# faasm/faabric

Hardware: AMD Instinct MI355X
Metric: MPI_Allreduce GB/s + batch-exec msgs/sec, 8-rank world at 1/2/4/8 MI355X (higher is better)
Workload: dtype fp32; 1 GPU; model=faabric composite: 256MB fp32 allreduce + 1MB alltoall + kvtouch batch, global_batch=128, parallelism=mpi1, allreduce_bytes=268435456, pingpong_bytes=0, kv_bytes=4096, full=False, snapshot_bytes_per_rank=0, snapshot_dirty=random-scattered 25pct, random-byte region, gpu=True

## Files before the change

### cpp/bindings/bindings_runtime.cpp

```cpp
#include <pybind11/functional.h>
#include <pybind11/pybind11.h>
#include <pybind11/stl.h>

#include "faabricamd/endpoint.h"
#include "faabricamd/executor.h"
#include "faabricamd/flat.h"
#include "faabricamd/hipipc.h"
#include "faabricamd/planner.h"
#include "faabricamd/ptp.h"
#include "faabricamd/runner.h"
#include "faabricamd/scheduler.h"
#include "faabricamd/snapshot.h"
#include "faabricamd/state.h"
#include "faabricamd/util.h"
#include "faabricamd/utilextras.h"
#include "faabricamd/dirty.h"
#include <hip/hip_runtime.h>

namespace py = pybind11;
using namespace faabricamd;

namespace faabricamd {
void registerBenchFunctions();
std::map<std::string, std::vector<uint8_t>> benchLastOutputs();
void registerMpiExampleFunctions();
}

void initRuntimeBindings(py::module_& m)
{
    m.def("set_endpoint_host", [](const std::string& host) {
        getSystemConfig().endpointHost = host;
    });
    m.def("get_endpoint_host",
          [] { return getSystemConfig().endpointHost; });
    m.def("set_planner_host", [](const std::string& host) {
        getSystemConfig().plannerHost = host;
        resetPlannerClient();
    });
    m.def("set_batch_scheduler_mode", [](const std::string& mode) {
        resetBatchScheduler(mode);
    });
    m.def("test_make_scheduling_decision",
          [](const std::string& mode,
             const std::vector<std::tuple<std::string, int, int>>& hosts,
             int nMessages,
             int32_t appId,
             bool migration,
             const std::vector<std::pair<int32_t, std::vector<std::string>>>&
               inFlight) {
              std::shared_ptr<BatchScheduler> sched;
              if (mode == "bin-pack") {
                  sched = std::make_shared<BinPackScheduler>();
              } else if (mode == "compact") {
                  sched = std::make_shared<CompactScheduler>();
              } else if (mode == "spot") {
                  sched = std::make_shared<SpotScheduler>();
              } else {
                  throw FaabricException("bad mode");
              }
              HostMap hostMap;
              for (const auto& [ip, slots, used] : hosts) {
                  hostMap[ip] =
                    std::make_shared<HostState>(ip, slots, used);
              }
              InFlightReqs reqs;
              for (const auto& [ifAppId, ifHosts] : inFlight) {
                  auto ber = std::make_shared<BatchExecuteRequest>();
                  ber->appId = ifAppId;
                  ber->user = "t";
                  ber->function = "t";
                  auto dec =
                    std::make_shared<SchedulingDecision>(ifAppId, 1);
                  int idx = 0;
                  for (const auto& h : ifHosts) {
                      Message m;
                      m.id = ifAppId * 1000 + idx;
                      m.appId = ifAppId;
                      m.appIdx = idx;
                      m.groupIdx = idx;
                      ber->messages.push_back(m);
                      dec->addMessage(h, m);
                      idx++;
                  }
                  reqs[ifAppId] = { ber, dec };
              }
              BatchExecuteRequest req;
              req.appId = appId;
              req.user = "t";
              req.function = "t";
              req.type = migration ? BatchExecuteType::MIGRATION
                                   : BatchExecuteType::FUNCTIONS;
              for (int i = 0; i < nMessages; i++) {
                  Message m;
                  m.id = appId * 1000 + i;
                  m.appId = appId;
                  m.appIdx = i;
                  m.groupIdx = i;
                  req.messages.push_back(m);
              }
              return *sched->makeSchedulingDecision(hostMap, reqs, req);
          },
          py::arg("mode"),
          py::arg("hosts"),
          py::arg("n_messages"),
          py::arg("app_id") = 12345,
          py::arg("migration") = false,
          py::arg("in_flight") =
            std::vector<std::pair<int32_t, std::vector<std::string>>>{});
    m.def("decision_cache_size",
          [] { return DecisionCache::get().size(); });
    m.def("decision_cache_clear", [] { DecisionCache::get().clear(); });

    py::class_<SchedulingDecision>(m, "SchedulingDecision")
      .def(py::init<>())
      .def_readwrite("app_id", &SchedulingDecision::appId)
      .def_readwrite("group_id", &SchedulingDecision::groupId)
      .def_readwrite("n_functions", &SchedulingDecision::nFunctions)
      .def_readwrite("hosts", &SchedulingDecision::hosts)
      .def_readwrite("message_ids", &SchedulingDecision::messageIds)
      .def_readwrite("app_idxs", &SchedulingDecision::appIdxs)
      .def_readwrite("group_idxs", &SchedulingDecision::groupIdxs)
      .def_readwrite("mpi_ports", &SchedulingDecision::mpiPorts);

    m.def("NOT_ENOUGH_SLOTS", [] { return NOT_ENOUGH_SLOTS; });
    m.def("DO_NOT_MIGRATE", [] { return DO_NOT_MIGRATE; });
    m.def("MUST_FREEZE", [] { return MUST_FREEZE; });

    py::class_<PlannerRuntime>(m, "PlannerRuntime")
      .def(py::init<>())
      .def("start",
           &PlannerRuntime::start,
           py::arg("with_snapshot_server") = true,
           py::arg("with_state_server") = false,
           py::call_guard<py::gil_scoped_release>())
      .def("shutdown",
           &PlannerRuntime::shutdown,
           py::call_guard<py::gil_scoped_release>());

    py::class_<FaabricMain>(m, "FaabricMain")
      .def(py::init([]() {
          return new FaabricMain(getExecutorFactory());
      }))
      .def("start_background",
           &FaabricMain::startBackground,
           py::call_guard<py::gil_scoped_release>())
      .def("shutdown",
           &FaabricMain::shutdown,
           py::call_guard<py::gil_scoped_release>());

    m.def("register_function",
          [](const std::string& user,
             const std::string& function,
             py::function fn) {
              FunctionRegistry::get().registerFunction(
                user, function, [fn](Message& msg) -> int32_t {
                    py::gil_scoped_acquire gil;
                    py::object result = fn(&msg);
                    if (result.is_none()) {
                        return 0;
                    }
                    return result.cast<int32_t>();
                });
          });
    m.def("clear_function_registry",
          [] { FunctionRegistry::get().clear(); });

    m.def("register_native_noop",
          [](const std::string& user, const std::string& function) {
              FunctionRegistry::get().registerFunction(
                user, function, [](Message&) -> int32_t { return 0; });
          });
    m.def("register_native_echo",
          [](const std::string& user, const std::string& function) {
              FunctionRegistry::get().registerFunction(
                user, function, [](Message& msg) -> int32_t {
                    msg.outputData.assign(msg.inputData.begin(),
                                          msg.inputData.end());
                    return 0;
                });
          });
    m.def("register_native_sleep",
          [](const std::string& user,
             const std::string& function,
             int sleepMs) {
              FunctionRegistry::get().registerFunction(
                user, function, [sleepMs](Message&) -> int32_t {
                    std::this_thread::sleep_for(
                      std::chrono::milliseconds(sleepMs));
                    return 0;
                });
          });

    m.def(
      "call_functions",
      [](const BatchExecuteRequest& reqIn) {
          auto req = std::make_shared<BatchExecuteRequest>(reqIn);
          py::gil_scoped_release release;
          return *getPlannerClient().callFunctions(req);
      });
    m.def(
      "get_message_result",
      [](int32_t appId, int32_t msgId, int timeoutMs) {
          py::gil_scoped_release release;
          return getPlannerClient().getMessageResult(appId, msgId, timeoutMs);
      });
    m.def("get_batch_results", [](int32_t appId) {
        py::gil_scoped_release release;
        return getPlannerClient().getBatchResults(appId);
    });
    m.def("get_available_hosts", [] {
        py::gil_scoped_release release;
        return getPlannerClient().getAvailableHosts();
    });
    m.def("get_num_migrations", [] {
        py::gil_scoped_release release;
        return getPlannerClient().getNumMigrations();
    });
    m.def("preload_scheduling_decision",
          [](int32_t appId, const SchedulingDecision& decision) {
              py::gil_scoped_release release;
              getPlannerClient().preloadSchedulingDecision(appId, decision);
          });
    m.def("planner_ping", [] {
        py::gil_scoped_release release;
        getPlannerClient().ping();
    });

    m.def("planner_reset", [] { Planner::get().reset(); });
    m.def("planner_flush_scheduling_state",
          [] { Planner::get().flushSchedulingState(); });
    m.def("planner_set_next_evicted_vms",
          [](const std::vector<std::string>& ips) {
              Planner::get().setNextEvictedVm(
                { ips.begin(), ips.end() });
          });
    m.def("planner_set_policy",
          [](const std::string& p) { Planner::get().setPolicy(p); });
    m.def("planner_get_policy", [] { return Planner::get().getPolicy(); });
    m.def("planner_num_in_flight_apps", [] {
        return (int)Planner::get().getInFlightApps().apps.size();
    });

    m.def("set_this_host_resources", [](int slots, int usedSlots) {
        HostResources res;
        res.slots = slots;
        res.usedSlots = usedSlots;
        Scheduler::get().setThisHostResources(res);
    });
    m.def("get_this_host_slots", [] {
        return Scheduler::get().getThisHostResources().slots;
    });
    m.def("get_executor_count",
          [] { return (int)Scheduler::get().getExecutorCount(); });
    m.def("scheduler_reset", [] {
        py::gil_scoped_release release;
        Scheduler::get().reset();
    });
    m.def("get_recorded_messages",
          [] { return Scheduler::get().getRecordedMessages(); });
    m.def("set_test_mode", &setTestMode);

    m.def("ptp_send",
          [](int32_t appId,
             int32_t groupId,
             int32_t sendIdx,
             int32_t recvIdx,
             const py::bytes& data,
             bool ordered) {
              std::string s = data;
              py::gil_scoped_release release;
              getPointToPointBroker().sendMessage(appId,
                                                  groupId,
                                                  sendIdx,
                                                  recvIdx,
                                                  (const uint8_t*)s.data(),
                                                  s.size(),
                                                  ordered);
          },
          py::arg("app_id"),
          py::arg("group_id"),
          py::arg("send_idx"),
          py::arg("recv_idx"),
          py::arg("data"),
          py::arg("ordered") = false);
    m.def("ptp_recv",
          [](int32_t groupId,
             int32_t sendIdx,
             int32_t recvIdx,
             bool ordered,
             int timeoutMs) {
              std::vector<uint8_t> out;
              {
                  py::gil_scoped_release release;
                  out = getPointToPointBroker().recvMessage(
                    groupId, sendIdx, recvIdx, ordered, timeoutMs);
              }
              return py::bytes((const char*)out.data(), out.size());
          },
          py::arg("group_id"),
          py::arg("send_idx"),
          py::arg("recv_idx"),
          py::arg("ordered") = false,
          py::arg("timeout_ms") = DEFAULT_QUEUE_TIMEOUT_MS);
    m.def("ptp_send_device",
          [](int32_t appId,
             int32_t groupId,
             int32_t sendIdx,
             int32_t recvIdx,
             uintptr_t devPtr,
             size_t size,
             bool ordered) {
              py::gil_scoped_release release;
              getPointToPointBroker().sendMessageDevice(
                appId, groupId, sendIdx, recvIdx, (const void*)devPtr,
                size, ordered);
          },
          py::arg("app_id"),
          py::arg("group_id"),
          py::arg("send_idx"),
          py::arg("recv_idx"),
          py::arg("dev_ptr"),
          py::arg("size"),
          py::arg("ordered") = false);
    m.def("ptp_recv_device",
          [](int32_t groupId,
             int32_t sendIdx,
             int32_t recvIdx,
             uintptr_t devPtr,
             size_t capacity,
             bool ordered,
             int timeoutMs) {
              py::gil_scoped_release release;
              return getPointToPointBroker().recvMessageDevice(
                groupId, sendIdx, recvIdx, (void*)devPtr, capacity,
                ordered, timeoutMs);
          },
          py::arg("group_id"),
          py::arg("send_idx"),
          py::arg("recv_idx"),
          py::arg("dev_ptr"),
          py::arg("capacity"),
          py::arg("ordered") = false,
          py::arg("timeout_ms") = DEFAULT_QUEUE_TIMEOUT_MS);
    m.def("ptp_group_barrier", [](int32_t groupId, int32_t groupIdx) {
        py::gil_scoped_release release;
        PointToPointGroup::getOrAwaitGroup(groupId)->barrier(groupIdx);
    });
    m.def("ptp_group_lock",
          [](int32_t groupId, int32_t groupIdx, bool recursive) {
              py::gil_scoped_release release;
              PointToPointGroup::getOrAwaitGroup(groupId)->lock(groupIdx,
                                                                recursive);
          },
          py::arg("group_id"),
          py::arg("group_idx"),
          py::arg("recursive") = false);
    m.def("ptp_group_unlock",
          [](int32_t groupId, int32_t groupIdx, bool recursive) {
              py::gil_scoped_release release;
              PointToPointGroup::getOrAwaitGroup(groupId)->unlock(groupIdx,
                                                                  recursive);
          },
          py::arg("group_id"),
          py::arg("group_idx"),
          py::arg("recursive") = false);
    m.def("ptp_group_notify", [](int32_t groupId, int32_t groupIdx) {
        py::gil_scoped_release release;
        PointToPointGroup::getOrAwaitGroup(groupId)->notify(groupIdx);
    });
    m.def("ptp_setup_local_mappings", [](const SchedulingDecision& d) {
        getPointToPointBroker().setUpLocalMappingsFromSchedulingDecision(d);
    });
    m.def("ptp_clear", [] { getPointToPointBroker().clear(); });
    m.def("_test_ptp_deliver_seq",
          [](int32_t appId,
             int32_t groupId,
             int32_t sendIdx,
             int32_t recvIdx,
             const py::bytes& data,
             uint32_t seq) {
              PointToPointMessage msg;
              msg.appId = appId;
              msg.groupId = groupId;
              msg.sendIdx = sendIdx;
              msg.recvIdx = recvIdx;
              std::string s = data;
              msg.data.assign(s.begin(), s.end());
              py::gil_scoped_release release;
              getPointToPointBroker().deliverRemoteMessage(msg, seq);
          });
    py::class_<PointToPointServer>(m, "PointToPointServerHandle")
      .def(py::init<>())
      .def("start",
           [](PointToPointServer& s) {
               py::gil_scoped_release release;
               s.start();
           })
      .def("stop", [](PointToPointServer& s) {
          py::gil_scoped_release release;
          s.stop();
      });
    py::class_<StateServer>(m, "StateServerHandle")
      .def(py::init<>())
      .def("start",
           [](StateServer& s) {
               py::gil_scoped_release release;
               s.start();
           })
      .def("stop", [](StateServer& s) {
          py::gil_scoped_release release;
          s.stop();
      });
    py::class_<SnapshotServer>(m, "SnapshotServerHandle")
      .def(py::init<>())
      .def("start",
           [](SnapshotServer& s) {
               py::gil_scoped_release release;
               s.start();
           })
      .def("stop", [](SnapshotServer& s) {
          py::gil_scoped_release release;
          s.stop();
      });
    m.def("snapshot_push_device_from_ptr",
          [](const std::string& host,
             const std::string& key,
             uintptr_t devPtr,
             size_t size) {
              py::gil_scoped_release release;
              getSnapshotClient(host)->pushDeviceSnapshotFromDevice(
                key, (const void*)devPtr, size);
          },
          py::arg("host"),
          py::arg("key"),
          py::arg("dev_ptr"),
          py::arg("size"));
    m.def("ipc_shipped", [] {
        return py::make_tuple(IpcSender::get().shippedSegments(),
                              IpcSender::get().shippedBytes());
    });
    m.def("ipc_available",
          [](const std::string& host) {
              py::gil_scoped_release release;
              return IpcSender::get().available(host);
          },
          py::arg("host"));
    m.def("ptp_wait_for_mappings", [](int32_t groupId) {
        py::gil_scoped_release release;
        getPointToPointBroker().waitForMappingsOnThisHost(groupId);
    });

    py::class_<StateKeyValue, std::shared_ptr<StateKeyValue>>(m,
                                                              "StateKeyValue")
      .def_property_readonly("user", &StateKeyValue::getUser)
      .def_property_readonly("key", &StateKeyValue::getKey)
      .def_property_readonly("size", &StateKeyValue::size)
      .def_property_readonly("is_master", &StateKeyValue::isMaster)
      .def_property_readonly("master_host", &StateKeyValue::getMasterHost)
      .def_property_readonly("on_device", &StateKeyValue::isOnDevice)
      .def_property_readonly("data_ptr",
                             [](StateKeyValue& kv) {
                                 return (uintptr_t)kv.getDataPtr();
                             })
      .def("get",
           [](StateKeyValue& kv) {
               std::vector<uint8_t> out;
               {
                   py::gil_scoped_release release;
                   out = kv.get();
               }
               return py::bytes((const char*)out.data(), out.size());
           })
      .def("set",
           [](StateKeyValue& kv, const py::bytes& data) {
               std::string s = data;
               py::gil_scoped_release release;
               kv.set((const uint8_t*)s.data(), s.size());
           })
      .def("get_chunk",
           [](StateKeyValue& kv, uint64_t offset, size_t len) {
               std::vector<uint8_t> out(len);
               {
                   py::gil_scoped_release release;
                   kv.getChunk(offset, out.data(), len);
               }
               return py::bytes((const char*)out.data(), out.size());
           })
      .def("set_chunk",
           [](StateKeyValue& kv, uint64_t offset, const py::bytes& data) {
               std::string s = data;
               py::gil_scoped_release release;
               kv.setChunk(offset, (const uint8_t*)s.data(), s.size());
           })
      .def("append",
           [](StateKeyValue& kv, const py::bytes& data) {
               std::string s = data;
               py::gil_scoped_release release;
               kv.append((const uint8_t*)s.data(), s.size());
           })
      .def("get_appended",
           [](StateKeyValue& kv, size_t n) {
               std::vector<std::vector<uint8_t>> vals;
               {
                   py::gil_scoped_release release;
                   vals = kv.getAppended(n);
               }
               py::list out;
               for (auto& v : vals) {
                   out.append(py::bytes((const char*)v.data(), v.size()));
               }
               return out;
           })
      .def("clear_appended", [](StateKeyValue& kv) {
          py::gil_scoped_release release;
          kv.clearAppended();
      })
      .def("pull",
           [](StateKeyValue& kv) {
               py::gil_scoped_release release;
               kv.pull();
           })
      .def("push_partial", [](StateKeyValue& kv) {
          py::gil_scoped_release release;
          kv.pushPartial();
      })
      .def("push_full", [](StateKeyValue& kv) {
          py::gil_scoped_release release;
          kv.pushFull();
      })
      .def("sync", [](StateKeyValue& kv) {
          py::gil_scoped_release release;
          kv.sync();
      });
    m.def("state_sync_all", [] {
        py::gil_scoped_release release;
        State::get().syncAll();
    });
    m.def("set_state_mode", [](const std::string& mode) {
        getSystemConfig().stateMode = mode;
    });
    m.def("state_acquire_lock",
          [](const std::string& user, const std::string& key,
             int expiryMs) {
              py::gil_scoped_release release;
              return State::get().acquireLock(user, key, expiryMs);
          },
          py::arg("user"),
          py::arg("key"),
          py::arg("expiry_ms") = 10000);
    m.def("state_release_lock",
          [](const std::string& user, const std::string& key,
             uint64_t token) {
              py::gil_scoped_release release;
              State::get().releaseLock(user, key, token);
          });

    m.def("state_get_kv_device",
          [](const std::string& user,
             const std::string& key,
             size_t size,
             int device) {
              return State::get().getKVDevice(user, key, size, device);
          },
          py::arg("user"),
          py::arg("key"),
          py::arg("size"),
          py::arg("device") = 0);
    m.def("state_get_kv",
          [](const std::string& user, const std::string& key, size_t size) {
              return State::get().getKV(user, key, size);
          });
    m.def("state_set_master_host",
          [](const std::string& user,
             const std::string& key,
             const std::string& host) {
              State::get().setMasterHost(user, key, host);
          });
    m.def("state_size",
          [](const std::string& user, const std::string& key) {
              py::gil_scoped_release release;
              return State::get().getStateSize(user, key);
          });
    m.def("state_clear_all", [] { State::get().forceClearAll(false); });
    m.def("state_kv_count", [] { return State::get().getKVCount(); });

    py::enum_<SnapshotDataType>(m, "SnapshotDataType")
      .value("Raw", SnapshotDataType::Raw)
      .value("Bool", SnapshotDataType::Bool)
      .value("Int", SnapshotDataType::Int)
      .value("Long", SnapshotDataType::Long)
      .value("Float", SnapshotDataType::Float)
      .value("Double", SnapshotDataType::Double);

    py::enum_<SnapshotMergeOperation>(m, "SnapshotMergeOperation")
      .value("Bytewise", SnapshotMergeOperation::Bytewise)
      .value("Sum", SnapshotMergeOperation::Sum)
      .value("Product", SnapshotMergeOperation::Product)
      .value("Subtract", SnapshotMergeOperation::Subtract)
      .value("Max", SnapshotMergeOperation::Max)
      .value("Min", SnapshotMergeOperation::Min)
      .value("XOR", SnapshotMergeOperation::XOR);

    py::class_<SnapshotDiff>(m, "SnapshotDiff")
      .def(py::init<>())
      .def_readwrite("data_type", &SnapshotDiff::dataType)
      .def_readwrite("operation", &SnapshotDiff::operation)
      .def_readwrite("offset", &SnapshotDiff::offset)
      .def_property(
        "data",
        [](const SnapshotDiff& d) {
            return py::bytes((const char*)d.getData(), d.size());
        },
        [](SnapshotDiff& d, const py::bytes& b) {
            std::string s = b;
            d.dataCopy.assign(s.begin(), s.end());
        });

    py::class_<SnapshotData, std::shared_ptr<SnapshotData>>(m,
                                                            "SnapshotData")
      .def(py::init([](const py::bytes& data, size_t maxSize) {
               std::string s = data;
               std::vector<uint8_t> v(s.begin(), s.end());
               if (maxSize == 0) {
                   return std::make_shared<SnapshotData>(v);
               }
               return std::make_shared<SnapshotData>(v, maxSize);
           }),
           py::arg("data"),
           py::arg("max_size") = 0)
      .def(py::init([](size_t size) {
          return std::make_shared<SnapshotData>(size);
      }))
      .def_property_readonly("size", &SnapshotData::getSize)
      .def_property_readonly("max_size", &SnapshotData::getMaxSize)
      .def("get_data",
           [](SnapshotData& s) {
               auto v = s.getDataCopy();
               return py::bytes((const char*)v.data(), v.size());
           })
      .def("copy_in_data",
           [](SnapshotData& s, const py::bytes& data, uint32_t offset) {
               std::string str = data;
               s.copyInData((const uint8_t*)str.data(), str.size(), offset);
           },
           py::arg("data"),
           py::arg("offset") = 0)
      .def("add_merge_region",
           &SnapshotData::addMergeRegion,
           py::arg("offset"),
           py::arg("length"),
           py::arg("data_type"),
           py::arg("operation"))
      .def("fill_gaps_with_bytewise_regions",
           &SnapshotData::fillGapsWithBytewiseRegions)
      .def("clear_merge_regions", &SnapshotData::clearMergeRegions)
      .def("diff_with_memory",
           [](SnapshotData& s, const py::bytes& updated) {
               std::string str = updated;
               return s.diffWithMemory((const uint8_t*)str.data(),
                                       str.size());
           })
      .def("diff_with_dirty_regions",
           [](SnapshotData& s,
              const py::bytes& updated,
              const std::vector<char>& dirtyPages) {
               std::string str = updated;
               return s.diffWithDirtyRegions(
                 (const uint8_t*)str.data(), str.size(), dirtyPages);
           })
      .def("apply_diffs", &SnapshotData::applyDiffs)
      .def("queue_diffs", &SnapshotData::queueDiffs)
      .def("write_queued_diffs", &SnapshotData::writeQueuedDiffs);

    m.def("snapshot_register",
          [](const std::string& key, std::shared_ptr<SnapshotData> snap) {
              SnapshotRegistry::get().registerSnapshot(key, snap);
          });
    m.def("snapshot_get", [](const std::string& key) {
        return SnapshotRegistry::get().getSnapshot(key);
    });
    m.def("snapshot_exists", [](const std::string& key) {
        return SnapshotRegistry::get().snapshotExists(key);
    });
    m.def("snapshot_delete", [](const std::string& key) {
        SnapshotRegistry::get().deleteSnapshot(key);
    });
    m.def("snapshot_count",
          [] { return SnapshotRegistry::get().getSnapshotCount(); });
    m.def("snapshot_clear", [] { SnapshotRegistry::get().clear(); });

    m.def("get_batch_requests_sent_mock", [] {
        return getBatchRequestsSentMock();
    });
    m.def("clear_mocked_function_calls", &clearMockedFunctionCalls);

    m.def("delta_default_config", [] { return DeltaConfig{}.str(); });
    m.def("flat_encode_push",
          [](const std::string& key, uint64_t maxSize,
             const py::bytes& contents,
             const std::vector<std::tuple<int32_t, uint64_t, int32_t,
                                          int32_t>>& regions) {
              FlatSnapshotPush req;
              req.key = key;
              req.maxSize = maxSize;
              std::string c = contents;
              req.contents.assign(c.begin(), c.end());
              for (auto& [off, len, dt, op] : regions) {
                  FlatMergeRegion m;
                  m.offset = off;
                  m.length = len;
                  m.dataType = dt;
                  m.mergeOp = op;
                  req.mergeRegions.push_back(m);
              }
              std::string out = req.encode();
              return py::bytes(out);
          });
    m.def("flat_decode_push", [](const py::bytes& buf) {
        std::string s = buf;
        auto req = FlatSnapshotPush::decode(s);
        py::list regions;
        for (auto& m : req.mergeRegions) {
            regions.append(py::make_tuple(m.offset, m.length, m.dataType,
                                          m.mergeOp));
        }
        return py::make_tuple(
          req.key, req.maxSize,
          py::bytes((const char*)req.contents.data(),
                    req.contents.size()),
          regions);
    });
    m.def("flat_encode_thread_result",
          [](int32_t appId, int32_t messageId, int32_t returnValue,
             const std::string& key,
             const std::vector<std::tuple<int32_t, int32_t, int32_t,
                                          py::bytes>>& diffs) {
              FlatThreadResult req;
              req.appId = appId;
              req.messageId = messageId;
              req.returnValue = returnValue;
              req.key = key;
              for (auto& [off, dt, op, data] : diffs) {
                  FlatSnapshotDiff d;
                  d.offset = off;
                  d.dataType = dt;
                  d.mergeOp = op;
                  std::string s = data;
                  d.data.assign(s.begin(), s.end());
                  req.diffs.push_back(std::move(d));
              }
              return py::bytes(req.encode());
          });
    m.def("flat_decode_thread_result", [](const py::bytes& buf) {
        std::string s = buf;
        auto req = FlatThreadResult::decode(s);
        py::list diffs;
        for (auto& d : req.diffs) {
            diffs.append(py::make_tuple(
              d.offset, d.dataType, d.mergeOp,
              py::bytes((const char*)d.data.data(), d.data.size())));
        }
        return py::make_tuple(req.appId, req.messageId, req.returnValue,
                              req.key, diffs, req.executedHost);
    });
    m.def("delta_encode",
          [](const py::bytes& oldData,
             const py::bytes& newData,
             const std::string& config) {
              std::string o = oldData;
              std::string n = newData;
              DeltaConfig conf = config.empty() ? DeltaConfig{}
                                                : DeltaConfig::parse(config);
              auto out = deltaEncode({ o.begin(), o.end() },
                                     { n.begin(), n.end() },
                                     conf);
              return py::bytes((const char*)out.data(), out.size());
          },
          py::arg("old_data"),
          py::arg("new_data"),
          py::arg("config") = "");
    m.def("delta_apply",
          [](const py::bytes& oldData, const py::bytes& delta) {
              std::string o = oldData;
              std::string d = delta;
              auto out = deltaApply({ o.begin(), o.end() },
                                    { d.begin(), d.end() });
              return py::bytes((const char*)out.data(), out.size());
          });
    m.def("prof_summary", &profSummary);
    m.def("prof_clear", &profClear);
    m.def("set_up_crash_handler", &setUpCrashHandler);
    m.def("pin_thread_to_free_cpu", &pinThreadToFreeCpu);

    m.def("_selftest_segfault_tracker", [] {
        py::gil_scoped_release release;
        SegfaultDirtyTracker tracker;
        PageAlignedBuffer buf;
        buf.resize(16 * 4096);
        tracker.startTracking(buf.data(), buf.size());
        buf.data()[3 * 4096 + 5] = 42;
        buf.data()[9 * 4096] = 7;
        tracker.stopTracking(buf.data(), buf.size());
        auto dirty = tracker.getDirtyPages(buf.data(), buf.size());
        int nDirty = 0;
        for (char c : dirty) {
            nDirty += c != 0;
        }
        return nDirty == 2 && dirty[3] == 1 && dirty[9] == 1;
    });

    m.def("_selftest_uffd_tracker", []() -> py::object {
        if (!UffdDirtyTracker::isAvailable()) {
            return py::none();
        }
        bool ok;
        {
            py::gil_scoped_release release;
            UffdDirtyTracker tracker;
            PageAlignedBuffer buf;
            buf.resize(16 * 4096);
            tracker.startTracking(buf.data(), buf.size());
            buf.data()[2 * 4096 + 11] = 42;
            buf.data()[14 * 4096] = 7;
            tracker.stopTracking(buf.data(), buf.size());
            auto dirty = tracker.getDirtyPages(buf.data(), buf.size());
            int nDirty = 0;
            for (char d : dirty) {
                nDirty += d != 0;
            }
            ok = nDirty == 2 && dirty[2] == 1 && dirty[14] == 1;
        }
        return py::bool_(ok);
    });

    m.def("_selftest_softpte_tracker", []() -> py::object {
        if (!SoftPTEDirtyTracker::isAvailable()) {
            return py::none();
        }
        bool ok;
        {
            py::gil_scoped_release release;
            SoftPTEDirtyTracker tracker;
            PageAlignedBuffer buf;
            buf.resize(16 * 4096);
            std::memset(buf.data(), 1, buf.size());
            tracker.startTracking(buf.data(), buf.size());
            buf.data()[5 * 4096 + 3] = 42;
            buf.data()[12 * 4096] = 7;
            tracker.stopTracking(buf.data(), buf.size());
            auto dirty = tracker.getDirtyPages(buf.data(), buf.size());
            ok = dirty.size() == 16 && dirty[5] == 1 && dirty[12] == 1;
        }
        return py::bool_(ok);
    });

    m.def("_debug_runtime_sizes", [] {
        py::dict d;
        d["planner_app_results"] = Planner::get().debugAppResultsCount();
        d["planner_done_apps"] = Planner::get().debugDoneAppsCount();
        d["planner_in_flight"] = Planner::get().debugInFlightCount();
        d["broker_mappings"] = getPointToPointBroker().debugMappingsCount();
        d["broker_channels"] = getPointToPointBroker().debugChannelsCount();
        d["broker_send_seqs"] = getPointToPointBroker().debugSendSeqsCount();
        d["decision_cache"] = DecisionCache::get().size();
        return d;
    });
    m.def("_debug_kv_commit_stats", [] {
        KvCommitStats s = kvCommitStats();
        py::dict d;
        d["launches"] = s.launches;
        d["pages"] = s.pages;
        return d;
    });
    m.def("_debug_kv_sweep_bitmap",
          [](size_t nPages, const std::vector<uint64_t>& setBits) {
              size_t nWords = (nPages + 63) / 64;
              auto words = std::make_unique<std::atomic<uint64_t>[]>(
                std::max<size_t>(nWords, 1));
              for (size_t w = 0; w < nWords; w++) {
                  words[w].store(0);
              }
              for (uint64_t b : setBits) {
                  if (b >= nPages) {
                      throw FaabricException("bit beyond the bitmap");
                  }
                  words[b / 64].fetch_or(1ULL << (b % 64));
              }
              std::vector<uint32_t> pages(nPages);
              size_t n =
                kvSweepDirtyBitmap(words.get(), nPages, pages.data());
              pages.resize(n);
              std::vector<uint64_t> after(nWords);
              for (size_t w = 0; w < nWords; w++) {
                  after[w] = words[w].load();
              }
              return py::make_tuple(pages, after);
          },
          py::arg("n_pages"),
          py::arg("set_bits"));
    m.def("wait_batch_done",
          [](int32_t appId, int timeoutMs) {
              py::gil_scoped_release release;
              return getPlannerClient().waitBatchDone(appId, timeoutMs);
          },
          py::arg("app_id"),
          py::arg("timeout_ms") = 30000);
    m.def("set_bound_timeout",
          [](int ms) { getSystemConfig().boundTimeout = ms; });
    m.def("reap_stale_executors", [] {
        py::gil_scoped_release release;
        return Scheduler::get().reapStaleExecutors();
    });
    m.def("register_bench_functions", [] { registerBenchFunctions(); });
    m.def("bench_last_outputs", [] {
        py::dict d;
        for (const auto& [name, data] : benchLastOutputs()) {
            d[py::str(name)] =
              py::bytes((const char*)data.data(), data.size());
        }
        return d;
    });
    m.def("register_mpi_example_functions",
          [] { registerMpiExampleFunctions(); });

    m.def("execute_threads",
          [](const std::string& user,
             const std::string& function,
             int nThreads,
             const std::vector<std::tuple<uint32_t, size_t, int, int>>&
               regions,
             const py::bytes& inputData,
             bool elastic) {
              Executor* exec = ExecutorContext::get().getExecutor();
              std::string input = inputData;
              std::vector<std::pair<int32_t, int32_t>> results;
              {
                  py::gil_scoped_release release;
                  auto req = std::make_shared<BatchExecuteRequest>(
                    batchExecFactory(user, function, nThreads));
                  req->elasticScaleHint = elastic;
                  for (auto& m2 : req->messages) {
                      m2.inputData.assign(input.begin(), input.end());
                  }
                  std::vector<SnapshotMergeRegion> mr;
                  for (const auto& [off, len, dt, op] : regions) {
                      mr.emplace_back(off,
                                      len,
                                      (SnapshotDataType)dt,
                                      (SnapshotMergeOperation)op);
                  }
                  results = exec->executeThreads(req, mr);
              }
              py::list out;
              for (auto& [msgId, rv] : results) {
                  out.append(py::make_tuple(msgId, rv));
              }
              return out;
          },
          py::arg("user"),
          py::arg("function"),
          py::arg("n_threads"),
          py::arg("merge_regions") =
            std::vector<std::tuple<uint32_t, size_t, int, int>>{},
          py::arg("input_data") = py::bytes(""),
          py::arg("elastic") = false);

    m.def("chain_function",
          [](const std::string& user,
             const std::string& function,
             const py::bytes& input) {
              std::string s = input;
              std::vector<uint8_t> in(s.begin(), s.end());
              py::gil_scoped_release release;
              return chainFunction(user, function, in);
          },
          py::arg("user"),
          py::arg("function"),
          py::arg("input") = py::bytes(""));
    m.def("await_chained_call", [](int32_t msgId, int timeoutMs) {
        py::gil_scoped_release release;
        return awaitChainedCall(msgId, timeoutMs);
    },
          py::arg("msg_id"),
          py::arg("timeout_ms") = 60000);
    m.def("get_exec_graph_json", [](int32_t appId, int32_t msgId) {
        return getExecGraphJson(appId, msgId);
    });
    m.def("migration_point",
          [](const py::bytes& reentryInput) {
              std::string s = reentryInput;
              std::vector<uint8_t> in(s.begin(), s.end());
              py::gil_scoped_release release;
              return migrationPoint(in);
          },
          py::arg("reentry_input") = py::bytes(""));
    m.def("MIGRATED_FUNCTION_RETURN_VALUE",
          [] { return MIGRATED_FUNCTION_RETURN_VALUE; });
    m.def("FROZEN_FUNCTION_RETURN_VALUE",
          [] { return FROZEN_FUNCTION_RETURN_VALUE; });

    py::class_<PlannerEndpoint>(m, "PlannerEndpoint")
      .def(py::init<int>(), py::arg("port") = PLANNER_HTTP_PORT)
      .def("start",
           &PlannerEndpoint::start,
           py::call_guard<py::gil_scoped_release>())
      .def("stop",
           &PlannerEndpoint::stop,
           py::call_guard<py::gil_scoped_release>())
      .def("handle", [](PlannerEndpoint& ep, const std::string& body) {
          std::pair<int, std::string> out;
          {
              py::gil_scoped_release release;
              out = ep.handle(body);
          }
          return py::make_tuple(out.first, out.second);
      });

    m.def("executor_set_memory_size", [](size_t n) {
        ExecutorContext::get().getExecutor()->setMemorySize(n);
    });
    m.def("executor_memory_size", [] {
        return ExecutorContext::get().getExecutor()->getMemoryView().second;
    });
    m.def("executor_write_memory", [](size_t offset, const py::bytes& data) {
        std::string s = data;
        auto [base, size] = ExecutorContext::get().getExecutor()
                              ->getMemoryView();
        if (offset + s.size() > size) {
            throw FaabricException("executor memory write out of bounds");
        }
        std::memcpy(base + offset, s.data(), s.size());
    });
    m.def("executor_read_memory", [](size_t offset, size_t n) {
        auto [base, size] = ExecutorContext::get().getExecutor()
                              ->getMemoryView();
        if (offset + n > size) {
            throw FaabricException("executor memory read out of bounds");
        }
        return py::bytes((const char*)base + offset, n);
    });

    m.def("executor_set_device_memory_size", [](size_t n) {
        py::gil_scoped_release release;
        ExecutorContext::get().getExecutor()->setDeviceMemorySize(n);
    });
    m.def("executor_device_ptr", [] {
        return (uintptr_t)ExecutorContext::get()
          .getExecutor()
          ->getDeviceMemoryView()
          .first;
    });
    m.def("executor_device_write_memory",
          [](size_t offset, const py::bytes& data) {
              std::string s = data;
              auto [base, size] = ExecutorContext::get()
                                    .getExecutor()
                                    ->getDeviceMemoryView();
              if (base == nullptr || offset + s.size() > size) {
                  throw FaabricException("device arena write out of bounds");
              }
              py::gil_scoped_release release;
              if (hipMemcpy(base + offset, s.data(), s.size(),
                            hipMemcpyHostToDevice) != hipSuccess) {
                  throw FaabricException("device arena write failed");
              }
          });
    m.def("executor_device_read_memory", [](size_t offset, size_t n) {
        auto [base, size] =
          ExecutorContext::get().getExecutor()->getDeviceMemoryView();
        if (base == nullptr || offset + n > size) {
            throw FaabricException("device arena read out of bounds");
        }
        std::vector<uint8_t> out(n);
        {
            py::gil_scoped_release release;
            if (hipMemcpy(out.data(), base + offset, n,
                          hipMemcpyDeviceToHost) != hipSuccess) {
                throw FaabricException("device arena read failed");
            }
        }
        return py::bytes((const char*)out.data(), out.size());
    });
}
```

### cpp/include/faabricamd/executor.h

```cpp
#pragma once

#include <atomic>
#include <functional>
#include <memory>
#include <string>
#include <thread>
#include <vector>

#include "faabricamd/messages.h"
#include "faabricamd/queue.h"
#include "faabricamd/dirty.h"
#include "faabricamd/snapshot.h"

namespace faabricamd {

class Executor;


class ExecutorContext
{
  public:
    static bool isSet();
    static void set(Executor* executor,
                    std::shared_ptr<BatchExecuteRequest> req,
                    int msgIdx);
    static void unset();
    static ExecutorContext& get();

    Executor* getExecutor() const { return executor; }
    std::shared_ptr<BatchExecuteRequest> getBatchRequest() const
    {
        return req;
    }
    Message& getMsg();
    int getMsgIdx() const { return msgIdx; }

  private:
    Executor* executor = nullptr;
    std::shared_ptr<BatchExecuteRequest> req;
    int msgIdx = 0;
};


using FaabricFunction = std::function<int32_t(Message&)>;

class FunctionRegistry
{
  public:
    static FunctionRegistry& get();
    void registerFunction(const std::string& user,
                          const std::string& function,
                          FaabricFunction fn);
    FaabricFunction* getFunction(const std::string& user,
                                 const std::string& function);
    void clear();

  private:
    std::mutex mx;
    std::map<std::string, FaabricFunction> functions;
};


struct ExecutorTask
{
    ExecutorTask() = default;
    ExecutorTask(int msgIdxIn, std::shared_ptr<BatchExecuteRequest> reqIn)
      : msgIdx(msgIdxIn)
      , req(std::move(reqIn))
    {}
    int msgIdx = 0;
    std::shared_ptr<BatchExecuteRequest> req;
    bool stop = false;
};

class Executor
{
  public:
    explicit Executor(Message& msg);
    virtual ~Executor();

    void executeTasks(std::vector<int> msgIdxs,
                      std::shared_ptr<BatchExecuteRequest> req);

    std::vector<std::pair<int32_t, int32_t>> executeThreads(
      std::shared_ptr<BatchExecuteRequest> req,
      const std::vector<SnapshotMergeRegion>& mergeRegions);

    virtual int32_t executeTask(int threadPoolIdx,
                                int msgIdx,
                                std::shared_ptr<BatchExecuteRequest> req);

    virtual std::pair<uint8_t*, size_t> getMemoryView();
    virtual void setMemorySize(size_t newSize);
    void setDeviceMemorySize(size_t newSize);
    std::pair<uint8_t*, size_t> getDeviceMemoryView();
    bool hasDeviceArena() const { return deviceArena != nullptr; }
    virtual void restore(const std::string& snapshotKey);
    virtual void reset(Message& msg);
    virtual void flush();

    bool tryClaim();
    void claim();
    void releaseClaim();
    bool isClaimed() const { return claimed.load(); }

    long getMillisSinceLastExec() const;
    void shutdown();

    std::string id;
    Message boundMsg;
    int gpuDevice = -1;

    void setThreadResult(Message& msg,
                         int32_t returnValue,
                         const std::string& key,
                         const std::vector<SnapshotDiffMsg>& diffs);

  protected:
    void threadPoolThread(int poolIdx);
    void handleTaskResult(Message& msg,
                          int32_t returnValue,
                          std::shared_ptr<BatchExecuteRequest> req,
                          bool isLastInBatch);

    int threadPoolSize = 0;
    std::vector<std::shared_ptr<Queue<ExecutorTask>>> threadTaskQueues;
    std::vector<std::thread> threadPoolThreads;
    std::mutex threadsMx;

    std::atomic<bool> claimed{ false };
    std::atomic<int64_t> lastExecMs{ 0 };

    std::string lastForkSnapshotKey;
    std::vector<std::string> lastForkRemoteHosts;
    void cleanupForkSnapshot();

    std::shared_ptr<std::atomic<int>> batchCounter;

    PageAlignedBuffer dummyMemory;

    uint8_t* deviceArena = nullptr;
    size_t deviceArenaSize = 0;
};

class ExecutorFactory
{
  public:
    virtual ~ExecutorFactory() = default;
    virtual std::shared_ptr<Executor> createExecutor(Message& msg)
    {
        return std::make_shared<Executor>(msg);
    }
    virtual void flushHost() {}
};

void setExecutorFactory(std::shared_ptr<ExecutorFactory> factory);
std::shared_ptr<ExecutorFactory> getExecutorFactory();

int32_t chainFunction(const std::string& user,
                      const std::string& function,
                      const std::vector<uint8_t>& input);
Message awaitChainedCall(int32_t msgId, int timeoutMs = 60000);

int32_t migrationPoint(const std::vector<uint8_t>& reentryInput);

}
```

### cpp/include/faabricamd/planner.h

```cpp
#pragma once

#include <deque>
#include <atomic>
#include <map>
#include <memory>
#include <set>
#include <shared_mutex>
#include <thread>
#include <vector>

#include "faabricamd/messages.h"
#include "faabricamd/queue.h"
#include "faabricamd/scheduling.h"
#include "faabricamd/transport.h"

namespace faabricamd {

enum class PlannerCalls : uint8_t
{
    Ping = 1,
    GetAvailableHosts = 2,
    RegisterHost = 3,
    RemoveHost = 4,
    SetMessageResult = 8,
    SetMessageResultBatch = 15,
    GetMessageResult = 9,
    GetBatchResults = 10,
    GetSchedulingDecision = 11,
    GetNumMigrations = 12,
    CallBatch = 13,
    PreloadSchedulingDecision = 14,
    WaitBatchDone = 16,
};

inline constexpr int NUM_MPI_PORTS_PER_HOST = 64;

struct PlannerHost
{
    Host info;
    std::vector<bool> mpiPortUsed =
      std::vector<bool>(NUM_MPI_PORTS_PER_HOST, false);
};

struct PlannerState
{
    std::map<std::string, std::shared_ptr<PlannerHost>> hostMap;
    InFlightReqs inFlightReqs;
    std::map<int32_t, std::shared_ptr<SchedulingDecision>>
      preloadedSchedulingDecisions;
    std::map<int32_t, std::map<int32_t, std::shared_ptr<Message>>> appResults;
    std::deque<std::pair<int64_t, int32_t>> doneApps;
    std::map<int32_t, std::vector<std::string>> appResultWaiters;
    std::map<int32_t, std::shared_ptr<BatchExecuteRequest>> evictedRequests;
    std::map<int32_t, std::vector<std::string>> batchDoneWaiters;
    std::map<int32_t,
             std::vector<std::pair<int32_t, std::vector<std::string>>>>
      supersededGroups;
    std::set<std::string> nextEvictedHostIps;
    int numMigrations = 0;
};

class Planner
{
  public:
    static Planner& get();

    PlannerConfig getConfig();
    void printConfig();

    bool registerHost(const Host& hostIn, bool overwrite);
    void removeHost(const Host& hostIn);
    std::vector<Host> getAvailableHosts();

    size_t debugAppResultsCount();
    size_t debugDoneAppsCount();
    size_t debugInFlightCount();

    bool registerBatchDoneWaiter(int32_t appId, const std::string& host);

    std::shared_ptr<SchedulingDecision> callBatch(
      std::shared_ptr<BatchExecuteRequest> req);
    void dispatchSchedulingDecision(
      std::shared_ptr<BatchExecuteRequest> req,
      std::shared_ptr<SchedulingDecision> decision);
    void preloadSchedulingDecision(
      int32_t appId,
      std::shared_ptr<SchedulingDecision> decision);
    std::shared_ptr<SchedulingDecision> getSchedulingDecision(int32_t appId);

    void setMessageResult(std::shared_ptr<Message> msg);
    void setMessageResults(std::vector<std::shared_ptr<Message>>& msgs);
    std::shared_ptr<Message> getMessageResult(const Message& msg);
    std::shared_ptr<BatchExecuteRequestStatus> getBatchResults(int32_t appId);

    int getNumMigrations();
    GetInFlightAppsResponse getInFlightApps();
    void setNextEvictedVm(const std::set<std::string>& vmIps);
    void setPolicy(const std::string& policy);
    std::string getPolicy();

    void reset();
    void flushExecutors();
    void flushSchedulingState();

    int hostTimeoutMs = 5000;

  private:
    void purgeOldResultsLocked();
    void setMessageResultLocked(
      const std::shared_ptr<Message>& msg,
      std::vector<std::pair<std::string, std::shared_ptr<Message>>>& waiters,
      std::vector<std::pair<std::string, int32_t>>& batchWaiters,
      std::vector<std::pair<std::string, int32_t>>& groupClears);

    Planner();

    std::shared_mutex plannerMx;
    PlannerState state;

    bool isHostExpired(const PlannerHost& host, int64_t nowMs) const;
    void flushHosts();
    std::shared_ptr<SchedulingDecision> getPreloadedSchedulingDecision(
      int32_t appId,
      const BatchExecuteRequest& req);
    int32_t claimHostMpiPort(std::shared_ptr<PlannerHost>& host);
    void releaseHostMpiPort(std::shared_ptr<PlannerHost>& host, int32_t port);
};


class PlannerServer : public MessageEndpointServer
{
  public:
    PlannerServer();
    ~PlannerServer() override;
    void doAsyncRecv(uint8_t code,
                     const std::string& body,
                     uint32_t seq) override;
    std::string doSyncRecv(uint8_t code, const std::string& body) override;

  private:
    void resultWorkerLoop();
    Queue<std::string> resultQueue;
    std::vector<std::thread> resultWorkers;
    std::atomic<bool> resultWorkersStop{ false };
};

class PlannerClient
{
  public:
    PlannerClient();
    ~PlannerClient();

    void ping();
    std::vector<Host> getAvailableHosts();
    int32_t registerHost(const Host& host, bool overwrite);
    void removeHost(const Host& host);

    std::shared_ptr<SchedulingDecision> callFunctions(
      std::shared_ptr<BatchExecuteRequest> req);

    void setMessageResult(std::shared_ptr<Message> msg);
    void setMessageResults(std::vector<std::shared_ptr<Message>>& msgs);
    void setMessageResultsBatch(
      const std::vector<std::shared_ptr<Message>>& msgs);
    void setMessageResultLocally(std::shared_ptr<Message> msg);

    Message getMessageResult(const Message& msg, int timeoutMs);
    Message getMessageResult(int32_t appId, int32_t msgId, int timeoutMs);
    BatchExecuteRequestStatus getBatchResults(int32_t appId);
    std::pair<bool, int> getBatchStatusCounts(int32_t appId);

    bool waitBatchDone(int32_t appId, int timeoutMs);

    SchedulingDecision getSchedulingDecision(int32_t appId);
    void preloadSchedulingDecision(
      int32_t appId,
      const SchedulingDecision& decision);
    int getNumMigrations();

    void startKeepAlive();
    void stopKeepAlive();
    void clearCache();

  private:
    MessageEndpointClient rpc;

    std::mutex resultsMx;
    std::condition_variable resultsCv;
    std::map<int32_t, std::shared_ptr<Message>> localResults;

    class KeepAliveThread;
    std::shared_ptr<KeepAliveThread> keepAlive;
};

PlannerClient& getPlannerClient();
void resetPlannerClient();

}
```

### cpp/include/faabricamd/scheduler.h

```cpp
#pragma once

#include <memory>
#include <mutex>
#include <shared_mutex>
#include <unordered_map>
#include <vector>

#include "faabricamd/executor.h"
#include "faabricamd/messages.h"
#include "faabricamd/queue.h"
#include "faabricamd/transport.h"

namespace faabricamd {

enum class FunctionCalls : uint8_t
{
    ExecuteFunctions = 1,
    Flush = 2,
    SetMessageResult = 3,
    BatchDone = 4,
};

class Scheduler
{
  public:
    static Scheduler& get();

    void executeBatch(std::shared_ptr<BatchExecuteRequest> req);

    HostResources getThisHostResources();
    void setThisHostResources(const HostResources& res);

    int reapStaleExecutors();
    void startReaper();
    void stopReaper();

    std::shared_ptr<PendingMigration> checkForMigrationOpportunities(
      Message& msg,
      int32_t overwriteNewGroupId = 0);

    void flushLocally();
    void shutdown();
    void reset();

    std::vector<Message> getRecordedMessages();
    void clearRecordedMessages();

    size_t getExecutorCount();

  private:
    Scheduler();

    std::shared_ptr<Executor> claimExecutor(Message& msg);

    std::shared_mutex schedMx;
    struct WarmPool
    {
        std::vector<std::shared_ptr<Executor>> list;
        std::atomic<size_t> hint{ 0 };
    };
    std::unordered_map<std::string, std::unique_ptr<WarmPool>> executors;
    HostResources overriddenResources;
    bool resourcesOverridden = false;

    std::vector<Message> recordedMessages;

    class ReaperThread;
    std::shared_ptr<ReaperThread> reaper;
};

bool functionCallServerRunning();

class FunctionCallServer : public MessageEndpointServer
{
  public:
    FunctionCallServer();
    ~FunctionCallServer() override;
    void doAsyncRecv(uint8_t code,
                     const std::string& body,
                     uint32_t seq) override;
    std::string doSyncRecv(uint8_t code, const std::string& body) override;
};

class FunctionCallClient : public MessageEndpointClient
{
  public:
    explicit FunctionCallClient(const std::string& host);
    void executeFunctions(const BatchExecuteRequest& req);
    void setMessageResult(const Message& msg);
    void sendFlush();
    void batchDone(int32_t appId);
};

std::shared_ptr<FunctionCallClient> getFunctionCallClient(
  const std::string& host);

std::shared_ptr<FlagWaiter> batchDoneWaiterPrepare(int32_t appId);
void batchDoneWaiterDiscard(int32_t appId);
void signalBatchDone(int32_t appId);
void clearFunctionCallClients();

std::vector<std::pair<std::string, BatchExecuteRequest>>
getBatchRequestsSentMock();
void clearMockedFunctionCalls();

}
```

### cpp/include/faabricamd/scheduling.h

```cpp
#pragma once

#include <map>
#include <mutex>
#include <memory>
#include <set>
#include <string>
#include <vector>

#include "faabricamd/messages.h"

namespace faabricamd {

inline constexpr int32_t DO_NOT_MIGRATE = -98;
inline constexpr int32_t NOT_ENOUGH_SLOTS = -99;
inline constexpr int32_t MUST_FREEZE = -97;
inline const std::string MUST_EVICT_IP = "E.VI.CT.ME";

inline constexpr int32_t FIXED_SIZE_PRELOADED_DECISION_GROUPID = -99;

enum class DecisionType
{
    NO_DECISION_TYPE = 0,
    NEW = 1,
    DIST_CHANGE = 2,
    SCALE_CHANGE = 3,
};

class SchedulingDecision
{
  public:
    SchedulingDecision() = default;
    SchedulingDecision(int32_t appIdIn, int32_t groupIdIn)
      : appId(appIdIn)
      , groupId(groupIdIn)
    {}

    static SchedulingDecision fromPointToPointMappings(
      const PointToPointMappings& mappings);
    PointToPointMappings toPointToPointMappings() const;

    bool operator==(const SchedulingDecision& rhs) const
    {
        return appId == rhs.appId && groupId == rhs.groupId &&
               hosts == rhs.hosts && messageIds == rhs.messageIds;
    }

    int32_t appId = 0;
    int32_t groupId = 0;
    int32_t nFunctions = 0;
    std::vector<std::string> hosts;
    std::vector<int32_t> messageIds;
    std::vector<int32_t> appIdxs;
    std::vector<int32_t> groupIdxs;
    std::vector<int32_t> mpiPorts;
    std::string returnHost;

    bool isSingleHost() const;
    void addMessage(const std::string& host, const Message& msg);
    void addMessage(const std::string& host,
                    int32_t messageId,
                    int32_t appIdx,
                    int32_t groupIdx);
    void addMessageInPosition(int32_t pos,
                              const std::string& host,
                              int32_t messageId,
                              int32_t appIdx,
                              int32_t groupIdx,
                              int32_t mpiPort);
    int32_t removeMessage(int32_t messageId);
    std::set<std::string> uniqueHosts() const;
    void print() const;
};

struct HostState
{
    HostState(std::string ipIn, int slotsIn, int usedSlotsIn)
      : ip(std::move(ipIn))
      , slots(slotsIn)
      , usedSlots(usedSlotsIn)
    {}
    std::string ip;
    int slots;
    int usedSlots;
};

using HostMap = std::map<std::string, std::shared_ptr<HostState>>;
using InFlightPair = std::pair<std::shared_ptr<BatchExecuteRequest>,
                               std::shared_ptr<SchedulingDecision>>;
using InFlightReqs = std::map<int32_t, InFlightPair>;

class BatchScheduler
{
  public:
    virtual ~BatchScheduler() = default;

    static DecisionType getDecisionType(
      const InFlightReqs& inFlightReqs,
      const BatchExecuteRequest& req);

    virtual std::shared_ptr<SchedulingDecision> makeSchedulingDecision(
      HostMap& hostMap,
      const InFlightReqs& inFlightReqs,
      const BatchExecuteRequest& req) = 0;

  protected:
    static int numSlotsAvailable(const std::shared_ptr<HostState>& h)
    {
        return std::max(0, h->slots - h->usedSlots);
    }
};

class BinPackScheduler : public BatchScheduler
{
  public:
    std::shared_ptr<SchedulingDecision> makeSchedulingDecision(
      HostMap& hostMap,
      const InFlightReqs& inFlightReqs,
      const BatchExecuteRequest& req) override;
};

class CompactScheduler : public BatchScheduler
{
  public:
    std::shared_ptr<SchedulingDecision> makeSchedulingDecision(
      HostMap& hostMap,
      const InFlightReqs& inFlightReqs,
      const BatchExecuteRequest& req) override;
};

class SpotScheduler : public BatchScheduler
{
  public:
    std::shared_ptr<SchedulingDecision> makeSchedulingDecision(
      HostMap& hostMap,
      const InFlightReqs& inFlightReqs,
      const BatchExecuteRequest& req) override;
};

class DecisionCache
{
  public:
    static DecisionCache& get();
    std::shared_ptr<SchedulingDecision> getCachedDecision(
      const BatchExecuteRequest& req);
    void addCachedDecision(const BatchExecuteRequest& req,
                           const SchedulingDecision& decision);
    void clear();
    size_t size();

  private:
    std::string keyOf(const BatchExecuteRequest& req);
    std::mutex mx;
    std::map<std::string, std::shared_ptr<SchedulingDecision>> cache;
};

std::shared_ptr<BatchScheduler> getBatchScheduler();
void resetBatchScheduler();
void resetBatchScheduler(const std::string& newMode);
std::string getBatchSchedulerMode();

std::shared_ptr<SchedulingDecision> minimiseNumOfMigrations(
  std::shared_ptr<SchedulingDecision> newDecision,
  std::shared_ptr<SchedulingDecision> oldDecision);

}
```

### cpp/include/faabricamd/utilextras.h

```cpp
#pragma once

#include <cstdint>
#include <string>
#include <vector>

namespace faabricamd {


struct DeltaConfig
{
    size_t pageSize = 4096;
    bool xorWithOld = true;
    bool compress = true;
    bool useZstd = true;

    static DeltaConfig parse(const std::string& s);
    std::string str() const;
};

std::vector<uint8_t> deltaEncode(const std::vector<uint8_t>& oldData,
                                 const std::vector<uint8_t>& newData,
                                 const DeltaConfig& conf = {});

std::vector<uint8_t> deltaApply(const std::vector<uint8_t>& oldData,
                                const std::vector<uint8_t>& delta);


void profStart(const std::string& name);
void profEnd(const std::string& name);
std::vector<std::pair<std::string, double>> profTotalsMs();
void profClear();
std::string profSummary();

#define PROF_START(name) ::faabricamd::profStart(#name);
#define PROF_END(name) ::faabricamd::profEnd(#name);

void setUpCrashHandler();

int pinThreadToFreeCpu();
void unpinThisThread();

}
```

### cpp/src/batchsched.cpp

```cpp
#include "faabricamd/scheduling.h"
#include "faabricamd/util.h"

#include <algorithm>
#include <mutex>

namespace faabricamd {


SchedulingDecision SchedulingDecision::fromPointToPointMappings(
  const PointToPointMappings& mappings)
{
    SchedulingDecision d(mappings.appId, mappings.groupId);
    for (const auto& m : mappings.mappings) {
        d.addMessageInPosition(
          d.nFunctions, m.host, m.messageId, m.appIdx, m.groupIdx, m.mpiPort);
    }
    return d;
}

PointToPointMappings SchedulingDecision::toPointToPointMappings() const
{
    PointToPointMappings out;
    out.appId = appId;
    out.groupId = groupId;
    for (int i = 0; i < nFunctions; i++) {
        PointToPointMapping m;
        m.host = hosts[i];
        m.messageId = messageIds[i];
        m.appIdx = appIdxs[i];
        m.groupIdx = groupIdxs[i];
        m.mpiPort = mpiPorts[i];
        out.mappings.push_back(std::move(m));
    }
    return out;
}

bool SchedulingDecision::isSingleHost() const
{
    const std::string& thisHost = getSystemConfig().endpointHost;
    return std::all_of(hosts.begin(), hosts.end(), [&](const auto& h) {
        return h == thisHost;
    });
}

void SchedulingDecision::addMessage(const std::string& host,
                                    const Message& msg)
{
    addMessage(host, msg.id, msg.appIdx, msg.groupIdx);
}

void SchedulingDecision::addMessage(const std::string& host,
                                    int32_t messageId,
                                    int32_t appIdx,
                                    int32_t groupIdx)
{
    nFunctions++;
    hosts.push_back(host);
    messageIds.push_back(messageId);
    appIdxs.push_back(appIdx);
    groupIdxs.push_back(groupIdx);
    mpiPorts.push_back(0);
}

void SchedulingDecision::addMessageInPosition(int32_t pos,
                                              const std::string& host,
                                              int32_t messageId,
                                              int32_t appIdx,
                                              int32_t groupIdx,
                                              int32_t mpiPort)
{
    int32_t desiredSize = std::max<int32_t>(pos + 1, nFunctions);
    nFunctions = desiredSize;
    if ((int32_t)hosts.size() < desiredSize) {
        hosts.resize(desiredSize);
        messageIds.resize(desiredSize, 0);
        appIdxs.resize(desiredSize, 0);
        groupIdxs.resize(desiredSize, 0);
        mpiPorts.resize(desiredSize, 0);
    }
    hosts[pos] = host;
    messageIds[pos] = messageId;
    appIdxs[pos] = appIdx;
    groupIdxs[pos] = groupIdx;
    mpiPorts[pos] = mpiPort;
}

int32_t SchedulingDecision::removeMessage(int32_t messageId)
{
    auto it = std::find(messageIds.begin(), messageIds.end(), messageId);
    if (it == messageIds.end()) {
        return 0;
    }
    size_t idx = (size_t)std::distance(messageIds.begin(), it);
    int32_t port = mpiPorts[idx];
    nFunctions--;
    size_t last = messageIds.size() - 1;
    hosts[idx] = std::move(hosts[last]);
    messageIds[idx] = messageIds[last];
    appIdxs[idx] = appIdxs[last];
    groupIdxs[idx] = groupIdxs[last];
    mpiPorts[idx] = mpiPorts[last];
    hosts.pop_back();
    messageIds.pop_back();
    appIdxs.pop_back();
    groupIdxs.pop_back();
    mpiPorts.pop_back();
    return port;
}

std::set<std::string> SchedulingDecision::uniqueHosts() const
{
    return { hosts.begin(), hosts.end() };
}

void SchedulingDecision::print() const
{
    FAM_DEBUG("decision app=%d group=%d n=%d", appId, groupId, nFunctions);
    for (int i = 0; i < nFunctions; i++) {
        FAM_DEBUG("  msg=%d appIdx=%d grpIdx=%d host=%s port=%d",
                  messageIds[i],
                  appIdxs[i],
                  groupIdxs[i],
                  hosts[i].c_str(),
                  mpiPorts[i]);
    }
}


DecisionType BatchScheduler::getDecisionType(const InFlightReqs& inFlightReqs,
                                             const BatchExecuteRequest& req)
{
    if (inFlightReqs.find(req.appId) == inFlightReqs.end()) {
        return DecisionType::NEW;
    }
    if (req.type == BatchExecuteType::MIGRATION) {
        return DecisionType::DIST_CHANGE;
    }
    return DecisionType::SCALE_CHANGE;
}

using HostPtr = std::shared_ptr<HostState>;

static std::map<std::string, int> hostFreqCountOf(
  const SchedulingDecision& decision)
{
    std::map<std::string, int> freq;
    for (const auto& h : decision.hosts) {
        freq[h] += 1;
    }
    return freq;
}

static bool moreCapacityFirst(const HostPtr& a, const HostPtr& b)
{
    int availA = std::max(0, a->slots - a->usedSlots);
    int availB = std::max(0, b->slots - b->usedSlots);
    if (availA != availB) {
        return availA > availB;
    }
    if (a->slots != b->slots) {
        return a->slots > b->slots;
    }
    return a->ip > b->ip;
}

static auto makeFreqComparator(const std::map<std::string, int>& freq)
{
    return [&freq](const HostPtr& a, const HostPtr& b) {
        auto count = [&freq](const HostPtr& h) {
            auto it = freq.find(h->ip);
            return it == freq.end() ? 0 : it->second;
        };
        int fa = count(a);
        int fb = count(b);
        if (fa != fb) {
            return fa > fb;
        }
        return moreCapacityFirst(a, b);
    };
}

static bool binPackInto(std::vector<HostPtr>& sortedHosts,
                        const BatchExecuteRequest& req,
                        SchedulingDecision& decision)
{
    int numLeft = (int)req.messages.size();
    int msgIdx = 0;
    for (auto& h : sortedHosts) {
        int avail = std::max(0, h->slots - h->usedSlots);
        int n = std::min(numLeft, avail);
        for (int i = 0; i < n; i++) {
            decision.addMessage(h->ip, req.messages[msgIdx++]);
        }
        numLeft -= n;
        if (numLeft == 0) {
            return true;
        }
    }
    return false;
}

std::shared_ptr<SchedulingDecision> minimiseNumOfMigrations(
  std::shared_ptr<SchedulingDecision> newDecision,
  std::shared_ptr<SchedulingDecision> oldDecision)
{
    auto out = std::make_shared<SchedulingDecision>(oldDecision->appId,
                                                    oldDecision->groupId);
    auto freq = hostFreqCountOf(*newDecision);

    for (int i = 0; i < oldDecision->nFunctions; i++) {
        const auto& oldHost = oldDecision->hosts[i];
        auto it = freq.find(oldHost);
        if (it != freq.end() && it->second > 0) {
            out->addMessageInPosition(i,
                                      oldHost,
                                      oldDecision->messageIds[i],
                                      oldDecision->appIdxs[i],
                                      oldDecision->groupIdxs[i],
                                      oldDecision->mpiPorts[i]);
            it->second--;
        }
    }

    for (int i = 0; i < oldDecision->nFunctions; i++) {
        if (out->nFunctions <= i || out->hosts[i].empty()) {
            std::string nextHost;
            for (auto& [ip, n] : freq) {
                if (n > 0) {
                    nextHost = ip;
                    break;
                }
            }
            if (nextHost.empty()) {
                throw FaabricException("migration histogram exhausted");
            }
            out->addMessageInPosition(i,
                                      nextHost,
                                      oldDecision->messageIds[i],
                                      oldDecision->appIdxs[i],
                                      oldDecision->groupIdxs[i],
                                      -1);
            freq[nextHost]--;
        }
    }
    return out;
}


static std::pair<int, int> localityScore(const SchedulingDecision& d)
{
    auto freq = hostFreqCountOf(d);
    if (freq.size() <= 1) {
        return { (int)freq.size(), 0 };
    }
    int total = 0;
    for (auto& [h, n] : freq) {
        total += n;
    }
    int score = 0;
    for (auto& [h, n] : freq) {
        score += n * (total - n);
    }
    return { (int)freq.size(), score / 2 };
}

std::shared_ptr<SchedulingDecision> BinPackScheduler::makeSchedulingDecision(
  HostMap& hostMap,
  const InFlightReqs& inFlightReqs,
  const BatchExecuteRequest& req)
{
    auto decision = std::make_shared<SchedulingDecision>(req.appId, 0);
    auto decisionType = getDecisionType(inFlightReqs, req);

    std::vector<HostPtr> sorted;
    for (auto& [ip, h] : hostMap) {
        sorted.push_back(h);
    }

    std::map<std::string, int> freq;
    if (decisionType != DecisionType::NEW) {
        freq = hostFreqCountOf(*inFlightReqs.at(req.appId).second);
    }

    switch (decisionType) {
        case DecisionType::NEW:
            std::sort(sorted.begin(), sorted.end(), moreCapacityFirst);
            break;
        case DecisionType::SCALE_CHANGE:
            std::sort(sorted.begin(), sorted.end(), makeFreqComparator(freq));
            break;
        case DecisionType::DIST_CHANGE: {
            for (auto& h : sorted) {
                auto it = freq.find(h->ip);
                if (it != freq.end()) {
                    h->usedSlots = std::max(0, h->usedSlots - it->second);
                }
            }
            auto freqCmp = makeFreqComparator(freq);
            std::sort(sorted.begin(),
                      sorted.end(),
                      [&](const HostPtr& a, const HostPtr& b) {
                          int availA = std::max(0, a->slots - a->usedSlots);
                          int availB = std::max(0, b->slots - b->usedSlots);
                          if (availA != availB) {
                              return availA > availB;
                          }
                          return freqCmp(a, b);
                      });
            break;
        }
        default:
            throw FaabricException("unrecognised decision type");
    }

    if (!binPackInto(sorted, req, *decision)) {
        return std::make_shared<SchedulingDecision>(NOT_ENOUGH_SLOTS,
                                                    NOT_ENOUGH_SLOTS);
    }

    if (decisionType == DecisionType::DIST_CHANGE) {
        auto oldDecision = inFlightReqs.at(req.appId).second;
        auto newScore = localityScore(*decision);
        auto oldScore = localityScore(*oldDecision);
        bool better = newScore.first != oldScore.first
                        ? newScore.first < oldScore.first
                        : newScore.second < oldScore.second;
        if (better) {
            return minimiseNumOfMigrations(decision, oldDecision);
        }
        return std::make_shared<SchedulingDecision>(DO_NOT_MIGRATE,
                                                    DO_NOT_MIGRATE);
    }
    return decision;
}


std::shared_ptr<SchedulingDecision> CompactScheduler::makeSchedulingDecision(
  HostMap& hostMap,
  const InFlightReqs& inFlightReqs,
  const BatchExecuteRequest& req)
{
    auto decision = std::make_shared<SchedulingDecision>(req.appId, 0);
    auto decisionType = getDecisionType(inFlightReqs, req);

    HostMap filtered = hostMap;
    for (const auto& [appId, pair] : inFlightReqs) {
        if (pair.first->subType == req.subType) {
            continue;
        }
        for (const auto& ip : pair.second->hosts) {
            filtered.erase(ip);
        }
    }

    std::vector<HostPtr> sorted;
    for (auto& [ip, h] : filtered) {
        sorted.push_back(h);
    }

    std::map<std::string, int> freq;
    if (decisionType != DecisionType::NEW) {
        freq = hostFreqCountOf(*inFlightReqs.at(req.appId).second);
    }

    switch (decisionType) {
        case DecisionType::NEW:
            std::sort(sorted.begin(), sorted.end(), moreCapacityFirst);
            break;
        case DecisionType::SCALE_CHANGE:
            std::sort(sorted.begin(), sorted.end(), makeFreqComparator(freq));
            break;
        case DecisionType::DIST_CHANGE: {
            for (auto& h : sorted) {
                auto it = freq.find(h->ip);
                if (it != freq.end()) {
                    h->usedSlots = std::max(0, h->usedSlots - it->second);
                }
            }
            std::sort(sorted.begin(),
                      sorted.end(),
                      [&](const HostPtr& a, const HostPtr& b) {
                          if (a->usedSlots != b->usedSlots) {
                              return a->usedSlots > b->usedSlots;
                          }
                          return moreCapacityFirst(a, b);
                      });
            break;
        }
        default:
            throw FaabricException("unrecognised decision type");
    }

    if (!binPackInto(sorted, req, *decision)) {
        return std::make_shared<SchedulingDecision>(NOT_ENOUGH_SLOTS,
                                                    NOT_ENOUGH_SLOTS);
    }

    if (decisionType == DecisionType::DIST_CHANGE) {
        auto oldDecision = inFlightReqs.at(req.appId).second;

        auto countFreeWith = [&](const SchedulingDecision& d) {
            std::map<std::string, int> used;
            for (auto& [ip, h] : filtered) {
                used[ip] = h->usedSlots;
            }
            for (const auto& ip : d.hosts) {
                used[ip]++;
            }
            int free = 0;
            for (auto& [ip, u] : used) {
                if (u == 0) {
                    free++;
                }
            }
            return free;
        };
        if (countFreeWith(*decision) > countFreeWith(*oldDecision)) {
            return minimiseNumOfMigrations(decision, oldDecision);
        }
        return std::make_shared<SchedulingDecision>(DO_NOT_MIGRATE,
                                                    DO_NOT_MIGRATE);
    }
    return decision;
}


std::shared_ptr<SchedulingDecision> SpotScheduler::makeSchedulingDecision(
  HostMap& hostMap,
  const InFlightReqs& inFlightReqs,
  const BatchExecuteRequest& req)
{
    auto decision = std::make_shared<SchedulingDecision>(req.appId, 0);
    auto decisionType = getDecisionType(inFlightReqs, req);

    std::set<std::string> evictedIps;
    HostMap filtered;
    for (auto& [ip, h] : hostMap) {
        if (h->ip == MUST_EVICT_IP) {
            evictedIps.insert(ip);
        } else {
            filtered[ip] = h;
        }
    }

    std::vector<HostPtr> sorted;
    for (auto& [ip, h] : filtered) {
        sorted.push_back(h);
    }

    std::map<std::string, int> freq;
    if (decisionType != DecisionType::NEW) {
        freq = hostFreqCountOf(*inFlightReqs.at(req.appId).second);
    }

    switch (decisionType) {
        case DecisionType::NEW:
            std::sort(sorted.begin(), sorted.end(), moreCapacityFirst);
            break;
        case DecisionType::SCALE_CHANGE:
            std::sort(sorted.begin(), sorted.end(), makeFreqComparator(freq));
            break;
        case DecisionType::DIST_CHANGE: {
            for (auto& h : sorted) {
                auto it = freq.find(h->ip);
                if (it != freq.end()) {
                    h->usedSlots = std::max(0, h->usedSlots - it->second);
                }
            }
            std::sort(sorted.begin(), sorted.end(), makeFreqComparator(freq));
            break;
        }
        default:
            throw FaabricException("unrecognised decision type");
    }

    bool fits = binPackInto(sorted, req, *decision);
    bool isDistChange = decisionType == DecisionType::DIST_CHANGE;

    if (!fits && !isDistChange) {
        return std::make_shared<SchedulingDecision>(NOT_ENOUGH_SLOTS,
                                                    NOT_ENOUGH_SLOTS);
    }

    if (isDistChange) {
        if (!fits) {
            return std::make_shared<SchedulingDecision>(MUST_FREEZE,
                                                        MUST_FREEZE);
        }
        auto oldDecision = inFlightReqs.at(req.appId).second;
        for (const auto& ip : oldDecision->hosts) {
            if (evictedIps.count(ip) > 0) {
                return minimiseNumOfMigrations(decision, oldDecision);
            }
        }
        return std::make_shared<SchedulingDecision>(DO_NOT_MIGRATE,
                                                    DO_NOT_MIGRATE);
    }
    return decision;
}


DecisionCache& DecisionCache::get()
{
    static DecisionCache cache;
    return cache;
}

std::string DecisionCache::keyOf(const BatchExecuteRequest& req)
{
    return req.user + "/" + req.function + "/" +
           std::to_string(req.messages.size());
}

std::shared_ptr<SchedulingDecision> DecisionCache::getCachedDecision(
  const BatchExecuteRequest& req)
{
    std::lock_guard<std::mutex> lock(mx);
    auto it = cache.find(keyOf(req));
    return it == cache.end() ? nullptr : it->second;
}

void DecisionCache::addCachedDecision(const BatchExecuteRequest& req,
                                      const SchedulingDecision& decision)
{
    std::lock_guard<std::mutex> lock(mx);
    cache[keyOf(req)] = std::make_shared<SchedulingDecision>(decision);
}

void DecisionCache::clear()
{
    std::lock_guard<std::mutex> lock(mx);
    cache.clear();
}

size_t DecisionCache::size()
{
    std::lock_guard<std::mutex> lock(mx);
    return cache.size();
}


static std::shared_ptr<BatchScheduler> currentScheduler;
static std::string currentMode;
static std::mutex schedulerMx;

std::shared_ptr<BatchScheduler> getBatchScheduler()
{
    std::lock_guard<std::mutex> lock(schedulerMx);
    if (currentScheduler != nullptr) {
        return currentScheduler;
    }
    currentMode = getSystemConfig().batchSchedulerMode;
    if (currentMode == "bin-pack") {
        currentScheduler = std::make_shared<BinPackScheduler>();
    } else if (currentMode == "compact") {
        currentScheduler = std::make_shared<CompactScheduler>();
    } else if (currentMode == "spot") {
        currentScheduler = std::make_shared<SpotScheduler>();
    } else {
        throw FaabricException("unrecognised batch scheduler mode: " +
                               currentMode);
    }
    return currentScheduler;
}

void resetBatchScheduler()
{
    std::lock_guard<std::mutex> lock(schedulerMx);
    currentScheduler = nullptr;
}

void resetBatchScheduler(const std::string& newMode)
{
    {
        std::lock_guard<std::mutex> lock(schedulerMx);
        currentScheduler = nullptr;
        getSystemConfig().batchSchedulerMode = newMode;
    }
    getBatchScheduler();
}

std::string getBatchSchedulerMode()
{
    getBatchScheduler();
    std::lock_guard<std::mutex> lock(schedulerMx);
    return currentMode;
}

}
```

### cpp/src/executor.cpp

```cpp
#include "faabricamd/executor.h"
#include "faabricamd/utilextras.h"
#include "faabricamd/mpi.h"
#include "faabricamd/ops.h"
#include "faabricamd/planner.h"

#include <hip/hip_runtime.h>
#include "faabricamd/snapshot.h"
#include "faabricamd/util.h"

#include <algorithm>
#include <cstring>

namespace faabricamd {

void resultBatcherEnqueue(std::shared_ptr<Message> msg);


static thread_local std::shared_ptr<ExecutorContext> currentContext;

bool ExecutorContext::isSet()
{
    return currentContext != nullptr;
}

void ExecutorContext::set(Executor* executor,
                          std::shared_ptr<BatchExecuteRequest> req,
                          int msgIdx)
{
    auto ctx = std::make_shared<ExecutorContext>();
    ctx->executor = executor;
    ctx->req = std::move(req);
    ctx->msgIdx = msgIdx;
    currentContext = ctx;
}

void ExecutorContext::unset()
{
    currentContext = nullptr;
}

ExecutorContext& ExecutorContext::get()
{
    if (!currentContext) {
        throw FaabricException("no executor context set");
    }
    return *currentContext;
}

Message& ExecutorContext::getMsg()
{
    return req->messages.at(msgIdx);
}


FunctionRegistry& FunctionRegistry::get()
{
    static FunctionRegistry reg;
    return reg;
}

void FunctionRegistry::registerFunction(const std::string& user,
                                        const std::string& function,
                                        FaabricFunction fn)
{
    std::lock_guard<std::mutex> lock(mx);
    functions[user + "/" + function] = std::move(fn);
}

FaabricFunction* FunctionRegistry::getFunction(const std::string& user,
                                               const std::string& function)
{
    std::lock_guard<std::mutex> lock(mx);
    auto it = functions.find(user + "/" + function);
    return it == functions.end() ? nullptr : &it->second;
}

void FunctionRegistry::clear()
{
    std::lock_guard<std::mutex> lock(mx);
    functions.clear();
}


Executor::Executor(Message& msg)
  : id(funcToString(msg.user, msg.function, 0) + "_" +
       std::to_string(generateGid()))
  , boundMsg(msg)
{
    threadPoolSize = std::min(getUsableCores(), 64);
    threadTaskQueues.resize(threadPoolSize);
    for (auto& q : threadTaskQueues) {
        q = std::make_shared<Queue<ExecutorTask>>();
    }
    threadPoolThreads.resize(threadPoolSize);
    lastExecMs = getGlobalClockEpochMillis();
}

void Executor::cleanupForkSnapshot()
{
    if (lastForkSnapshotKey.empty()) {
        return;
    }
    DeviceSnapshotRegistry::get().deleteSnapshot(lastForkSnapshotKey);
    SnapshotRegistry::get().deleteSnapshot(lastForkSnapshotKey);
    for (const auto& host : lastForkRemoteHosts) {
        try {
            getSnapshotClient(host)->deleteSnapshot(lastForkSnapshotKey);
        } catch (const std::exception& e) {
            FAM_DEBUG("remote fork-snapshot delete failed: %s", e.what());
        }
    }
    lastForkSnapshotKey.clear();
    lastForkRemoteHosts.clear();
}

Executor::~Executor()
{
    try {
        cleanupForkSnapshot();
    } catch (...) {
    }
    shutdown();
    if (deviceArena != nullptr) {
        hipFree(deviceArena);
    }
}

void Executor::setDeviceMemorySize(size_t newSize)
{
    if (!gpuAvailable()) {
        throw FaabricException("device arena requires a GPU");
    }
    size_t rounded =
      (newSize + DEVICE_PAGE - 1) / DEVICE_PAGE * DEVICE_PAGE;
    if (rounded <= deviceArenaSize) {
        deviceArenaSize = rounded;
        return;
    }
    int dev = gpuDevice >= 0 ? gpuDevice : 0;
    if (hipSetDevice(dev) != hipSuccess) {
        throw FaabricException("hipSetDevice failed");
    }
    uint8_t* fresh = nullptr;
    if (hipMalloc(&fresh, rounded) != hipSuccess) {
        throw FaabricException("device arena alloc failed");
    }
    hipMemset(fresh, 0, rounded);
    if (deviceArena != nullptr) {
        hipMemcpy(fresh, deviceArena, deviceArenaSize,
                  hipMemcpyDeviceToDevice);
        hipFree(deviceArena);
    }
    deviceArena = fresh;
    deviceArenaSize = rounded;
}

std::pair<uint8_t*, size_t> Executor::getDeviceMemoryView()
{
    return { deviceArena, deviceArenaSize };
}

void Executor::shutdown()
{
    std::lock_guard<std::mutex> lock(threadsMx);
    for (int i = 0; i < threadPoolSize; i++) {
        if (threadPoolThreads[i].joinable()) {
            ExecutorTask stopTask;
            stopTask.stop = true;
            threadTaskQueues[i]->enqueue(stopTask);
        }
    }
    for (auto& t : threadPoolThreads) {
        if (t.joinable()) {
            t.join();
        }
    }
}

long Executor::getMillisSinceLastExec() const
{
    return (long)(getGlobalClockEpochMillis() - lastExecMs.load());
}

bool Executor::tryClaim()
{
    bool expected = false;
    return claimed.compare_exchange_strong(expected, true);
}

void Executor::claim()
{
    claimed.store(true);
}

void Executor::releaseClaim()
{
    claimed.store(false);
}

void Executor::executeTasks(std::vector<int> msgIdxs,
                            std::shared_ptr<BatchExecuteRequest> req)
{
    lastExecMs = getGlobalClockEpochMillis();
    batchCounter = std::make_shared<std::atomic<int>>((int)msgIdxs.size());

    if (!req->snapshotKey.empty()) {
        restore(req->snapshotKey);
    } else if (!req->messages.empty() &&
               !req->messages[msgIdxs[0]].snapshotKey.empty() &&
               req->type != BatchExecuteType::THREADS) {
        const std::string& key = req->messages[msgIdxs[0]].snapshotKey;
        restore(key);
        if (startsWith(key, "migration_")) {
            SnapshotRegistry::get().deleteSnapshot(key);
            DeviceSnapshotRegistry::get().deleteSnapshot(key);
        }
    }

    if (req->type == BatchExecuteType::THREADS &&
        !req->snapshotKey.empty()) {
        auto tracker = getDirtyTracker();
        if (tracker->getType() == "segfault") {
            auto [base, size] = getMemoryView();
            if (size > 0) {
                tracker->startTracking(base, size);
            }
        }
    }

    std::lock_guard<std::mutex> lock(threadsMx);
    for (int msgIdx : msgIdxs) {
        int poolIdx = threadPoolSize == 0 ? 0 : msgIdx % threadPoolSize;
        if (!threadPoolThreads[poolIdx].joinable()) {
            threadPoolThreads[poolIdx] =
              std::thread([this, poolIdx] { threadPoolThread(poolIdx); });
        }
        threadTaskQueues[poolIdx]->enqueue(ExecutorTask(msgIdx, req));
    }
}

std::vector<std::pair<int32_t, int32_t>> Executor::executeThreads(
  std::shared_ptr<BatchExecuteRequest> req,
  const std::vector<SnapshotMergeRegion>& mergeRegions)
{
    Message& parentMsg = ExecutorContext::get().getMsg();
    std::string key = getMainThreadSnapshotKey(
      parentMsg.user, parentMsg.function, parentMsg.appId);

    bool onDevice = hasDeviceArena();
    {
        Message& pm = ExecutorContext::get().getMsg();
        std::string newKey = getMainThreadSnapshotKey(
          pm.user, pm.function, pm.appId);
        if (!lastForkSnapshotKey.empty() &&
            lastForkSnapshotKey != newKey) {
            cleanupForkSnapshot();
        }
    }
    std::shared_ptr<SnapshotData> snap;
    std::shared_ptr<DeviceSnapshot> dsnap;
    if (onDevice) {
        if (!mergeRegions.empty()) {
            throw FaabricException(
              "typed merge regions unsupported on the device arena "
              "(XOR page diffing applies)");
        }
        auto& dreg = DeviceSnapshotRegistry::get();
        if (dreg.snapshotExists(key) &&
            dreg.getSnapshot(key)->size() == deviceArenaSize) {
            dsnap = dreg.getSnapshot(key);
        } else {
            dsnap = std::make_shared<DeviceSnapshot>(
              deviceArenaSize, gpuDevice >= 0 ? gpuDevice : 0);
            dreg.registerSnapshot(key, dsnap);
        }
        dsnap->captureFromDevice(deviceArena);
    } else {
        auto [memBase, memSize] = getMemoryView();
        auto& reg = SnapshotRegistry::get();
        if (reg.snapshotExists(key)) {
            snap = reg.getSnapshot(key);
            snap->copyInData(memBase, memSize, 0);
        } else {
            snap = std::make_shared<SnapshotData>(
              std::vector<uint8_t>(memBase, memBase + memSize));
            reg.registerSnapshot(key, snap);
        }
        snap->clearMergeRegions();
        for (const auto& r : mergeRegions) {
            snap->addMergeRegion(r.offset, r.length, r.dataType,
                                 r.operation);
        }
    }

    req->appId = parentMsg.appId;
    req->type = BatchExecuteType::THREADS;
    req->snapshotKey = key;
    for (size_t i = 0; i < req->messages.size(); i++) {
        auto& m = req->messages[i];
        m.appId = parentMsg.appId;
        m.appIdx = (int32_t)i + 1;
        m.groupIdx = (int32_t)i + 1;
        m.snapshotKey = key;
        m.mainHost = getSystemConfig().endpointHost;
    }

    auto decision = getPlannerClient().callFunctions(req);
    if (decision->appId == NOT_ENOUGH_SLOTS) {
        throw FaabricException("not enough slots for thread fork");
    }

    lastForkSnapshotKey = key;
    {
        const std::string& thisHost = getSystemConfig().endpointHost;
        for (const auto& host : decision->uniqueHosts()) {
            if (host == thisHost) {
                continue;
            }
            if (std::find(lastForkRemoteHosts.begin(),
                          lastForkRemoteHosts.end(),
                          host) == lastForkRemoteHosts.end()) {
                lastForkRemoteHosts.push_back(host);
            }
            if (onDevice) {
                getSnapshotClient(host)->pushDeviceSnapshotFromDevice(
                  key, dsnap->data(), dsnap->size());
            } else {
                getSnapshotClient(host)->pushSnapshot(key, *snap);
            }
        }
    }

    std::vector<std::pair<int32_t, int32_t>> results;
    const auto& conf = getSystemConfig();
    std::set<int32_t> waitIds;
    for (const auto& m : req->messages) {
        waitIds.insert(m.id);
    }
    for (int i = 0; i < decision->nFunctions; i++) {
        int32_t id = decision->messageIds[i];
        if (id != 0 && id != parentMsg.id) {
            waitIds.insert(id);
        }
    }
    for (int32_t id : waitIds) {
        Message result = getPlannerClient().getMessageResult(
          parentMsg.appId, id, conf.globalMessageTimeout);
        results.emplace_back(id, result.returnValue);
    }
    if (onDevice) {
        dsnap->applyQueuedPackedDiffs();
        hipError_t err = hipMemcpy(deviceArena,
                                   dsnap->data(),
                                   dsnap->size(),
                                   hipMemcpyDeviceToDevice);
        if (err != hipSuccess ||
            hipStreamSynchronize(nullptr) != hipSuccess) {
            throw FaabricException("device snapshot merge-back failed");
        }
    } else {
        snap->writeQueuedDiffs();
        auto [memBase2, memSize2] = getMemoryView();
        snap->mapToMemory(memBase2, memSize2);
        snap->clearMergeRegions();
    }
    return results;
}

int32_t Executor::executeTask(int threadPoolIdx,
                              int msgIdx,
                              std::shared_ptr<BatchExecuteRequest> req)
{
    (void)threadPoolIdx;
    Message& msg = req->messages.at(msgIdx);
    FaabricFunction* fn =
      FunctionRegistry::get().getFunction(msg.user, msg.function);
    if (fn == nullptr) {
        throw FaabricException("function not registered: " + msg.user + "/" +
                               msg.function);
    }
    return (*fn)(msg);
}

std::pair<uint8_t*, size_t> Executor::getMemoryView()
{
    return { dummyMemory.data(), dummyMemory.size() };
}

void Executor::setMemorySize(size_t newSize)
{
    dummyMemory.resize(newSize);
}

void Executor::restore(const std::string& snapshotKey)
{
    const auto& conf = getSystemConfig();
    int64_t deadline = getGlobalClockEpochMillis() + conf.boundTimeout;
    while (true) {
        if (DeviceSnapshotRegistry::get().snapshotExists(snapshotKey)) {
            auto dsnap =
              DeviceSnapshotRegistry::get().getSnapshot(snapshotKey);
            if (deviceArenaSize < dsnap->size()) {
                setDeviceMemorySize(dsnap->size());
            }
            hipError_t err = hipMemcpy(deviceArena,
                                       dsnap->data(),
                                       dsnap->size(),
                                       hipMemcpyDeviceToDevice);
            if (err != hipSuccess ||
                hipStreamSynchronize(nullptr) != hipSuccess) {
                throw FaabricException("device snapshot restore failed");
            }
            return;
        }
        if (SnapshotRegistry::get().snapshotExists(snapshotKey)) {
            auto snap = SnapshotRegistry::get().getSnapshot(snapshotKey);
            if (dummyMemory.size() < snap->getSize()) {
                setMemorySize(snap->getSize());
            }
            auto [base, size] = getMemoryView();
            snap->mapToMemory(base, size);
            return;
        }
        if (getGlobalClockEpochMillis() >= deadline) {
            throw FaabricException("snapshot not found: " + snapshotKey);
        }
        usleep(10 * 1000);
    }
}

void Executor::reset(Message& msg)
{
    (void)msg;
}

void Executor::flush()
{
    FunctionRegistry::get().clear();
}

void Executor::setThreadResult(Message& msg,
                               int32_t returnValue,
                               const std::string& key,
                               const std::vector<SnapshotDiffMsg>& diffs)
{
    (void)key;
    (void)diffs;
    msg.returnValue = returnValue;
}

void Executor::threadPoolThread(int poolIdx)
{
    const auto& conf = getSystemConfig();
    while (true) {
        ExecutorTask task;
        try {
            task = threadTaskQueues[poolIdx]->dequeue(conf.boundTimeout);
        } catch (const QueueTimeoutException&) {
            continue;
        }
        if (task.stop) {
            break;
        }

        Message& msg = task.req->messages.at(task.msgIdx);
        int32_t returnValue = 0;
        ExecutorContext::set(this, task.req, task.msgIdx);
        try {
            PROF_START(exec_task)
            returnValue = executeTask(poolIdx, task.msgIdx, task.req);
            PROF_END(exec_task)
            if (msg.isMpi && msg.recordExecGraph &&
                MpiWorldRegistry::get().worldExists(msg.mpiWorldId)) {
                auto counts = MpiWorldRegistry::get()
                                .getWorld(msg.mpiWorldId)
                                .getMsgCountDetails(msg.mpiRank);
                for (const auto& [k, v] : counts) {
                    msg.intExecGraphDetails[k] = v;
                }
            }
        } catch (const FunctionMigratedException&) {
            FAM_DEBUG("task %d migrated", msg.id);
            returnValue = MIGRATED_FUNCTION_RETURN_VALUE;
        } catch (const FunctionFrozenException&) {
            FAM_DEBUG("task %d frozen", msg.id);
            returnValue = FROZEN_FUNCTION_RETURN_VALUE;
        } catch (const std::exception& e) {
            FAM_ERROR("task %d failed: %s", msg.id, e.what());
            returnValue = 1;
            msg.outputData = std::string("Task failed: ") + e.what();
        }
        ExecutorContext::unset();

        int remaining = batchCounter->fetch_sub(1) - 1;
        bool isLastInBatch = remaining == 0;
        handleTaskResult(msg, returnValue, task.req, isLastInBatch);
    }
}

void Executor::handleTaskResult(Message& msg,
                                int32_t returnValue,
                                std::shared_ptr<BatchExecuteRequest> req,
                                bool isLastInBatch)
{
    const auto& conf = getSystemConfig();
    msg.returnValue = returnValue;
    msg.executedHost = conf.endpointHost;
    msg.finishTimestamp = getGlobalClockEpochMillis();
    lastExecMs = getGlobalClockEpochMillis();

    bool isThreads = req->type == BatchExecuteType::THREADS;

    if (msg.isMpi && returnValue != MIGRATED_FUNCTION_RETURN_VALUE &&
        returnValue != FROZEN_FUNCTION_RETURN_VALUE &&
        MpiWorldRegistry::get().worldExists(msg.mpiWorldId)) {
        if (MpiWorldRegistry::get()
              .getWorld(msg.mpiWorldId)
              .rankFinished(msg.mpiRank)) {
            MpiWorldRegistry::get().clearWorld(msg.mpiWorldId);
        }
    }

    std::vector<SnapshotDiff> threadDiffs;
    bool deviceThreads =
      isThreads && !req->snapshotKey.empty() &&
      DeviceSnapshotRegistry::get().snapshotExists(req->snapshotKey);
    if (deviceThreads && isLastInBatch) {
        try {
            auto dsnap =
              DeviceSnapshotRegistry::get().getSnapshot(req->snapshotKey);
            uint32_t nd = dsnap->diffXor(deviceArena);
            if (nd > 0) {
                std::vector<uint32_t> pages;
                std::vector<uint8_t> payload;
                dsnap->gatherLastDiffToHost(pages, payload);
                std::vector<uint8_t> packed(4 + pages.size() * 4 +
                                            payload.size());
                uint32_t n = (uint32_t)pages.size();
                std::memcpy(packed.data(), &n, 4);
                std::memcpy(packed.data() + 4,
                            pages.data(),
                            pages.size() * 4);
                std::memcpy(packed.data() + 4 + pages.size() * 4,
                            payload.data(),
                            payload.size());
                threadDiffs.emplace_back(SnapshotDataType::Raw,
                                         SnapshotMergeOperation::XorPages,
                                         0,
                                         packed.data(),
                                         packed.size());
            }
        } catch (const std::exception& e) {
            FAM_ERROR("device thread diff failed: %s", e.what());
        }
    } else if (isThreads && isLastInBatch && !req->snapshotKey.empty()) {
        try {
            auto snap = SnapshotRegistry::get().getSnapshot(req->snapshotKey);
            auto [base, size] = getMemoryView();
            snap->fillGapsWithBytewiseRegions();
            auto tracker = getDirtyTracker();
            if (tracker->getType() == "segfault" && size > 0) {
                tracker->stopTracking(base, size);
                auto dirty = tracker->getDirtyPages(base, size);
                threadDiffs =
                  snap->diffWithDirtyRegions(base, size, dirty);
            } else {
                threadDiffs = snap->diffWithMemory(base, size);
            }
        } catch (const std::exception& e) {
            FAM_ERROR("thread diff failed: %s", e.what());
        }
    }

    if (isLastInBatch) {
        if (!isThreads) {
            try {
                reset(msg);
            } catch (const std::exception& e) {
                FAM_ERROR("executor reset failed: %s", e.what());
            }
        }
        releaseClaim();
    }

    if (isThreads && !req->snapshotKey.empty()) {
        const std::string& mainHost = msg.mainHost;
        if (mainHost == conf.endpointHost || mainHost.empty()) {
            if (!threadDiffs.empty()) {
                try {
                    if (deviceThreads) {
                        auto dsnap = DeviceSnapshotRegistry::get()
                                       .getSnapshot(req->snapshotKey);
                        for (auto& d : threadDiffs) {
                            dsnap->queuePackedDiff(d.dataCopy);
                        }
                    } else {
                        auto snap = SnapshotRegistry::get().getSnapshot(
                          req->snapshotKey);
                        snap->queueDiffs(threadDiffs);
                    }
                } catch (const std::exception& e) {
                    FAM_ERROR("queueing thread diffs failed: %s", e.what());
                }
            }
            auto resultMsg = std::make_shared<Message>(msg);
            PROF_START(result_rpc)
            getPlannerClient().setMessageResult(resultMsg);
            PROF_END(result_rpc)
        } else {
            getSnapshotClient(mainHost)->pushThreadResult(
              msg.appId, msg.id, returnValue, req->snapshotKey, threadDiffs);
        }
        return;
    }

    resultBatcherEnqueue(std::make_shared<Message>(msg));
}


namespace {

struct ResultBatcher
{
    std::mutex mx;
    std::condition_variable cv;
    std::vector<std::shared_ptr<Message>> queue;
    std::thread worker;
    bool stop = false;
    bool started = false;

    void ensureStarted()
    {
        std::lock_guard<std::mutex> lock(mx);
        if (started) {
            return;
        }
        started = true;
        worker = std::thread([this] { run(); });
    }

    void run()
    {
        std::vector<std::shared_ptr<Message>> batch;
        while (true) {
            {
                std::unique_lock<std::mutex> lock(mx);
                cv.wait(lock, [&] { return stop || !queue.empty(); });
                if (stop && queue.empty()) {
                    return;
                }
                batch.swap(queue);
            }
            try {
                PROF_START(result_batch_send)
                getPlannerClient().setMessageResultsBatch(batch);
                PROF_END(result_batch_send)
            } catch (const std::exception& e) {
                FAM_ERROR("result batch send failed: %s", e.what());
            }
            batch.clear();
        }
    }

    ~ResultBatcher()
    {
        {
            std::lock_guard<std::mutex> lock(mx);
            stop = true;
        }
        cv.notify_all();
        if (worker.joinable()) {
            worker.join();
        }
    }
};

ResultBatcher& resultBatcher()
{
    static ResultBatcher instance;
    return instance;
}

}

void resultBatcherEnqueue(std::shared_ptr<Message> msg)
{
    auto& b = resultBatcher();
    b.ensureStarted();
    {
        std::lock_guard<std::mutex> lock(b.mx);
        b.queue.push_back(std::move(msg));
    }
    b.cv.notify_one();
}


int32_t chainFunction(const std::string& user,
                      const std::string& function,
                      const std::vector<uint8_t>& input)
{
    Message& parent = ExecutorContext::get().getMsg();
    auto req = std::make_shared<BatchExecuteRequest>();
    req->appId = parent.appId;
    req->user = user;
    req->function = function;
    Message m = messageFactory(user, function);
    m.appId = parent.appId;
    m.appIdx = parent.appIdx;
    m.groupIdx = 1000 + (int32_t)(generateGid() % 14000);
    m.inputData = input;
    m.recordExecGraph = parent.recordExecGraph;
    req->messages.push_back(m);

    auto decision = getPlannerClient().callFunctions(req);
    if (decision->appId == NOT_ENOUGH_SLOTS) {
        throw FaabricException("not enough slots for chained call");
    }
    parent.chainedMsgIds.push_back(m.id);
    return m.id;
}

Message awaitChainedCall(int32_t msgId, int timeoutMs)
{
    Message& parent = ExecutorContext::get().getMsg();
    return getPlannerClient().getMessageResult(parent.appId, msgId,
                                               timeoutMs);
}


static std::shared_ptr<ExecutorFactory> executorFactory =
  std::make_shared<ExecutorFactory>();

void setExecutorFactory(std::shared_ptr<ExecutorFactory> factory)
{
    executorFactory = std::move(factory);
}

std::shared_ptr<ExecutorFactory> getExecutorFactory()
{
    return executorFactory;
}

}
```

### cpp/src/planner.cpp

```cpp
#include "faabricamd/planner.h"
#include "faabricamd/utilextras.h"
#include "faabricamd/ptp.h"
#include "faabricamd/scheduler.h"
#include "faabricamd/ops.h"
#include "faabricamd/snapshot.h"
#include "faabricamd/state.h"
#include "faabricamd/util.h"
#include "faabricamd/wire.h"

#include <string_view>
#include <algorithm>
#include <cassert>

namespace faabricamd {

Planner::Planner()
{
    hostTimeoutMs = getEnvVarInt("PLANNER_HOST_KEEPALIVE_MS", 5000);
}

Planner& Planner::get()
{
    static Planner planner;
    return planner;
}

PlannerConfig Planner::getConfig()
{
    PlannerConfig conf;
    conf.ip = getSystemConfig().endpointHost;
    conf.hostTimeout = hostTimeoutMs / 1000;
    conf.numThreadsHttpServer = 4;
    return conf;
}

void Planner::printConfig()
{
    FAM_INFO("planner config: hostTimeoutMs=%d", hostTimeoutMs);
}


bool Planner::isHostExpired(const PlannerHost& host, int64_t nowMs) const
{
    return (nowMs - host.info.registerTsEpochMs) > hostTimeoutMs;
}

bool Planner::registerHost(const Host& hostIn, bool overwrite)
{
    if (hostIn.ip.empty() || hostIn.slots < 0) {
        return false;
    }
    if (overwrite) {
        clearFunctionCallClients();
        clearSnapshotClients();
        clearStateClients();
        getPointToPointBroker().clearClients();
    }
    std::unique_lock lock(plannerMx);
    auto it = state.hostMap.find(hostIn.ip);
    if (it == state.hostMap.end() || overwrite) {
        auto h = std::make_shared<PlannerHost>();
        h->info = hostIn;
        h->info.usedSlots = 0;
        h->info.registerTsEpochMs = getGlobalClockEpochMillis();
        state.hostMap[hostIn.ip] = h;
        FAM_DEBUG("planner registered host %s (slots=%d)",
                  hostIn.ip.c_str(),
                  hostIn.slots);
    } else {
        it->second->info.registerTsEpochMs = getGlobalClockEpochMillis();
        it->second->info.slots = hostIn.slots;
    }
    return true;
}

void Planner::removeHost(const Host& hostIn)
{
    std::unique_lock lock(plannerMx);
    state.hostMap.erase(hostIn.ip);
}

std::vector<Host> Planner::getAvailableHosts()
{
    std::unique_lock lock(plannerMx);
    int64_t nowMs = getGlobalClockEpochMillis();
    std::vector<Host> out;
    for (auto it = state.hostMap.begin(); it != state.hostMap.end();) {
        if (isHostExpired(*it->second, nowMs)) {
            FAM_WARN("planner expiring host %s", it->first.c_str());
            it = state.hostMap.erase(it);
        } else {
            out.push_back(it->second->info);
            ++it;
        }
    }
    return out;
}


int32_t Planner::claimHostMpiPort(std::shared_ptr<PlannerHost>& host)
{
    for (int i = 0; i < NUM_MPI_PORTS_PER_HOST; i++) {
        if (!host->mpiPortUsed[i]) {
            host->mpiPortUsed[i] = true;
            return getSystemConfig().mpiBasePort + i;
        }
    }
    throw FaabricException("no free MPI ports on host " + host->info.ip);
}

void Planner::releaseHostMpiPort(std::shared_ptr<PlannerHost>& host,
                                 int32_t port)
{
    int idx = port - getSystemConfig().mpiBasePort;
    if (idx >= 0 && idx < NUM_MPI_PORTS_PER_HOST) {
        host->mpiPortUsed[idx] = false;
    }
}


std::shared_ptr<SchedulingDecision> Planner::getPreloadedSchedulingDecision(
  int32_t appId,
  const BatchExecuteRequest& req)
{
    auto full = state.preloadedSchedulingDecisions.at(appId);
    auto filtered =
      std::make_shared<SchedulingDecision>(full->appId, full->groupId);
    for (const auto& msg : req.messages) {
        auto it = std::find(
          full->groupIdxs.begin(), full->groupIdxs.end(), msg.groupIdx);
        if (it == full->groupIdxs.end()) {
            throw FaabricException("preloaded decision missing group idx " +
                                   std::to_string(msg.groupIdx));
        }
        size_t i = (size_t)std::distance(full->groupIdxs.begin(), it);
        filtered->addMessage(
          full->hosts[i], msg.id, full->appIdxs[i], full->groupIdxs[i]);
        filtered->mpiPorts[filtered->nFunctions - 1] = full->mpiPorts[i];
    }
    return filtered;
}

std::shared_ptr<SchedulingDecision> Planner::callBatch(
  std::shared_ptr<BatchExecuteRequest> req)
{
    int32_t appId = req->appId;
    std::unique_lock lock(plannerMx);

    auto scheduler = getBatchScheduler();
    auto decisionType =
      BatchScheduler::getDecisionType(state.inFlightReqs, *req);
    bool isNew = decisionType == DecisionType::NEW;
    bool isScaleChange = decisionType == DecisionType::SCALE_CHANGE;
    bool isDistChange = decisionType == DecisionType::DIST_CHANGE;
    bool isMpi = !req->messages.empty() && req->messages[0].isMpi;
    bool existsPreloadedDec =
      state.preloadedSchedulingDecisions.count(appId) > 0;

    HostMap hostMapCopy;
    for (const auto& [ip, h] : state.hostMap) {
        hostMapCopy[ip] = std::make_shared<HostState>(
          state.nextEvictedHostIps.count(ip) > 0 ? MUST_EVICT_IP : ip,
          h->info.slots,
          h->info.usedSlots);
    }

    if (isScaleChange && req->elasticScaleHint && !existsPreloadedDec) {
        auto oldDec = state.inFlightReqs.at(appId).second;
        const std::string& mainHost = oldDec->hosts.at(0);
        int numAvail = std::max(
          0,
          hostMapCopy.at(mainHost)->slots -
            hostMapCopy.at(mainHost)->usedSlots);
        int numRequested = (int)req->messages.size();
        int lastIdx =
          numRequested == 0 ? 0 : req->messages.back().groupIdx;
        for (int i = 0; i < numAvail - numRequested; i++) {
            int newIdx = lastIdx + i + 1;
            Message newMsg;
            if (numRequested == 0) {
                newMsg = state.inFlightReqs.at(appId).first->messages.at(0);
                newMsg.mainHost = mainHost;
                newMsg.funcPtr = req->groupId;
            } else {
                newMsg = req->messages.back();
            }
            newMsg.appIdx = newIdx;
            newMsg.groupIdx = newIdx;
            newMsg.id = generateGidInt32();
            req->messages.push_back(std::move(newMsg));
        }
    }

    if (isDistChange) {
        auto oldReq = state.inFlightReqs.at(appId).first;
        req->subType = oldReq->subType;
        req->messages = oldReq->messages;
    }

    std::shared_ptr<SchedulingDecision> decision;
    std::shared_ptr<BatchExecuteRequest> knownSizeReq;
    if (!isDistChange && existsPreloadedDec) {
        decision = getPreloadedSchedulingDecision(appId, *req);
        if (isScaleChange) {
            state.preloadedSchedulingDecisions.erase(appId);
        }
    } else if (isNew && isMpi) {
        knownSizeReq = std::make_shared<BatchExecuteRequest>(*req);
        int worldSize = req->messages[0].mpiWorldSize;
        for (int i = (int)req->messages.size(); i < worldSize; i++) {
            Message m;
            m.appId = appId;
            m.groupIdx = i;
            knownSizeReq->messages.push_back(std::move(m));
        }
        decision = scheduler->makeSchedulingDecision(
          hostMapCopy, state.inFlightReqs, *knownSizeReq);
    } else {
        decision = scheduler->makeSchedulingDecision(
          hostMapCopy, state.inFlightReqs, *req);
    }

    if (decision->appId == NOT_ENOUGH_SLOTS) {
        FAM_WARN("planner: not enough slots for app %d (requested %d)",
                 appId,
                 (int)req->messages.size());
        return decision;
    }
    if (decision->appId == DO_NOT_MIGRATE) {
        return decision;
    }
    if (decision->appId == MUST_FREEZE) {
        FAM_INFO("planner: freezing app %d", appId);
        state.evictedRequests[appId] = std::make_shared<BatchExecuteRequest>(
          *state.inFlightReqs.at(appId).first);
        return decision;
    }

    bool isSingleHost = false;
    {
        auto uniq = decision->uniqueHosts();
        isSingleHost = uniq.size() == 1;
    }
    if (!isSingleHost && req->singleHostHint) {
        return std::make_shared<SchedulingDecision>(NOT_ENOUGH_SLOTS,
                                                    NOT_ENOUGH_SLOTS);
    }

    bool isUnfreezeDispatch = false;
    if (state.evictedRequests.count(appId) > 0) {
        if (isNew && !isMpi) {
            state.evictedRequests.erase(appId);
        } else if (isNew && isMpi) {
            isUnfreezeDispatch = true;
            state.evictedRequests.erase(appId);
        } else if (isMpi && !isDistChange) {
            auto evictedBer = state.evictedRequests.at(appId);
            for (auto& m : req->messages) {
                for (size_t j = 1; j < evictedBer->messages.size(); j++) {
                    const auto& old = evictedBer->messages[j];
                    if (m.groupIdx == old.groupIdx) {
                        m.id = old.id;
                        m.funcPtr = old.funcPtr;
                        m.inputData = old.inputData;
                        m.snapshotKey = old.snapshotKey;
                        break;
                    }
                }
            }
            state.evictedRequests.erase(appId);
        }
    }

    bool skipClaim =
      decision->groupId == FIXED_SIZE_PRELOADED_DECISION_GROUPID;

    int32_t newGroupId = generateGidInt32();
    decision->groupId = newGroupId;
    updateBatchExecGroupId(*req, newGroupId);

    auto& broker = getPointToPointBroker();
    switch (decisionType) {
        case DecisionType::NEW: {
            for (int i = 0; i < decision->nFunctions; i++) {
                auto host = state.hostMap.at(decision->hosts[i]);
                host->info.usedSlots++;
                if (isMpi) {
                    try {
                        decision->mpiPorts[i] = claimHostMpiPort(host);
                    } catch (const std::exception& e) {
                        FAM_ERROR("mpi port claim failed for app %d: %s",
                                  appId,
                                  e.what());
                    }
                }
            }

            if (isMpi && knownSizeReq != nullptr && !isUnfreezeDispatch) {
                auto preload = std::make_shared<SchedulingDecision>(*decision);
                preload->groupId = FIXED_SIZE_PRELOADED_DECISION_GROUPID;
                state.preloadedSchedulingDecisions[appId] = preload;
                for (size_t i = 1; i < preload->messageIds.size(); i++) {
                    decision->removeMessage(preload->messageIds[i]);
                }
            }

            state.inFlightReqs[appId] = { req, decision };
            DecisionCache::get().addCachedDecision(*req, *decision);
            broker.setAndSendMappingsFromSchedulingDecision(*decision);
            break;
        }
        case DecisionType::SCALE_CHANGE: {
            if (!skipClaim) {
                for (int i = 0; i < decision->nFunctions; i++) {
                    state.hostMap.at(decision->hosts[i])->info.usedSlots++;
                }
            }
            auto oldReq = state.inFlightReqs.at(appId).first;
            auto oldDec = state.inFlightReqs.at(appId).second;
            updateBatchExecGroupId(*oldReq, newGroupId);
            oldDec->groupId = newGroupId;

            for (size_t i = 0; i < req->messages.size(); i++) {
                oldReq->messages.push_back(req->messages[i]);
                oldDec->addMessage(decision->hosts[i], req->messages[i]);
                if (!skipClaim && isMpi) {
                    oldDec->mpiPorts[oldDec->nFunctions - 1] =
                      claimHostMpiPort(
                        state.hostMap.at(decision->hosts[i]));
                } else if (skipClaim) {
                    oldDec->mpiPorts[oldDec->nFunctions - 1] =
                      decision->mpiPorts[i];
                }
            }
            broker.setAndSendMappingsFromSchedulingDecision(*oldDec);
            break;
        }
        case DecisionType::DIST_CHANGE: {
            auto oldReq = state.inFlightReqs.at(appId).first;
            auto oldDec = state.inFlightReqs.at(appId).second;

            std::set<std::string> evictedHosts;
            {
                auto newHosts = decision->uniqueHosts();
                for (const auto& h : oldDec->uniqueHosts()) {
                    if (newHosts.count(h) == 0) {
                        evictedHosts.insert(h);
                    }
                }
            }

            for (int i = 0; i < oldDec->nFunctions; i++) {
                if (decision->hosts[i] != oldDec->hosts[i]) {
                    auto oldHost = state.hostMap.at(oldDec->hosts[i]);
                    oldHost->info.usedSlots =
                      std::max(0, oldHost->info.usedSlots - 1);
                    releaseHostMpiPort(oldHost, oldDec->mpiPorts[i]);
                }
            }
            for (int i = 0; i < decision->nFunctions; i++) {
                if (decision->hosts[i] != oldDec->hosts[i]) {
                    auto newHost = state.hostMap.at(decision->hosts[i]);
                    newHost->info.usedSlots++;
                    try {
                        decision->mpiPorts[i] = claimHostMpiPort(newHost);
                    } catch (const std::exception& e) {
                        FAM_ERROR("mpi port claim failed: %s", e.what());
                    }
                }
            }

            state.numMigrations += 1;
            {
                auto oldHosts = oldDec->uniqueHosts();
                state.supersededGroups[appId].emplace_back(
                  oldDec->groupId,
                  std::vector<std::string>(oldHosts.begin(),
                                           oldHosts.end()));
            }
            updateBatchExecGroupId(*oldReq, newGroupId);
            state.inFlightReqs[appId] = { oldReq, decision };
            broker.setAndSendMappingsFromSchedulingDecision(*decision);
            broker.sendMappingsFromSchedulingDecision(*decision,
                                                      evictedHosts);
            break;
        }
        default:
            throw FaabricException("unrecognised decision type");
    }

    if (decisionType != DecisionType::DIST_CHANGE) {
        dispatchSchedulingDecision(req, decision);
    }
    return decision;
}

void Planner::dispatchSchedulingDecision(
  std::shared_ptr<BatchExecuteRequest> req,
  std::shared_ptr<SchedulingDecision> decision)
{
    std::map<std::string, std::shared_ptr<BatchExecuteRequest>> hostReqs;
    bool isSingleHost = decision->uniqueHosts().size() == 1;

    for (size_t i = 0; i < req->messages.size(); i++) {
        const std::string& host = decision->hosts.at(i);
        auto& hr = hostReqs[host];
        if (!hr) {
            hr = std::make_shared<BatchExecuteRequest>();
            hr->appId = decision->appId;
            hr->groupId = decision->groupId;
            hr->user = req->user;
            hr->function = req->function;
            hr->snapshotKey = req->snapshotKey;
            hr->type = req->type;
            hr->subType = req->subType;
            hr->contextData = req->contextData;
            hr->singleHost = isSingleHost;
            hr->singleHostHint = req->singleHostHint;
            hr->elasticScaleHint = req->elasticScaleHint;
        }
        hr->messages.push_back(req->messages[i]);
    }

    bool isThreads = req->type == BatchExecuteType::THREADS;
    for (auto& [host, hr] : hostReqs) {
        if (isThreads && !isSingleHost && !hr->messages.empty()) {
            const auto& m0 = hr->messages[0];
            std::string key =
              getMainThreadSnapshotKey(m0.user, m0.function, m0.appId);
            if (host != req->messages[0].mainHost) {
                try {
                    auto snap = SnapshotRegistry::get().getSnapshot(key);
                    getSnapshotClient(host)->pushSnapshot(key, *snap);
                } catch (const std::exception& e) {
                    FAM_ERROR("push of snapshot %s to %s failed: %s",
                              key.c_str(),
                              host.c_str(),
                              e.what());
                }
            }
        }
        if (!isThreads && !hr->messages.empty() &&
            !hr->messages[0].snapshotKey.empty()) {
            for (const auto& m : hr->messages) {
                try {
                    auto snap =
                      SnapshotRegistry::get().getSnapshot(m.snapshotKey);
                    getSnapshotClient(host)->pushSnapshot(m.snapshotKey,
                                                          *snap);
                } catch (const std::exception& e) {
                    FAM_ERROR("push of snapshot %s to %s failed: %s",
                              m.snapshotKey.c_str(),
                              host.c_str(),
                              e.what());
                }
            }
        }
        getFunctionCallClient(host)->executeFunctions(*hr);
    }
}

void Planner::preloadSchedulingDecision(
  int32_t appId,
  std::shared_ptr<SchedulingDecision> decision)
{
    std::unique_lock lock(plannerMx);
    if (state.preloadedSchedulingDecisions.count(appId) > 0) {
        FAM_ERROR("preloaded decision already exists for app %d", appId);
        return;
    }
    auto preload = std::make_shared<SchedulingDecision>(*decision);
    preload->groupId = FIXED_SIZE_PRELOADED_DECISION_GROUPID;
    state.preloadedSchedulingDecisions[appId] = preload;
}

std::shared_ptr<SchedulingDecision> Planner::getSchedulingDecision(
  int32_t appId)
{
    std::shared_lock lock(plannerMx);
    auto it = state.inFlightReqs.find(appId);
    if (it == state.inFlightReqs.end()) {
        return nullptr;
    }
    return std::make_shared<SchedulingDecision>(*it->second.second);
}


void Planner::setMessageResult(std::shared_ptr<Message> msg)
{
    std::vector<std::shared_ptr<Message>> one;
    one.push_back(std::move(msg));
    setMessageResults(one);
}

void Planner::setMessageResults(
  std::vector<std::shared_ptr<Message>>& msgs)
{
    std::vector<std::pair<std::string, std::shared_ptr<Message>>> waiters;
    std::vector<std::pair<std::string, int32_t>> batchWaiters;
    std::vector<std::pair<std::string, int32_t>> groupClears;
    {
        std::unique_lock lock(plannerMx);
        for (auto& msg : msgs) {
            setMessageResultLocked(msg, waiters, batchWaiters, groupClears);
        }
    }

    auto& broker = getPointToPointBroker();
    for (const auto& [host, groupId] : groupClears) {
        broker.sendGroupClear(host, groupId);
    }

    for (const auto& msg : msgs) {
        if (msg->returnValue != FROZEN_FUNCTION_RETURN_VALUE &&
            startsWith(msg->snapshotKey, "migration_")) {
            SnapshotRegistry::get().deleteSnapshot(msg->snapshotKey);
            DeviceSnapshotRegistry::get().deleteSnapshot(msg->snapshotKey);
        }
    }

    for (const auto& [host, appId] : batchWaiters) {
        try {
            getFunctionCallClient(host)->batchDone(appId);
        } catch (const std::exception& e) {
            FAM_ERROR(
              "batch-done push to %s failed: %s", host.c_str(), e.what());
        }
    }

    for (const auto& [host, msg] : waiters) {
        try {
            getFunctionCallClient(host)->setMessageResult(*msg);
        } catch (const std::exception& e) {
            FAM_ERROR("result push to %s failed: %s", host.c_str(), e.what());
        }
    }
}

void Planner::purgeOldResultsLocked()
{
    static const int64_t ttlMs =
      getEnvVarInt("FAABRIC_RESULT_TTL_MS", 5 * 60 * 1000);
    static const size_t maxDone =
      (size_t)getEnvVarInt("FAABRIC_MAX_DONE_APPS", 512);
    int64_t now = getGlobalClockEpochMillis();
    while (!state.doneApps.empty() &&
           (state.doneApps.size() > maxDone ||
            now - state.doneApps.front().first > ttlMs)) {
        int32_t appId = state.doneApps.front().second;
        state.doneApps.pop_front();
        if (state.inFlightReqs.count(appId) == 0) {
            state.appResults.erase(appId);
        }
    }
}

void Planner::setMessageResultLocked(
  const std::shared_ptr<Message>& msg,
  std::vector<std::pair<std::string, std::shared_ptr<Message>>>& waiters,
  std::vector<std::pair<std::string, int32_t>>& batchWaiters,
  std::vector<std::pair<std::string, int32_t>>& groupClears)
{
    int32_t appId = msg->appId;
    int32_t msgId = msg->id;

    if (msg->returnValue == MIGRATED_FUNCTION_RETURN_VALUE) {
        return;
    }
    {

        bool isFrozenMsg = msg->returnValue == FROZEN_FUNCTION_RETURN_VALUE;
        if (isFrozenMsg) {
            auto it = state.evictedRequests.find(appId);
            if (it == state.evictedRequests.end()) {
                FAM_ERROR("frozen message %d has no evicted app %d",
                          msgId,
                          appId);
            } else {
                for (auto& m : it->second->messages) {
                    if (m.id == msgId) {
                        m.funcPtr = msg->funcPtr;
                        m.inputData = msg->inputData;
                        m.snapshotKey = msg->snapshotKey;
                        m.returnValue = msg->returnValue;
                        break;
                    }
                }
            }
        }

        auto hostIt = state.hostMap.find(msg->executedHost);
        bool alreadySet = state.appResults[appId].count(msgId) > 0;
        if (hostIt != state.hostMap.end() && (!alreadySet || isFrozenMsg)) {
            hostIt->second->info.usedSlots =
              std::max(0, hostIt->second->info.usedSlots - 1);
        }

        if (!isFrozenMsg) {
            state.appResults[appId][msgId] = msg;
        }

        auto ifIt = state.inFlightReqs.find(appId);
        if (ifIt != state.inFlightReqs.end()) {
            auto req = ifIt->second.first;
            auto decision = ifIt->second.second;
            auto msgIt = std::find_if(
              req->messages.begin(),
              req->messages.end(),
              [&](const Message& m) { return m.id == msgId; });
            if (msgIt != req->messages.end()) {
                *msgIt = std::move(req->messages.back());
                req->messages.pop_back();
                int32_t freedPort = decision->removeMessage(msgId);
                if (hostIt != state.hostMap.end()) {
                    releaseHostMpiPort(hostIt->second, freedPort);
                }
                if (req->messages.empty()) {
                    state.inFlightReqs.erase(appId);
                    state.preloadedSchedulingDecisions.erase(appId);
                    auto bwIt = state.batchDoneWaiters.find(appId);
                    if (bwIt != state.batchDoneWaiters.end()) {
                        for (auto& h : bwIt->second) {
                            batchWaiters.emplace_back(std::move(h), appId);
                        }
                        state.batchDoneWaiters.erase(bwIt);
                    }
                    state.doneApps.emplace_back(
                      getGlobalClockEpochMillis(), appId);
                    purgeOldResultsLocked();
                    if (decision->groupId != 0) {
                        std::set<std::string> hosts(
                          decision->hosts.begin(), decision->hosts.end());
                        hosts.insert(getSystemConfig().endpointHost);
                        for (const auto& h : hosts) {
                            groupClears.emplace_back(h,
                                                     decision->groupId);
                        }
                    }
                    auto sgIt = state.supersededGroups.find(appId);
                    if (sgIt != state.supersededGroups.end()) {
                        for (auto& [gid, hosts] : sgIt->second) {
                            for (auto& h : hosts) {
                                groupClears.emplace_back(std::move(h),
                                                         gid);
                            }
                            groupClears.emplace_back(
                              getSystemConfig().endpointHost, gid);
                        }
                        state.supersededGroups.erase(sgIt);
                    }
                }
            }
        }

        if (isFrozenMsg) {
            return;
        }

        auto wIt = state.appResultWaiters.find(msgId);
        if (wIt != state.appResultWaiters.end()) {
            for (auto& h : wIt->second) {
                waiters.emplace_back(std::move(h), msg);
            }
            state.appResultWaiters.erase(wIt);
        }
    }
}

bool Planner::registerBatchDoneWaiter(int32_t appId,
                                      const std::string& host)
{
    std::unique_lock lock(plannerMx);
    if (state.inFlightReqs.count(appId) == 0) {
        return true;
    }
    state.batchDoneWaiters[appId].push_back(host);
    return false;
}

size_t Planner::debugAppResultsCount()
{
    std::shared_lock lock(plannerMx);
    size_t n = 0;
    for (const auto& [a, m] : state.appResults) {
        n += m.size();
    }
    return n;
}
size_t Planner::debugDoneAppsCount()
{
    std::shared_lock lock(plannerMx);
    return state.doneApps.size();
}
size_t Planner::debugInFlightCount()
{
    std::shared_lock lock(plannerMx);
    return state.inFlightReqs.size();
}

std::shared_ptr<Message> Planner::getMessageResult(const Message& msg)
{
    int32_t appId = msg.appId;
    int32_t msgId = msg.id;
    {
        std::shared_lock lock(plannerMx);
        auto appIt = state.appResults.find(appId);
        if (appIt != state.appResults.end()) {
            auto msgIt = appIt->second.find(msgId);
            if (msgIt != appIt->second.end()) {
                return msgIt->second;
            }
        }
    }
    if (!msg.mainHost.empty()) {
        std::unique_lock lock(plannerMx);
        auto appIt = state.appResults.find(appId);
        if (appIt != state.appResults.end() &&
            appIt->second.count(msgId) > 0) {
            return appIt->second.at(msgId);
        }
        state.appResultWaiters[msgId].push_back(msg.mainHost);
    }
    return nullptr;
}

std::shared_ptr<BatchExecuteRequestStatus> Planner::getBatchResults(
  int32_t appId)
{
    auto status = std::make_shared<BatchExecuteRequestStatus>();
    status->appId = appId;

    std::shared_ptr<BatchExecuteRequest> frozenBer;
    {
        std::shared_lock lock(plannerMx);
        auto evIt = state.evictedRequests.find(appId);
        if (evIt != state.evictedRequests.end()) {
            bool fullyFrozen = std::all_of(
              evIt->second->messages.begin(),
              evIt->second->messages.end(),
              [](const Message& m) {
                  return m.returnValue == FROZEN_FUNCTION_RETURN_VALUE;
              });
            if (fullyFrozen && state.inFlightReqs.count(appId) == 0) {
                frozenBer = std::make_shared<BatchExecuteRequest>(
                  *evIt->second);
            }
            if (!frozenBer) {
                status->finished = false;
                return status;
            }
        }
    }
    if (frozenBer) {
        for (auto& m : frozenBer->messages) {
            m.returnValue = 0;
            m.executedHost.clear();
            m.finishTimestamp = 0;
        }
        auto decision = callBatch(frozenBer);
        if (decision->appId == NOT_ENOUGH_SLOTS) {
            FAM_DEBUG("cannot un-freeze app %d yet: no slots", appId);
        }
        status->finished = false;
        return status;
    }

    std::shared_lock lock(plannerMx);
    auto it = state.appResults.find(appId);
    if (it == state.appResults.end()) {
        return nullptr;
    }
    for (const auto& [msgId, msg] : it->second) {
        status->messageResults.push_back(*msg);
    }
    status->finished = state.inFlightReqs.count(appId) == 0;
    return status;
}


int Planner::getNumMigrations()
{
    std::shared_lock lock(plannerMx);
    return state.numMigrations;
}

GetInFlightAppsResponse Planner::getInFlightApps()
{
    std::shared_lock lock(plannerMx);
    GetInFlightAppsResponse resp;
    for (const auto& [appId, pair] : state.inFlightReqs) {
        InFlightAppEntry e;
        e.appId = appId;
        e.subType = pair.first->subType;
        e.size = pair.second->nFunctions;
        e.hostIps = pair.second->hosts;
        resp.apps.push_back(std::move(e));
    }
    resp.numMigrations = state.numMigrations;
    for (const auto& ip : state.nextEvictedHostIps) {
        resp.nextEvictedVmIps.push_back(ip);
    }
    for (const auto& [appId, ber] : state.evictedRequests) {
        InFlightAppEntry e;
        e.appId = appId;
        e.subType = ber->subType;
        e.size = (int)ber->messages.size();
        resp.frozenApps.push_back(std::move(e));
    }
    return resp;
}

void Planner::setNextEvictedVm(const std::set<std::string>& vmIps)
{
    std::unique_lock lock(plannerMx);
    state.nextEvictedHostIps = vmIps;
}

void Planner::setPolicy(const std::string& policy)
{
    resetBatchScheduler(policy);
}

std::string Planner::getPolicy()
{
    return getBatchSchedulerMode();
}


void Planner::reset()
{
    std::unique_lock lock(plannerMx);
    state = PlannerState();
}

void Planner::flushSchedulingState()
{
    std::unique_lock lock(plannerMx);
    state.inFlightReqs.clear();
    state.appResults.clear();
    state.appResultWaiters.clear();
    state.preloadedSchedulingDecisions.clear();
    state.evictedRequests.clear();
    state.numMigrations = 0;
    for (auto& [ip, h] : state.hostMap) {
        h->info.usedSlots = 0;
        std::fill(h->mpiPortUsed.begin(), h->mpiPortUsed.end(), false);
    }
}

void Planner::flushExecutors()
{
    std::vector<std::string> hosts;
    {
        std::shared_lock lock(plannerMx);
        for (const auto& [ip, h] : state.hostMap) {
            hosts.push_back(ip);
        }
    }
    for (const auto& host : hosts) {
        try {
            getFunctionCallClient(host)->sendFlush();
        } catch (const std::exception& e) {
            FAM_ERROR("flush of %s failed: %s", host.c_str(), e.what());
        }
    }
}

void Planner::flushHosts()
{
    std::unique_lock lock(plannerMx);
    state.hostMap.clear();
}


PlannerServer::PlannerServer()
  : MessageEndpointServer(PLANNER_ASYNC_PORT, PLANNER_SYNC_PORT, "planner")
{
    const int nResultWorkers = getEnvVarInt("FAABRIC_RESULT_WORKERS", 4);
    for (int i = 0; i < nResultWorkers; i++) {
        resultWorkers.emplace_back([this] { resultWorkerLoop(); });
    }
}

PlannerServer::~PlannerServer()
{
    resultWorkersStop.store(true);
    for (size_t i = 0; i < resultWorkers.size(); i++) {
        resultQueue.enqueue(std::string());
    }
    for (auto& t : resultWorkers) {
        if (t.joinable()) {
            t.join();
        }
    }
}

void PlannerServer::resultWorkerLoop()
{
    while (true) {
        std::string body;
        try {
            body = resultQueue.dequeue(0);
        } catch (...) {
            continue;
        }
        if (resultWorkersStop.load()) {
            return;
        }
        if (body.empty()) {
            continue;
        }
        try {
            char tag = body[0];
            std::string_view payload(body.data() + 1, body.size() - 1);
            if (tag == 'B') {
                PROF_START(result_decode)
                std::vector<std::shared_ptr<Message>> msgs;
                std::string payloadStr(payload);
                PbReader r(payloadStr);
                uint32_t f;
                WireType t;
                while (r.next(f, t)) {
                    if (f != 1) {
                        r.skip(t);
                        continue;
                    }
                    auto sub = r.asString();
                    msgs.push_back(
                      std::make_shared<Message>(Message::decode(sub)));
                }
                PROF_END(result_decode)
                PROF_START(result_core)
                Planner::get().setMessageResults(msgs);
                PROF_END(result_core)
            } else {
                PROF_START(result_decode)
                auto msg = std::make_shared<Message>(
                  Message::decode(std::string(payload)));
                PROF_END(result_decode)
                PROF_START(result_core)
                Planner::get().setMessageResult(msg);
                PROF_END(result_core)
            }
        } catch (const std::exception& e) {
            FAM_ERROR("result ingestion failed: %s", e.what());
        }
    }
}

void PlannerServer::doAsyncRecv(uint8_t code,
                                const std::string& body,
                                uint32_t seq)
{
    (void)seq;
    if ((PlannerCalls)code == PlannerCalls::SetMessageResult) {
        if (resultWorkers.empty()) {
            auto msg = std::make_shared<Message>(Message::decode(body));
            Planner::get().setMessageResult(msg);
        } else {
            resultQueue.enqueue("S" + body);
        }
        return;
    }
    if ((PlannerCalls)code == PlannerCalls::SetMessageResultBatch) {
        if (resultWorkers.empty()) {
            std::vector<std::shared_ptr<Message>> msgs;
            PbReader r(body);
            uint32_t f;
            WireType t;
            while (r.next(f, t)) {
                if (f != 1) {
                    r.skip(t);
                    continue;
                }
                msgs.push_back(std::make_shared<Message>(
                  Message::decode(r.asString())));
            }
            Planner::get().setMessageResults(msgs);
        } else {
            resultQueue.enqueue("B" + body);
        }
        return;
    }
    FAM_ERROR("planner server: bad async code %d", (int)code);
}

std::string PlannerServer::doSyncRecv(uint8_t code, const std::string& body)
{
    auto& planner = Planner::get();
    switch ((PlannerCalls)code) {
        case PlannerCalls::Ping: {
            PbWriter w;
            w.putMessage(1, planner.getConfig().encode());
            return w.take();
        }
        case PlannerCalls::GetAvailableHosts: {
            AvailableHostsResponse resp;
            resp.hosts = planner.getAvailableHosts();
            return resp.encode();
        }
        case PlannerCalls::RegisterHost: {
            auto req = RegisterHostRequest::decode(body);
            bool ok = planner.registerHost(req.host, req.overwrite);
            RegisterHostResponse resp;
            resp.status = ok ? 0 : 1;
            resp.config = planner.getConfig();
            return resp.encode();
        }
        case PlannerCalls::RemoveHost: {
            auto req = RegisterHostRequest::decode(body);
            planner.removeHost(req.host);
            return {};
        }
        case PlannerCalls::WaitBatchDone: {
            PbReader r(body);
            int32_t appId = 0;
            std::string host;
            uint32_t f;
            WireType t;
            while (r.next(f, t)) {
                if (f == 1) {
                    appId = r.asInt32();
                } else if (f == 2) {
                    host = r.asString();
                } else {
                    r.skip(t);
                }
            }
            bool done = planner.registerBatchDoneWaiter(appId, host);
            PbWriter w;
            w.putBool(1, done);
            return w.take();
        }
        case PlannerCalls::SetMessageResult: {
            auto msg = std::make_shared<Message>(Message::decode(body));
            planner.setMessageResult(msg);
            return {};
        }
        case PlannerCalls::GetMessageResult: {
            Message query = Message::decode(body);
            auto result = planner.getMessageResult(query);
            if (!result) {
                Message empty;
                empty.type = MessageType::EMPTY;
                return empty.encode();
            }
            return result->encode();
        }
        case PlannerCalls::GetBatchResults: {
            BatchExecuteRequest req = BatchExecuteRequest::decode(body);
            auto status = planner.getBatchResults(req.appId);
            if (!status) {
                BatchExecuteRequestStatus empty;
                empty.appId = req.appId;
                empty.expectedNumMessages = -1;
                return empty.encode();
            }
            if (req.subType == 1) {
                BatchExecuteRequestStatus counts;
                counts.appId = status->appId;
                counts.finished = status->finished;
                counts.expectedNumMessages =
                  (int32_t)status->messageResults.size();
                return counts.encode();
            }
            return status->encode();
        }
        case PlannerCalls::GetSchedulingDecision: {
            BatchExecuteRequest req = BatchExecuteRequest::decode(body);
            auto decision = planner.getSchedulingDecision(req.appId);
            if (!decision) {
                return PointToPointMappings{}.encode();
            }
            return decision->toPointToPointMappings().encode();
        }
        case PlannerCalls::GetNumMigrations: {
            PbWriter w;
            w.putInt32(1, planner.getNumMigrations());
            return w.take();
        }
        case PlannerCalls::CallBatch: {
            auto req = std::make_shared<BatchExecuteRequest>(
              BatchExecuteRequest::decode(body));
            auto decision = planner.callBatch(req);
            PointToPointMappings out = decision->toPointToPointMappings();
            out.appId = decision->appId;
            out.groupId = decision->groupId;
            return out.encode();
        }
        case PlannerCalls::PreloadSchedulingDecision: {
            auto mappings = PointToPointMappings::decode(body);
            auto decision = std::make_shared<SchedulingDecision>(
              SchedulingDecision::fromPointToPointMappings(mappings));
            planner.preloadSchedulingDecision(mappings.appId, decision);
            return {};
        }
        default:
            throw FaabricException("planner server: bad sync code " +
                                   std::to_string(code));
    }
}


class PlannerClient::KeepAliveThread : public PeriodicBackgroundThread
{
  public:
    void doWork() override
    {
        Host host;
        host.ip = getSystemConfig().endpointHost;
        host.slots = Scheduler::get().getThisHostResources().slots;
        getPlannerClient().registerHost(host, false);
    }
};

PlannerClient::PlannerClient()
  : rpc(getSystemConfig().plannerHost, PLANNER_ASYNC_PORT, PLANNER_SYNC_PORT)
{}

PlannerClient::~PlannerClient()
{
    stopKeepAlive();
}

void PlannerClient::ping()
{
    rpc.syncSend((uint8_t)PlannerCalls::Ping, "");
}

std::vector<Host> PlannerClient::getAvailableHosts()
{
    std::string resp =
      rpc.syncSend((uint8_t)PlannerCalls::GetAvailableHosts, "");
    return AvailableHostsResponse::decode(resp).hosts;
}

int32_t PlannerClient::registerHost(const Host& host, bool overwrite)
{
    RegisterHostRequest req;
    req.host = host;
    req.overwrite = overwrite;
    std::string resp =
      rpc.syncSend((uint8_t)PlannerCalls::RegisterHost, req.encode());
    auto r = RegisterHostResponse::decode(resp);
    if (r.status != 0) {
        throw FaabricException("planner rejected host registration");
    }
    return r.hostId;
}

void PlannerClient::removeHost(const Host& host)
{
    RegisterHostRequest req;
    req.host = host;
    rpc.syncSend((uint8_t)PlannerCalls::RemoveHost, req.encode());
}

std::shared_ptr<SchedulingDecision> PlannerClient::callFunctions(
  std::shared_ptr<BatchExecuteRequest> req)
{
    std::string resp =
      rpc.syncSend((uint8_t)PlannerCalls::CallBatch, req->encode());
    auto mappings = PointToPointMappings::decode(resp);
    auto decision = std::make_shared<SchedulingDecision>(
      SchedulingDecision::fromPointToPointMappings(mappings));
    decision->appId = mappings.appId;
    decision->groupId = mappings.groupId;
    return decision;
}

void PlannerClient::setMessageResult(std::shared_ptr<Message> msg)
{
    if (isMockMode()) {
        return;
    }
    rpc.asyncSend((uint8_t)PlannerCalls::SetMessageResult, msg->encode());
}

void PlannerClient::setMessageResultsBatch(
  const std::vector<std::shared_ptr<Message>>& msgs)
{
    if (isMockMode() || msgs.empty()) {
        return;
    }
    if (msgs.size() == 1) {
        setMessageResult(msgs[0]);
        return;
    }
    PbWriter w;
    for (const auto& m : msgs) {
        w.putMessage(1, m->encode());
    }
    rpc.asyncSend((uint8_t)PlannerCalls::SetMessageResultBatch, w.take());
}

void PlannerClient::setMessageResultLocally(std::shared_ptr<Message> msg)
{
    {
        std::lock_guard<std::mutex> lock(resultsMx);
        localResults[msg->id] = msg;
    }
    resultsCv.notify_all();
}

Message PlannerClient::getMessageResult(const Message& msg, int timeoutMs)
{
    return getMessageResult(msg.appId, msg.id, timeoutMs);
}

Message PlannerClient::getMessageResult(int32_t appId,
                                        int32_t msgId,
                                        int timeoutMs)
{
    int64_t deadline = getGlobalClockEpochMillis() + timeoutMs;
    int64_t nextRpcAt = 0;
    while (true) {
        {
            std::unique_lock<std::mutex> lock(resultsMx);
            auto it = localResults.find(msgId);
            if (it != localResults.end()) {
                Message out = *it->second;
                localResults.erase(it);
                return out;
            }
        }

        int64_t now = getGlobalClockEpochMillis();
        if (now >= deadline) {
            throw QueueTimeoutException("timed out waiting for result of " +
                                        std::to_string(msgId));
        }

        if (now >= nextRpcAt) {
            Message query;
            query.appId = appId;
            query.id = msgId;
            query.mainHost = getSystemConfig().endpointHost;
            std::string resp = rpc.syncSend(
              (uint8_t)PlannerCalls::GetMessageResult, query.encode());
            Message result = Message::decode(resp);
            if (!(result.type == MessageType::EMPTY && result.id == 0)) {
                return result;
            }
            nextRpcAt = now + 2000;
        }

        std::unique_lock<std::mutex> lock(resultsMx);
        resultsCv.wait_for(lock, std::chrono::milliseconds(50), [&] {
            return localResults.count(msgId) > 0;
        });
    }
}

BatchExecuteRequestStatus PlannerClient::getBatchResults(int32_t appId)
{
    BatchExecuteRequest req;
    req.appId = appId;
    std::string resp =
      rpc.syncSend((uint8_t)PlannerCalls::GetBatchResults, req.encode());
    return BatchExecuteRequestStatus::decode(resp);
}

std::pair<bool, int> PlannerClient::getBatchStatusCounts(int32_t appId)
{
    BatchExecuteRequest req;
    req.appId = appId;
    req.subType = 1;
    std::string resp =
      rpc.syncSend((uint8_t)PlannerCalls::GetBatchResults, req.encode());
    auto status = BatchExecuteRequestStatus::decode(resp);
    if (status.expectedNumMessages == -1) {
        return { false, -1 };
    }
    return { status.finished, status.expectedNumMessages };
}

bool PlannerClient::waitBatchDone(int32_t appId, int timeoutMs)
{
    if (!functionCallServerRunning()) {
        auto deadline = std::chrono::steady_clock::now() +
                        std::chrono::milliseconds(timeoutMs);
        int sleepUs = 200;
        while (std::chrono::steady_clock::now() < deadline) {
            auto [finished, n] = getBatchStatusCounts(appId);
            (void)n;
            if (finished) {
                return true;
            }
            std::this_thread::sleep_for(std::chrono::microseconds(sleepUs));
            sleepUs = std::min(sleepUs * 2, 20000);
        }
        return false;
    }

    auto waiter = batchDoneWaiterPrepare(appId);

    PbWriter w;
    w.putInt32(1, appId);
    w.putString(2, getSystemConfig().endpointHost);
    std::string resp =
      rpc.syncSend((uint8_t)PlannerCalls::WaitBatchDone, w.take());
    bool already = false;
    {
        PbReader r(resp);
        uint32_t f;
        WireType t;
        while (r.next(f, t)) {
            if (f == 1) {
                already = r.asBool();
            } else {
                r.skip(t);
            }
        }
    }
    if (already) {
        batchDoneWaiterDiscard(appId);
        return true;
    }

    auto deadline = std::chrono::steady_clock::now() +
                    std::chrono::milliseconds(timeoutMs);
    bool done = false;
    while (!done) {
        if (waiter->isSet()) {
            done = true;
            break;
        }
        if (std::chrono::steady_clock::now() > deadline) {
            break;
        }
        if (waiter->waitMs(500)) {
            done = true;
            break;
        }
        auto [finished, n] = getBatchStatusCounts(appId);
        (void)n;
        if (finished) {
            done = true;
            break;
        }
    }
    batchDoneWaiterDiscard(appId);
    return done;
}

SchedulingDecision PlannerClient::getSchedulingDecision(int32_t appId)
{
    BatchExecuteRequest req;
    req.appId = appId;
    std::string resp = rpc.syncSend(
      (uint8_t)PlannerCalls::GetSchedulingDecision, req.encode());
    return SchedulingDecision::fromPointToPointMappings(
      PointToPointMappings::decode(resp));
}

void PlannerClient::preloadSchedulingDecision(
  int32_t appId,
  const SchedulingDecision& decision)
{
    PointToPointMappings mappings = decision.toPointToPointMappings();
    mappings.appId = appId;
    rpc.syncSend((uint8_t)PlannerCalls::PreloadSchedulingDecision,
                 mappings.encode());
}

int PlannerClient::getNumMigrations()
{
    std::string resp =
      rpc.syncSend((uint8_t)PlannerCalls::GetNumMigrations, "");
    PbReader r(resp);
    uint32_t f;
    WireType t;
    while (r.next(f, t)) {
        if (f == 1) {
            return r.asInt32();
        }
        r.skip(t);
    }
    return 0;
}

void PlannerClient::startKeepAlive()
{
    if (!keepAlive) {
        keepAlive = std::make_shared<KeepAliveThread>();
        keepAlive->startMillis(
          std::max(500, Planner::get().hostTimeoutMs / 2));
    }
}

void PlannerClient::stopKeepAlive()
{
    if (keepAlive) {
        keepAlive->stop();
        keepAlive = nullptr;
    }
}

void PlannerClient::clearCache()
{
    std::lock_guard<std::mutex> lock(resultsMx);
    localResults.clear();
}

static std::shared_ptr<PlannerClient> plannerClientInstance;
static std::mutex plannerClientMx;

PlannerClient& getPlannerClient()
{
    std::lock_guard<std::mutex> lock(plannerClientMx);
    if (!plannerClientInstance) {
        plannerClientInstance = std::make_shared<PlannerClient>();
    }
    return *plannerClientInstance;
}

void resetPlannerClient()
{
    std::lock_guard<std::mutex> lock(plannerClientMx);
    plannerClientInstance = nullptr;
}

}
```

### cpp/src/scheduler.cpp

```cpp
#include "faabricamd/scheduler.h"
#include "faabricamd/utilextras.h"

#include <atomic>
#include <thread>
#include <functional>
#include <condition_variable>
#include "faabricamd/planner.h"
#include "faabricamd/ptp.h"
#include "faabricamd/util.h"
#include "faabricamd/wire.h"

#include <hip/hip_runtime.h>

namespace faabricamd {

static int getNumGpus()
{
    static int n = []() {
        const auto& conf = getSystemConfig();
        if (conf.overrideGpuCount >= 0) {
            return conf.overrideGpuCount;
        }
        if (!conf.useGpu) {
            return 0;
        }
        int count = 0;
        if (hipGetDeviceCount(&count) != hipSuccess) {
            return 0;
        }
        return count;
    }();
    return n;
}

class Scheduler::ReaperThread : public PeriodicBackgroundThread
{
  public:
    void doWork() override { Scheduler::get().reapStaleExecutors(); }
};

namespace {

class DispatchPool
{
  public:
    static constexpr int N = 7;

    int run(const std::function<void()>& fn)
    {
        std::lock_guard<std::mutex> lock(mx);
        ensureStarted();
        current = fn;
        generation++;
        cv.notify_all();
        return N;
    }

    void awaitDone(std::atomic<int>& done, int target)
    {
        while (done.load(std::memory_order_acquire) < target) {
            std::this_thread::yield();
        }
        std::lock_guard<std::mutex> lock(mx);
        current = nullptr;
    }

  private:
    void ensureStarted()
    {
        if (started) {
            return;
        }
        started = true;
        for (int i = 0; i < N; i++) {
            workers.emplace_back([this] { loop(); });
            workers.back().detach();
        }
    }

    void loop()
    {
        uint64_t seen = 0;
        while (true) {
            std::function<void()> fn;
            {
                std::unique_lock<std::mutex> lock(mx);
                cv.wait(lock, [&] {
                    return generation != seen && current != nullptr;
                });
                seen = generation;
                fn = current;
            }
            fn();
        }
    }

    std::mutex mx;
    std::condition_variable cv;
    std::vector<std::thread> workers;
    std::function<void()> current;
    uint64_t generation = 0;
    bool started = false;
};

DispatchPool& dispatchPool()
{
    static DispatchPool* pool = new DispatchPool();
    return *pool;
}

}

Scheduler::Scheduler() = default;

Scheduler& Scheduler::get()
{
    static Scheduler sched;
    return sched;
}

HostResources Scheduler::getThisHostResources()
{
    {
        std::unique_lock<std::shared_mutex> lock(schedMx);
        if (resourcesOverridden) {
            return overriddenResources;
        }
    }
    HostResources res;
    int nGpus = getNumGpus();
    res.slots = nGpus > 0 ? nGpus : getUsableCores();
    res.usedSlots = 0;
    return res;
}

void Scheduler::setThisHostResources(const HostResources& res)
{
    std::unique_lock<std::shared_mutex> lock(schedMx);
    overriddenResources = res;
    resourcesOverridden = true;
}

void Scheduler::executeBatch(std::shared_ptr<BatchExecuteRequest> req)
{
    if (req->messages.empty()) {
        return;
    }
    PROF_START(sched_execute_batch)
    bool isThreads = req->type == BatchExecuteType::THREADS;

    if (isTestMode()) {
        std::unique_lock<std::shared_mutex> lock(schedMx);
        for (const auto& msg : req->messages) {
            recordedMessages.push_back(msg);
        }
    }

    if (isThreads) {
        auto exec = claimExecutor(req->messages[0]);
        std::vector<int> idxs(req->messages.size());
        for (size_t i = 0; i < idxs.size(); i++) {
            idxs[i] = (int)i;
        }
        exec->executeTasks(idxs, req);
    } else {
        size_t n = req->messages.size();
        auto dispatchOne = [&](size_t i) {
            try {
                PROF_START(dispatch_claim)
                auto exec = claimExecutor(req->messages[i]);
                PROF_END(dispatch_claim)
                PROF_START(dispatch_enqueue)
                exec->executeTasks({ (int)i }, req);
                PROF_END(dispatch_enqueue)
            } catch (const std::exception& e) {
                FAM_ERROR("claiming executor failed: %s", e.what());
                auto msg = std::make_shared<Message>(req->messages[i]);
                msg->returnValue = 1;
                msg->executedHost = getSystemConfig().endpointHost;
                msg->outputData = std::string("executor claim failed: ") +
                                  e.what();
                getPlannerClient().setMessageResult(msg);
            }
        };
        if (n < 32) {
            for (size_t i = 0; i < n; i++) {
                dispatchOne(i);
            }
        } else {
            static std::mutex fanMx;
            std::lock_guard<std::mutex> fanLock(fanMx);
            std::atomic<size_t> next{ 0 };
            std::atomic<int> done{ 0 };
            auto work = [&] {
                size_t i;
                while ((i = next.fetch_add(1)) < n) {
                    dispatchOne(i);
                }
                done.fetch_add(1, std::memory_order_acq_rel);
            };
            int helpers = dispatchPool().run(work);
            work();
            dispatchPool().awaitDone(done, helpers + 1);
        }
    }
    PROF_END(sched_execute_batch)
}

std::shared_ptr<Executor> Scheduler::claimExecutor(Message& msg)
{
    std::string key = msg.user + "/" + msg.function;

    {
        std::shared_lock<std::shared_mutex> rlock(schedMx);
        auto it = executors.find(key);
        if (it != executors.end()) {
            auto& pool = *it->second;
            size_t n = pool.list.size();
            if (n > 0) {
                size_t start =
                  pool.hint.fetch_add(1, std::memory_order_relaxed);
                for (size_t k = 0; k < n; k++) {
                    size_t i = (start + k) % n;
                    if (pool.list[i]->tryClaim()) {
                        return pool.list[i];
                    }
                }
            }
        }
    }

    std::unique_lock<std::shared_mutex> lock(schedMx);
    auto& poolPtr = executors[key];
    if (!poolPtr) {
        poolPtr = std::make_unique<WarmPool>();
    }
    auto& pool = *poolPtr;
    for (auto& e : pool.list) {
        if (e->tryClaim()) {
            return e;
        }
    }
    auto exec = getExecutorFactory()->createExecutor(msg);
    exec->claim();
    if (getNumGpus() > 0) {
        const auto& conf = getSystemConfig();
        exec->gpuDevice =
          conf.gpuDevicePinned
            ? conf.gpuDevice
            : (int)((pool.list.size()) % (size_t)getNumGpus());
    }
    pool.list.push_back(exec);
    return exec;
}

int Scheduler::reapStaleExecutors()
{
    std::unique_lock<std::shared_mutex> lock(schedMx);
    const auto& conf = getSystemConfig();
    int reaped = 0;
    for (auto& [key, pool] : executors) {
        auto& list = pool->list;
        for (auto it = list.begin(); it != list.end();) {
            auto& exec = *it;
            if (!exec->isClaimed() &&
                exec->getMillisSinceLastExec() > conf.boundTimeout) {
                exec->shutdown();
                it = list.erase(it);
                reaped++;
            } else {
                ++it;
            }
        }
    }
    return reaped;
}

void Scheduler::startReaper()
{
    if (!reaper) {
        reaper = std::make_shared<ReaperThread>();
        reaper->startMillis(getSystemConfig().boundTimeout);
    }
}

void Scheduler::stopReaper()
{
    if (reaper) {
        reaper->stop();
        reaper = nullptr;
    }
}

std::shared_ptr<PendingMigration> Scheduler::checkForMigrationOpportunities(
  Message& msg,
  int32_t overwriteNewGroupId)
{
    int32_t newGroupId = 0;
    if (msg.groupIdx == 0 && overwriteNewGroupId == 0) {
        auto req = std::make_shared<BatchExecuteRequest>();
        req->appId = msg.appId;
        req->groupId = msg.groupId;
        req->user = msg.user;
        req->function = msg.function;
        req->type = BatchExecuteType::MIGRATION;
        auto decision = getPlannerClient().callFunctions(req);
        if (decision->appId == DO_NOT_MIGRATE) {
            newGroupId = 0;
        } else if (decision->appId == MUST_FREEZE) {
            newGroupId = MUST_FREEZE;
        } else {
            newGroupId = decision->groupId;
        }
        auto& broker = getPointToPointBroker();
        int32_t payload = newGroupId;
        for (int i = 1; i < msg.groupSize; i++) {
            broker.sendMessage(msg.appId,
                               msg.groupId,
                               PTP_MIGRATION_CHANNEL_OFFSET,
                               i,
                               (const uint8_t*)&payload,
                               sizeof(payload));
        }
    } else if (overwriteNewGroupId != 0) {
        newGroupId = overwriteNewGroupId;
    } else {
        auto data = getPointToPointBroker().recvMessage(
          msg.groupId, PTP_MIGRATION_CHANNEL_OFFSET, msg.groupIdx);
        newGroupId = *(const int32_t*)data.data();
    }

    if (newGroupId == 0) {
        return nullptr;
    }

    auto migration = std::make_shared<PendingMigration>();
    migration->appId = msg.appId;
    migration->groupIdx = msg.groupIdx;
    migration->srcHost = getSystemConfig().endpointHost;

    if (newGroupId == MUST_FREEZE) {
        migration->appId = MUST_FREEZE;
        return migration;
    }

    migration->groupId = newGroupId;
    auto decision = getPlannerClient().getSchedulingDecision(msg.appId);
    for (int i = 0; i < decision.nFunctions; i++) {
        if (decision.groupIdxs[i] == msg.groupIdx) {
            migration->dstHost = decision.hosts[i];
            break;
        }
    }
    return migration;
}

void Scheduler::flushLocally()
{
    std::unique_lock<std::shared_mutex> lock(schedMx);
    for (auto& [key, pool] : executors) {
        for (auto& e : pool->list) {
            e->flush();
        }
    }
    executors.clear();
    getExecutorFactory()->flushHost();
}

void Scheduler::shutdown()
{
    stopReaper();
    std::unique_lock<std::shared_mutex> lock(schedMx);
    for (auto& [key, pool] : executors) {
        for (auto& e : pool->list) {
            e->shutdown();
        }
    }
    executors.clear();
}

void Scheduler::reset()
{
    shutdown();
    std::unique_lock<std::shared_mutex> lock(schedMx);
    recordedMessages.clear();
    resourcesOverridden = false;
}

std::vector<Message> Scheduler::getRecordedMessages()
{
    std::unique_lock<std::shared_mutex> lock(schedMx);
    return recordedMessages;
}

void Scheduler::clearRecordedMessages()
{
    std::unique_lock<std::shared_mutex> lock(schedMx);
    recordedMessages.clear();
}

size_t Scheduler::getExecutorCount()
{
    std::unique_lock<std::shared_mutex> lock(schedMx);
    size_t n = 0;
    for (auto& [key, pool] : executors) {
        n += pool->list.size();
    }
    return n;
}


static std::atomic<int> fnServersUp{ 0 };

bool functionCallServerRunning()
{
    return fnServersUp.load(std::memory_order_relaxed) > 0;
}

FunctionCallServer::FunctionCallServer()
  : MessageEndpointServer(FUNCTION_CALL_ASYNC_PORT,
                          FUNCTION_CALL_SYNC_PORT,
                          "function-call")
{
    fnServersUp.fetch_add(1, std::memory_order_relaxed);
}

FunctionCallServer::~FunctionCallServer()
{
    fnServersUp.fetch_sub(1, std::memory_order_relaxed);
}


static std::mutex batchDoneMx;
static std::map<int32_t, std::shared_ptr<FlagWaiter>> batchDoneFlags;

std::shared_ptr<FlagWaiter> batchDoneWaiterPrepare(int32_t appId)
{
    std::lock_guard<std::mutex> lock(batchDoneMx);
    auto& w = batchDoneFlags[appId];
    if (!w) {
        w = std::make_shared<FlagWaiter>();
    }
    return w;
}

void batchDoneWaiterDiscard(int32_t appId)
{
    std::lock_guard<std::mutex> lock(batchDoneMx);
    batchDoneFlags.erase(appId);
}

void signalBatchDone(int32_t appId)
{
    std::shared_ptr<FlagWaiter> w;
    {
        std::lock_guard<std::mutex> lock(batchDoneMx);
        auto it = batchDoneFlags.find(appId);
        if (it == batchDoneFlags.end()) {
            return;
        }
        w = it->second;
    }
    w->setFlag(true);
}

void FunctionCallServer::doAsyncRecv(uint8_t code,
                                     const std::string& body,
                                     uint32_t seq)
{
    (void)seq;
    switch ((FunctionCalls)code) {
        case FunctionCalls::ExecuteFunctions: {
            auto req = std::make_shared<BatchExecuteRequest>(
              BatchExecuteRequest::decode(body));
            Scheduler::get().executeBatch(req);
            break;
        }
        case FunctionCalls::SetMessageResult: {
            auto msg = std::make_shared<Message>(Message::decode(body));
            getPlannerClient().setMessageResultLocally(msg);
            break;
        }
        case FunctionCalls::BatchDone: {
            PbReader r(body);
            int32_t appId = 0;
            uint32_t f;
            WireType t;
            while (r.next(f, t)) {
                if (f == 1) {
                    appId = (int32_t)r.varint();
                } else {
                    r.skip(t);
                }
            }
            signalBatchDone(appId);
            break;
        }
        default:
            FAM_ERROR("function call server: bad async code %d", (int)code);
    }
}

std::string FunctionCallServer::doSyncRecv(uint8_t code,
                                           const std::string& body)
{
    (void)body;
    if ((FunctionCalls)code == FunctionCalls::Flush) {
        Scheduler::get().flushLocally();
        return {};
    }
    throw FaabricException("function call server: bad sync code " +
                           std::to_string(code));
}

FunctionCallClient::FunctionCallClient(const std::string& host)
  : MessageEndpointClient(host,
                          FUNCTION_CALL_ASYNC_PORT,
                          FUNCTION_CALL_SYNC_PORT)
{}

static std::mutex mockMx;
static std::vector<std::pair<std::string, BatchExecuteRequest>>
  mockedBatchRequests;

std::vector<std::pair<std::string, BatchExecuteRequest>>
getBatchRequestsSentMock()
{
    std::lock_guard<std::mutex> lock(mockMx);
    return mockedBatchRequests;
}

void clearMockedFunctionCalls()
{
    std::lock_guard<std::mutex> lock(mockMx);
    mockedBatchRequests.clear();
}

void FunctionCallClient::executeFunctions(const BatchExecuteRequest& req)
{
    if (isMockMode()) {
        std::lock_guard<std::mutex> lock(mockMx);
        mockedBatchRequests.emplace_back(getHost(), req);
        return;
    }
    asyncSend((uint8_t)FunctionCalls::ExecuteFunctions, req.encode());
}

void FunctionCallClient::setMessageResult(const Message& msg)
{
    if (isMockMode()) {
        return;
    }
    asyncSend((uint8_t)FunctionCalls::SetMessageResult, msg.encode());
}

void FunctionCallClient::batchDone(int32_t appId)
{
    if (isMockMode()) {
        return;
    }
    PbWriter w;
    w.putInt32(1, appId);
    std::string body = w.take();
    asyncSend((uint8_t)FunctionCalls::BatchDone, body.data(), body.size());
}

void FunctionCallClient::sendFlush()
{
    syncSend((uint8_t)FunctionCalls::Flush, "");
}

static std::mutex fcClientsMx;
static std::map<std::string, std::shared_ptr<FunctionCallClient>> fcClients;

std::shared_ptr<FunctionCallClient> getFunctionCallClient(
  const std::string& host)
{
    std::lock_guard<std::mutex> lock(fcClientsMx);
    auto& cli = fcClients[host];
    if (!cli) {
        cli = std::make_shared<FunctionCallClient>(host);
    }
    return cli;
}

void clearFunctionCallClients()
{
    std::lock_guard<std::mutex> lock(fcClientsMx);
    fcClients.clear();
}

}
```

### cpp/src/utilextras.cpp

```cpp
#include "faabricamd/utilextras.h"
#include "faabricamd/util.h"

#include <atomic>
#include <chrono>
#include <csignal>
#include <cstring>
#include <execinfo.h>
#include <map>
#include <mutex>
#include <pthread.h>
#include <sched.h>
#include <sstream>
#include <thread>
#include <zlib.h>

namespace faabricamd {


enum DeltaCmd : uint8_t
{
    DELTA_TOTAL_SIZE = 1,
    DELTA_XOR_PAGE = 2,
    DELTA_RAW_RANGE = 3,
    DELTA_COMPRESSED = 4,
    DELTA_COMPRESSED_ZSTD = 5,
    DELTA_END = 0xff,
};

extern "C" {
size_t ZSTD_compressBound(size_t srcSize);
size_t ZSTD_compress(void* dst,
                     size_t dstCapacity,
                     const void* src,
                     size_t srcSize,
                     int level);
size_t ZSTD_decompress(void* dst,
                       size_t dstCapacity,
                       const void* src,
                       size_t srcSize);
unsigned ZSTD_isError(size_t code);
}
static constexpr uint8_t DELTA_VERSION = 1;

DeltaConfig DeltaConfig::parse(const std::string& s)
{
    DeltaConfig conf;
    conf.xorWithOld = s.find("xor") != std::string::npos;
    conf.compress = s.find("zlib=1") != std::string::npos ||
                    s.find("zstd=1") != std::string::npos;
    conf.useZstd = s.find("zlib=1") == std::string::npos;
    auto pos = s.find("pages=");
    if (pos != std::string::npos) {
        conf.pageSize = (size_t)atoll(s.c_str() + pos + 6);
    }
    return conf;
}

std::string DeltaConfig::str() const
{
    std::string out = "pages=" + std::to_string(pageSize);
    if (xorWithOld) {
        out += ";xor";
    }
    if (compress) {
        out += useZstd ? ";zstd=1" : ";zlib=1";
    }
    return out;
}

static void putU64(std::vector<uint8_t>& out, uint64_t v)
{
    for (int i = 0; i < 8; i++) {
        out.push_back((uint8_t)(v >> (8 * i)));
    }
}

static uint64_t getU64(const uint8_t* p)
{
    uint64_t v = 0;
    for (int i = 0; i < 8; i++) {
        v |= (uint64_t)p[i] << (8 * i);
    }
    return v;
}

static std::vector<uint8_t> zlibCompress(const uint8_t* data, size_t n)
{
    uLongf bound = compressBound((uLong)n);
    std::vector<uint8_t> out(bound);
    if (compress2(out.data(), &bound, data, (uLong)n, Z_BEST_SPEED) !=
        Z_OK) {
        throw FaabricException("zlib compress failed");
    }
    out.resize(bound);
    return out;
}

static std::vector<uint8_t> zlibDecompress(const uint8_t* data,
                                           size_t n,
                                           size_t expected)
{
    std::vector<uint8_t> out(expected);
    uLongf outLen = (uLongf)expected;
    if (uncompress(out.data(), &outLen, data, (uLong)n) != Z_OK) {
        throw FaabricException("zlib decompress failed");
    }
    out.resize(outLen);
    return out;
}

std::vector<uint8_t> deltaEncode(const std::vector<uint8_t>& oldData,
                                 const std::vector<uint8_t>& newData,
                                 const DeltaConfig& conf)
{
    std::vector<uint8_t> cmds;
    cmds.push_back(DELTA_TOTAL_SIZE);
    putU64(cmds, newData.size());

    size_t common = std::min(oldData.size(), newData.size());
    size_t page = conf.pageSize;

    for (size_t off = 0; off < common; off += page) {
        size_t len = std::min(page, common - off);
        if (std::memcmp(oldData.data() + off, newData.data() + off, len) ==
            0) {
            continue;
        }
        if (conf.xorWithOld) {
            cmds.push_back(DELTA_XOR_PAGE);
            putU64(cmds, off);
            putU64(cmds, len);
            size_t base = cmds.size();
            cmds.resize(base + len);
            for (size_t i = 0; i < len; i++) {
                cmds[base + i] = oldData[off + i] ^ newData[off + i];
            }
        } else {
            cmds.push_back(DELTA_RAW_RANGE);
            putU64(cmds, off);
            putU64(cmds, len);
            cmds.insert(cmds.end(),
                        newData.begin() + off,
                        newData.begin() + off + len);
        }
    }
    if (newData.size() > common) {
        cmds.push_back(DELTA_RAW_RANGE);
        putU64(cmds, common);
        putU64(cmds, newData.size() - common);
        cmds.insert(cmds.end(), newData.begin() + common, newData.end());
    }
    cmds.push_back(DELTA_END);

    std::vector<uint8_t> out;
    out.push_back(DELTA_VERSION);
    if (conf.compress && conf.useZstd) {
        size_t bound = ZSTD_compressBound(cmds.size());
        std::vector<uint8_t> compressed(bound);
        size_t n = ZSTD_compress(compressed.data(), bound, cmds.data(),
                                 cmds.size(), 1);
        if (ZSTD_isError(n)) {
            throw FaabricException("zstd compress failed");
        }
        compressed.resize(n);
        out.push_back(DELTA_COMPRESSED_ZSTD);
        putU64(out, cmds.size());
        putU64(out, compressed.size());
        out.insert(out.end(), compressed.begin(), compressed.end());
    } else if (conf.compress) {
        auto compressed = zlibCompress(cmds.data(), cmds.size());
        out.push_back(DELTA_COMPRESSED);
        putU64(out, cmds.size());
        putU64(out, compressed.size());
        out.insert(out.end(), compressed.begin(), compressed.end());
    } else {
        out.insert(out.end(), cmds.begin(), cmds.end());
    }
    return out;
}

std::vector<uint8_t> deltaApply(const std::vector<uint8_t>& oldData,
                                const std::vector<uint8_t>& delta)
{
    if (delta.empty() || delta[0] != DELTA_VERSION) {
        throw FaabricException("bad delta version");
    }
    std::vector<uint8_t> cmds;
    size_t pos = 1;
    if (pos < delta.size() && delta[pos] == DELTA_COMPRESSED_ZSTD) {
        uint64_t rawLen = getU64(delta.data() + pos + 1);
        uint64_t compLen = getU64(delta.data() + pos + 9);
        cmds.resize(rawLen);
        size_t n = ZSTD_decompress(cmds.data(), rawLen,
                                   delta.data() + pos + 17, compLen);
        if (ZSTD_isError(n) || n != rawLen) {
            throw FaabricException("zstd decompress failed");
        }
    } else if (pos < delta.size() && delta[pos] == DELTA_COMPRESSED) {
        uint64_t rawLen = getU64(delta.data() + pos + 1);
        uint64_t compLen = getU64(delta.data() + pos + 9);
        cmds = zlibDecompress(delta.data() + pos + 17, compLen, rawLen);
    } else {
        cmds.assign(delta.begin() + 1, delta.end());
    }

    std::vector<uint8_t> out = oldData;
    size_t p = 0;
    while (p < cmds.size()) {
        uint8_t cmd = cmds[p++];
        if (cmd == DELTA_END) {
            break;
        }
        switch (cmd) {
            case DELTA_TOTAL_SIZE: {
                uint64_t total = getU64(cmds.data() + p);
                p += 8;
                out.resize(total, 0);
                break;
            }
            case DELTA_XOR_PAGE: {
                uint64_t off = getU64(cmds.data() + p);
                uint64_t len = getU64(cmds.data() + p + 8);
                p += 16;
                for (uint64_t i = 0; i < len; i++) {
                    out[off + i] ^= cmds[p + i];
                }
                p += len;
                break;
            }
            case DELTA_RAW_RANGE: {
                uint64_t off = getU64(cmds.data() + p);
                uint64_t len = getU64(cmds.data() + p + 8);
                p += 16;
                std::memcpy(out.data() + off, cmds.data() + p, len);
                p += len;
                break;
            }
            default:
                throw FaabricException("bad delta command");
        }
    }
    return out;
}


namespace {
struct ProfState
{
    std::mutex mx;
    std::map<std::string, double> totalsMs;
    std::map<std::string, int64_t> counts;
};
ProfState& profState()
{
    static ProfState st;
    return st;
}
thread_local std::map<std::string, std::chrono::steady_clock::time_point>
  profStarts;
}

static bool profEnabled()
{
    static const bool v = getEnvVarInt("FAABRIC_PROF", 0) != 0;
    return v;
}

void profStart(const std::string& name)
{
    if (!profEnabled()) {
        return;
    }
    profStarts[name] = std::chrono::steady_clock::now();
}

void profEnd(const std::string& name)
{
    if (!profEnabled()) {
        return;
    }
    auto it = profStarts.find(name);
    if (it == profStarts.end()) {
        return;
    }
    double ms = std::chrono::duration<double, std::milli>(
                  std::chrono::steady_clock::now() - it->second)
                  .count();
    profStarts.erase(it);
    auto& st = profState();
    std::lock_guard<std::mutex> lock(st.mx);
    st.totalsMs[name] += ms;
    st.counts[name] += 1;
}

std::vector<std::pair<std::string, double>> profTotalsMs()
{
    auto& st = profState();
    std::lock_guard<std::mutex> lock(st.mx);
    return { st.totalsMs.begin(), st.totalsMs.end() };
}

void profClear()
{
    auto& st = profState();
    std::lock_guard<std::mutex> lock(st.mx);
    st.totalsMs.clear();
    st.counts.clear();
}

std::string profSummary()
{
    auto& st = profState();
    std::lock_guard<std::mutex> lock(st.mx);
    std::ostringstream out;
    out << "--- PROF totals ---\n";
    for (const auto& [name, ms] : st.totalsMs) {
        out << name << ": " << ms << " ms (" << st.counts[name]
            << " calls)\n";
    }
    return out.str();
}


static void crashHandler(int sig)
{
    void* frames[64];
    int n = backtrace(frames, 64);
    fprintf(stderr, "--- crash: signal %d (%s) ---\n", sig,
            strsignal(sig));
    backtrace_symbols_fd(frames, n, 2);
    signal(sig, SIG_DFL);
    raise(sig);
}

void setUpCrashHandler()
{
    signal(SIGABRT, crashHandler);
    signal(SIGILL, crashHandler);
    signal(SIGFPE, crashHandler);
}


namespace {
std::mutex pinMx;
std::vector<bool> pinnedCores;
thread_local int myPinnedCore = -1;
}

int pinThreadToFreeCpu()
{
    int nCores = (int)std::thread::hardware_concurrency();
    std::lock_guard<std::mutex> lock(pinMx);
    if ((int)pinnedCores.size() != nCores) {
        pinnedCores.assign(nCores, false);
    }
    for (int i = 0; i < nCores; i++) {
        if (!pinnedCores[i]) {
            cpu_set_t set;
            CPU_ZERO(&set);
            CPU_SET(i, &set);
            if (pthread_setaffinity_np(pthread_self(), sizeof(set), &set) ==
                0) {
                pinnedCores[i] = true;
                myPinnedCore = i;
                return i;
            }
        }
    }
    return -1;
}

void unpinThisThread()
{
    std::lock_guard<std::mutex> lock(pinMx);
    if (myPinnedCore >= 0 && myPinnedCore < (int)pinnedCores.size()) {
        pinnedCores[myPinnedCore] = false;
        myPinnedCore = -1;
    }
}

}
```

Measured before the change: 169,800 msgs/sec.

## Replace executor queues with futex mailboxes and idle-list executor claiming

Replaces the per-thread task Queue with a lock-free slot mailbox that uses futex wait/wake, and adds a single-task fast path that posts directly to pool thread 0. Executor claiming now pops from a per-function idle list instead of scanning the whole warm pool, and batches claim all executors up front. The planner gains a per-app message position index so removals avoid linear searches, and the PROF macros check the enabled flag before building strings. This targets the batch-exec dispatch overhead, at the cost of more intricate concurrency: the idle list must stay consistent with the claim flags, and reaping now goes through tryClaim.

New measurement: 200,500 msgs/sec, median of 6. +18.1%, better.

```diff
diff --git a/cpp/bindings/bindings_runtime.cpp b/cpp/bindings/bindings_runtime.cpp
--- a/cpp/bindings/bindings_runtime.cpp
+++ b/cpp/bindings/bindings_runtime.cpp
@@ -864,6 +864,21 @@
         d["broker_send_seqs"] = getPointToPointBroker().debugSendSeqsCount();
         d["decision_cache"] = DecisionCache::get().size();
         return d;
+    });
+    m.def("_debug_dispatch_sizes", [] {
+        py::dict d;
+        d["idle_executors"] = Scheduler::get().debugIdleCount();
+        d["planner_msg_index_apps"] = Planner::get().debugMsgIndexCount();
+        d["planner_used_slots"] = Planner::get().debugUsedSlots();
+        return d;
+    });
+    m.def("_debug_current_executor_id", [] {
+        return ExecutorContext::get().getExecutor()->id;
+    });
+    m.def("_debug_set_message_result", [](const Message& msg) {
+        auto copy = std::make_shared<Message>(msg);
+        py::gil_scoped_release release;
+        getPlannerClient().setMessageResult(copy);
     });
     m.def("_debug_kv_commit_stats", [] {
         KvCommitStats s = kvCommitStats();
diff --git a/cpp/include/faabricamd/executor.h b/cpp/include/faabricamd/executor.h
--- a/cpp/include/faabricamd/executor.h
+++ b/cpp/include/faabricamd/executor.h
@@ -7,6 +7,7 @@
 #include <thread>
 #include <vector>
 
+#include "faabricamd/mailbox.h"
 #include "faabricamd/messages.h"
 #include "faabricamd/queue.h"
 #include "faabricamd/dirty.h"
@@ -71,16 +72,20 @@
     int msgIdx = 0;
     std::shared_ptr<BatchExecuteRequest> req;
     bool stop = false;
+    bool single = false;
+    int64_t enqueueNs = 0;
 };
 
-class Executor
+class Executor : public std::enable_shared_from_this<Executor>
 {
   public:
     explicit Executor(Message& msg);
     virtual ~Executor();
 
-    void executeTasks(std::vector<int> msgIdxs,
-                      std::shared_ptr<BatchExecuteRequest> req);
+    void executeTasks(const std::vector<int>& msgIdxs,
+                      const std::shared_ptr<BatchExecuteRequest>& req);
+    void executeSingleTask(int msgIdx,
+                           const std::shared_ptr<BatchExecuteRequest>& req);
 
     std::vector<std::pair<int32_t, int32_t>> executeThreads(
       std::shared_ptr<BatchExecuteRequest> req,
@@ -103,6 +108,11 @@
     void claim();
     void releaseClaim();
     bool isClaimed() const { return claimed.load(); }
+    using IdleExecutors = IdleList<std::shared_ptr<Executor>>;
+    void setIdleList(std::shared_ptr<IdleExecutors> list)
+    {
+        idleList = std::move(list);
+    }
 
     long getMillisSinceLastExec() const;
     void shutdown();
@@ -124,9 +134,15 @@
                           bool isLastInBatch);
 
     int threadPoolSize = 0;
-    std::vector<std::shared_ptr<Queue<ExecutorTask>>> threadTaskQueues;
+    using TaskMailbox = Mailbox<ExecutorTask>;
+    std::vector<std::unique_ptr<TaskMailbox>> threadMailboxes;
     std::vector<std::thread> threadPoolThreads;
+    std::unique_ptr<std::atomic<bool>[]> poolThreadUp;
     std::mutex threadsMx;
+    void ensurePoolThreadLocked(int poolIdx);
+    void postTask(int poolIdx, ExecutorTask&& task);
+
+    std::shared_ptr<IdleExecutors> idleList;
 
     std::atomic<bool> claimed{ false };
     std::atomic<int64_t> lastExecMs{ 0 };
diff --git a/cpp/include/faabricamd/mailbox.h b/cpp/include/faabricamd/mailbox.h
--- /dev/null
+++ b/cpp/include/faabricamd/mailbox.h
@@ -0,0 +1,211 @@
+#pragma once
+
+#include <atomic>
+#include <climits>
+#include <cstddef>
+#include <cstdint>
+#include <ctime>
+#include <mutex>
+#include <utility>
+#include <vector>
+
+#include <linux/futex.h>
+#include <sys/syscall.h>
+#include <unistd.h>
+
+namespace faabricamd {
+
+namespace detail {
+
+inline void futexWait(std::atomic<uint32_t>* word,
+                      uint32_t expected,
+                      int timeoutMs)
+{
+    static_assert(sizeof(std::atomic<uint32_t>) == sizeof(uint32_t));
+    struct timespec ts;
+    struct timespec* tsp = nullptr;
+    if (timeoutMs > 0) {
+        ts.tv_sec = timeoutMs / 1000;
+        ts.tv_nsec = (long)(timeoutMs % 1000) * 1000000L;
+        tsp = &ts;
+    }
+    syscall(SYS_futex,
+            reinterpret_cast<uint32_t*>(word),
+            FUTEX_WAIT_PRIVATE,
+            expected,
+            tsp,
+            nullptr,
+            0);
+}
+
+inline void futexWake(std::atomic<uint32_t>* word, int n)
+{
+    syscall(SYS_futex,
+            reinterpret_cast<uint32_t*>(word),
+            FUTEX_WAKE_PRIVATE,
+            n,
+            nullptr,
+            nullptr,
+            0);
+}
+
+}
+
+template<typename T, uint32_t SLOTS = 8>
+class Mailbox
+{
+    static_assert(SLOTS >= 2 && (SLOTS & (SLOTS - 1)) == 0,
+                  "SLOTS must be a power of two");
+
+  public:
+    Mailbox()
+    {
+        for (uint32_t i = 0; i < SLOTS; i++) {
+            slots[i].seq.store(i, std::memory_order_relaxed);
+        }
+    }
+    Mailbox(const Mailbox&) = delete;
+    Mailbox& operator=(const Mailbox&) = delete;
+
+    void post(T value)
+    {
+        uint32_t ticket = tail.fetch_add(1, std::memory_order_relaxed);
+        Slot& s = slots[ticket & (SLOTS - 1)];
+        uint32_t seen;
+        while ((seen = s.seq.load(std::memory_order_acquire)) != ticket) {
+            detail::futexWait(&s.seq, seen, 1);
+        }
+        s.value = std::move(value);
+        s.seq.store(ticket + 1, std::memory_order_seq_cst);
+        if (sleeping.load(std::memory_order_seq_cst) != 0) {
+            detail::futexWake(&s.seq, INT_MAX);
+        }
+    }
+
+    bool take(T& out, int timeoutMs)
+    {
+        Slot& s = slots[head & (SLOTS - 1)];
+        uint32_t ready = head + 1;
+        uint32_t seen = s.seq.load(std::memory_order_acquire);
+        if (seen != ready) {
+            struct timespec start;
+            clock_gettime(CLOCK_MONOTONIC, &start);
+            int leftMs = timeoutMs;
+            while (true) {
+                sleeping.store(1, std::memory_order_seq_cst);
+                seen = s.seq.load(std::memory_order_seq_cst);
+                if (seen != ready) {
+                    detail::futexWait(&s.seq, seen, leftMs);
+                    seen = s.seq.load(std::memory_order_acquire);
+                }
+                sleeping.store(0, std::memory_order_relaxed);
+                if (seen == ready) {
+                    break;
+                }
+                if (timeoutMs > 0) {
+                    struct timespec now;
+                    clock_gettime(CLOCK_MONOTONIC, &now);
+                    int64_t goneMs =
+                      (int64_t)(now.tv_sec - start.tv_sec) * 1000 +
+                      (now.tv_nsec - start.tv_nsec) / 1000000;
+                    if (goneMs >= timeoutMs) {
+                        return false;
+                    }
+                    leftMs = (int)(timeoutMs - goneMs);
+                }
+            }
+        }
+        out = std::move(s.value);
+        s.value = T();
+        s.seq.store(head + SLOTS, std::memory_order_release);
+        head++;
+        return true;
+    }
+
+  private:
+    struct alignas(64) Slot
+    {
+        std::atomic<uint32_t> seq{ 0 };
+        T value{};
+    };
+    Slot slots[SLOTS];
+    alignas(64) std::atomic<uint32_t> tail{ 0 };
+    std::atomic<uint32_t> sleeping{ 0 };
+    alignas(64) uint32_t head = 0;
+};
+
+template<typename T>
+class IdleList
+{
+  public:
+    void push(T value)
+    {
+        std::lock_guard<std::mutex> lock(mx);
+        if (!closed) {
+            entries.push_back(std::move(value));
+        }
+    }
+
+    size_t popMany(size_t n, std::vector<T>& out)
+    {
+        std::lock_guard<std::mutex> lock(mx);
+        size_t got = 0;
+        while (got < n && !entries.empty()) {
+            out.push_back(std::move(entries.back()));
+            entries.pop_back();
+            got++;
+        }
+        return got;
+    }
+
+    bool pop(T& out)
+    {
+        std::lock_guard<std::mutex> lock(mx);
+        if (entries.empty()) {
+            return false;
+        }
+        out = std::move(entries.back());
+        entries.pop_back();
+        return true;
+    }
+
+    size_t remove(const T& value)
+    {
+        std::lock_guard<std::mutex> lock(mx);
+        size_t before = entries.size();
+        size_t w = 0;
+        for (size_t r = 0; r < entries.size(); r++) {
+            if (!(entries[r] == value)) {
+                if (w != r) {
+                    entries[w] = std::move(entries[r]);
+                }
+                w++;
+            }
+        }
+        entries.resize(w);
+        return before - w;
+    }
+
+    void close()
+    {
+        std::vector<T> dropped;
+        {
+            std::lock_guard<std::mutex> lock(mx);
+            closed = true;
+            dropped.swap(entries);
+        }
+    }
+
+    size_t size()
+    {
+        std::lock_guard<std::mutex> lock(mx);
+        return entries.size();
+    }
+
+  private:
+    std::mutex mx;
+    std::vector<T> entries;
+    bool closed = false;
+};
+
+}
diff --git a/cpp/include/faabricamd/planner.h b/cpp/include/faabricamd/planner.h
--- a/cpp/include/faabricamd/planner.h
+++ b/cpp/include/faabricamd/planner.h
@@ -7,6 +7,7 @@
 #include <set>
 #include <shared_mutex>
 #include <thread>
+#include <unordered_map>
 #include <vector>
 
 #include "faabricamd/messages.h"
@@ -46,6 +47,8 @@
 {
     std::map<std::string, std::shared_ptr<PlannerHost>> hostMap;
     InFlightReqs inFlightReqs;
+    std::unordered_map<int32_t, std::unordered_map<int32_t, uint32_t>>
+      inFlightMsgPos;
     std::map<int32_t, std::shared_ptr<SchedulingDecision>>
       preloadedSchedulingDecisions;
     std::map<int32_t, std::map<int32_t, std::shared_ptr<Message>>> appResults;
@@ -75,6 +78,8 @@
     size_t debugAppResultsCount();
     size_t debugDoneAppsCount();
     size_t debugInFlightCount();
+    size_t debugMsgIndexCount();
+    int debugUsedSlots();
 
     bool registerBatchDoneWaiter(int32_t appId, const std::string& host);
 
@@ -107,6 +112,9 @@
 
   private:
     void purgeOldResultsLocked();
+    int64_t findInFlightPosLocked(int32_t appId,
+                                  const BatchExecuteRequest& req,
+                                  int32_t msgId);
     void setMessageResultLocked(
       const std::shared_ptr<Message>& msg,
       std::vector<std::pair<std::string, std::shared_ptr<Message>>>& waiters,
diff --git a/cpp/include/faabricamd/scheduler.h b/cpp/include/faabricamd/scheduler.h
--- a/cpp/include/faabricamd/scheduler.h
+++ b/cpp/include/faabricamd/scheduler.h
@@ -47,18 +47,26 @@
     void clearRecordedMessages();
 
     size_t getExecutorCount();
+    size_t debugIdleCount();
 
   private:
     Scheduler();
 
-    std::shared_ptr<Executor> claimExecutor(Message& msg);
-
-    std::shared_mutex schedMx;
     struct WarmPool
     {
         std::vector<std::shared_ptr<Executor>> list;
-        std::atomic<size_t> hint{ 0 };
+        std::shared_ptr<Executor::IdleExecutors> idle =
+          std::make_shared<Executor::IdleExecutors>();
     };
+
+    std::shared_ptr<Executor> claimExecutor(Message& msg);
+    void claimExecutors(BatchExecuteRequest& req,
+                        std::vector<std::shared_ptr<Executor>>& execs,
+                        std::vector<std::string>& errors);
+    std::shared_ptr<Executor> createExecutorLocked(WarmPool& pool,
+                                                   Message& msg);
+
+    std::shared_mutex schedMx;
     std::unordered_map<std::string, std::unique_ptr<WarmPool>> executors;
     HostResources overriddenResources;
     bool resourcesOverridden = false;
diff --git a/cpp/include/faabricamd/scheduling.h b/cpp/include/faabricamd/scheduling.h
--- a/cpp/include/faabricamd/scheduling.h
+++ b/cpp/include/faabricamd/scheduling.h
@@ -68,6 +68,7 @@
                               int32_t groupIdx,
                               int32_t mpiPort);
     int32_t removeMessage(int32_t messageId);
+    int32_t removeMessageAt(size_t pos, int32_t messageId);
     std::set<std::string> uniqueHosts() const;
     void print() const;
 };
diff --git a/cpp/include/faabricamd/utilextras.h b/cpp/include/faabricamd/utilextras.h
--- a/cpp/include/faabricamd/utilextras.h
+++ b/cpp/include/faabricamd/utilextras.h
@@ -28,12 +28,42 @@
 
 void profStart(const std::string& name);
 void profEnd(const std::string& name);
+bool profEnabled();
+int64_t profNowNs();
+void profRecord(const char* name, double ms);
 std::vector<std::pair<std::string, double>> profTotalsMs();
 void profClear();
 std::string profSummary();
 
-#define PROF_START(name) ::faabricamd::profStart(#name);
-#define PROF_END(name) ::faabricamd::profEnd(#name);
+#define PROF_START(name)                                                       \
+    if (::faabricamd::profEnabled()) {                                         \
+        ::faabricamd::profStart(#name);                                        \
+    }
+#define PROF_END(name)                                                         \
+    if (::faabricamd::profEnabled()) {                                         \
+        ::faabricamd::profEnd(#name);                                          \
+    }
+
+class ProfScope
+{
+  public:
+    explicit ProfScope(const char* nameIn)
+      : name(nameIn)
+      , startNs(profEnabled() ? profNowNs() : 0)
+    {}
+    ~ProfScope()
+    {
+        if (startNs != 0) {
+            profRecord(name, (double)(profNowNs() - startNs) / 1e6);
+        }
+    }
+    ProfScope(const ProfScope&) = delete;
+    ProfScope& operator=(const ProfScope&) = delete;
+
+  private:
+    const char* name;
+    int64_t startNs;
+};
 
 void setUpCrashHandler();
 
diff --git a/cpp/src/batchsched.cpp b/cpp/src/batchsched.cpp
--- a/cpp/src/batchsched.cpp
+++ b/cpp/src/batchsched.cpp
@@ -91,7 +91,15 @@
     if (it == messageIds.end()) {
         return 0;
     }
-    size_t idx = (size_t)std::distance(messageIds.begin(), it);
+    return removeMessageAt((size_t)std::distance(messageIds.begin(), it),
+                           messageId);
+}
+
+int32_t SchedulingDecision::removeMessageAt(size_t idx, int32_t messageId)
+{
+    if (idx >= messageIds.size() || messageIds[idx] != messageId) {
+        return removeMessage(messageId);
+    }
     int32_t port = mpiPorts[idx];
     nFunctions--;
     size_t last = messageIds.size() - 1;
diff --git a/cpp/src/executor.cpp b/cpp/src/executor.cpp
--- a/cpp/src/executor.cpp
+++ b/cpp/src/executor.cpp
@@ -88,11 +88,12 @@
   , boundMsg(msg)
 {
     threadPoolSize = std::min(getUsableCores(), 64);
-    threadTaskQueues.resize(threadPoolSize);
-    for (auto& q : threadTaskQueues) {
-        q = std::make_shared<Queue<ExecutorTask>>();
-    }
+    threadMailboxes.resize(threadPoolSize);
     threadPoolThreads.resize(threadPoolSize);
+    poolThreadUp = std::make_unique<std::atomic<bool>[]>(threadPoolSize);
+    for (int i = 0; i < threadPoolSize; i++) {
+        poolThreadUp[i].store(false, std::memory_order_relaxed);
+    }
     lastExecMs = getGlobalClockEpochMillis();
 }
 
@@ -167,12 +168,13 @@
         if (threadPoolThreads[i].joinable()) {
             ExecutorTask stopTask;
             stopTask.stop = true;
-            threadTaskQueues[i]->enqueue(stopTask);
-        }
-    }
-    for (auto& t : threadPoolThreads) {
-        if (t.joinable()) {
-            t.join();
+            threadMailboxes[i]->post(std::move(stopTask));
+        }
+    }
+    for (int i = 0; i < threadPoolSize; i++) {
+        if (threadPoolThreads[i].joinable()) {
+            threadPoolThreads[i].join();
+            poolThreadUp[i].store(false, std::memory_order_release);
         }
     }
 }
@@ -196,10 +198,53 @@
 void Executor::releaseClaim()
 {
     claimed.store(false);
-}
-
-void Executor::executeTasks(std::vector<int> msgIdxs,
-                            std::shared_ptr<BatchExecuteRequest> req)
+    if (idleList) {
+        idleList->push(shared_from_this());
+    }
+}
+
+void Executor::ensurePoolThreadLocked(int poolIdx)
+{
+    if (threadPoolThreads[poolIdx].joinable()) {
+        return;
+    }
+    if (!threadMailboxes[poolIdx]) {
+        threadMailboxes[poolIdx] = std::make_unique<TaskMailbox>();
+    }
+    threadPoolThreads[poolIdx] =
+      std::thread([this, poolIdx] { threadPoolThread(poolIdx); });
+    poolThreadUp[poolIdx].store(true, std::memory_order_release);
+}
+
+void Executor::postTask(int poolIdx, ExecutorTask&& task)
+{
+    task.enqueueNs = profEnabled() ? profNowNs() : 0;
+    threadMailboxes[poolIdx]->post(std::move(task));
+}
+
+void Executor::executeSingleTask(
+  int msgIdx,
+  const std::shared_ptr<BatchExecuteRequest>& req)
+{
+    if (req->type == BatchExecuteType::THREADS ||
+        !req->snapshotKey.empty() ||
+        !req->messages.at(msgIdx).snapshotKey.empty() ||
+        threadPoolSize == 0) {
+        executeTasks({ msgIdx }, req);
+        return;
+    }
+    lastExecMs = getGlobalClockEpochMillis();
+    if (!poolThreadUp[0].load(std::memory_order_acquire)) {
+        std::lock_guard<std::mutex> lock(threadsMx);
+        ensurePoolThreadLocked(0);
+    }
+    ExecutorTask task(msgIdx, req);
+    task.single = true;
+    postTask(0, std::move(task));
+}
+
+void Executor::executeTasks(const std::vector<int>& msgIdxs,
+                            const std::shared_ptr<BatchExecuteRequest>& req)
 {
     lastExecMs = getGlobalClockEpochMillis();
     batchCounter = std::make_shared<std::atomic<int>>((int)msgIdxs.size());
@@ -231,11 +276,8 @@
     std::lock_guard<std::mutex> lock(threadsMx);
     for (int msgIdx : msgIdxs) {
         int poolIdx = threadPoolSize == 0 ? 0 : msgIdx % threadPoolSize;
-        if (!threadPoolThreads[poolIdx].joinable()) {
-            threadPoolThreads[poolIdx] =
-              std::thread([this, poolIdx] { threadPoolThread(poolIdx); });
-        }
-        threadTaskQueues[poolIdx]->enqueue(ExecutorTask(msgIdx, req));
+        ensurePoolThreadLocked(poolIdx);
+        postTask(poolIdx, ExecutorTask(msgIdx, req));
     }
 }
 
@@ -452,15 +494,18 @@
 void Executor::threadPoolThread(int poolIdx)
 {
     const auto& conf = getSystemConfig();
+    TaskMailbox& mailbox = *threadMailboxes[poolIdx];
     while (true) {
         ExecutorTask task;
-        try {
-            task = threadTaskQueues[poolIdx]->dequeue(conf.boundTimeout);
-        } catch (const QueueTimeoutException&) {
+        if (!mailbox.take(task, conf.boundTimeout)) {
             continue;
         }
         if (task.stop) {
             break;
+        }
+        if (task.enqueueNs != 0) {
+            profRecord("exec_wake",
+                       (double)(profNowNs() - task.enqueueNs) / 1e6);
         }
 
         Message& msg = task.req->messages.at(task.msgIdx);
@@ -492,8 +537,8 @@
         }
         ExecutorContext::unset();
 
-        int remaining = batchCounter->fetch_sub(1) - 1;
-        bool isLastInBatch = remaining == 0;
+        bool isLastInBatch =
+          task.single || batchCounter->fetch_sub(1) - 1 == 0;
         handleTaskResult(msg, returnValue, task.req, isLastInBatch);
     }
 }
diff --git a/cpp/src/planner.cpp b/cpp/src/planner.cpp
--- a/cpp/src/planner.cpp
+++ b/cpp/src/planner.cpp
@@ -144,6 +144,7 @@
 std::shared_ptr<SchedulingDecision> Planner::callBatch(
   std::shared_ptr<BatchExecuteRequest> req)
 {
+    ProfScope profCallBatch("planner_call_batch");
     int32_t appId = req->appId;
     std::unique_lock lock(plannerMx);
 
@@ -399,6 +400,7 @@
   std::shared_ptr<BatchExecuteRequest> req,
   std::shared_ptr<SchedulingDecision> decision)
 {
+    ProfScope profDispatch("planner_dispatch");
     std::map<std::string, std::shared_ptr<BatchExecuteRequest>> hostReqs;
     bool isSingleHost = decision->uniqueHosts().size() == 1;
 
@@ -501,6 +503,7 @@
     std::vector<std::pair<std::string, int32_t>> groupClears;
     {
         std::unique_lock lock(plannerMx);
+        ProfScope profLocked("results_locked");
         for (auto& msg : msgs) {
             setMessageResultLocked(msg, waiters, batchWaiters, groupClears);
         }
@@ -553,6 +556,42 @@
             state.appResults.erase(appId);
         }
     }
+}
+
+int64_t Planner::findInFlightPosLocked(int32_t appId,
+                                       const BatchExecuteRequest& req,
+                                       int32_t msgId)
+{
+    auto& index = state.inFlightMsgPos[appId];
+    const auto& messages = req.messages;
+    auto lookup = [&]() -> int64_t {
+        if (index.size() != messages.size()) {
+            return -2;
+        }
+        auto it = index.find(msgId);
+        if (it == index.end()) {
+            return -1;
+        }
+        if (it->second >= messages.size() ||
+            messages[it->second].id != msgId) {
+            return -2;
+        }
+        return (int64_t)it->second;
+    };
+    int64_t pos = lookup();
+    if (pos != -2) {
+        return pos;
+    }
+    index.clear();
+    index.reserve(messages.size());
+    pos = -1;
+    for (size_t i = 0; i < messages.size(); i++) {
+        index.emplace(messages[i].id, (uint32_t)i);
+        if (pos < 0 && messages[i].id == msgId) {
+            pos = (int64_t)i;
+        }
+    }
+    return pos;
 }
 
 void Planner::setMessageResultLocked(
@@ -590,33 +629,44 @@
         }
 
         auto hostIt = state.hostMap.find(msg->executedHost);
-        bool alreadySet = state.appResults[appId].count(msgId) > 0;
+        auto& appResults = state.appResults[appId];
+        auto resultIt = appResults.find(msgId);
+        bool alreadySet = resultIt != appResults.end();
         if (hostIt != state.hostMap.end() && (!alreadySet || isFrozenMsg)) {
             hostIt->second->info.usedSlots =
               std::max(0, hostIt->second->info.usedSlots - 1);
         }
 
         if (!isFrozenMsg) {
-            state.appResults[appId][msgId] = msg;
+            if (alreadySet) {
+                resultIt->second = msg;
+            } else {
+                appResults.emplace_hint(appResults.end(), msgId, msg);
+            }
         }
 
         auto ifIt = state.inFlightReqs.find(appId);
         if (ifIt != state.inFlightReqs.end()) {
             auto req = ifIt->second.first;
             auto decision = ifIt->second.second;
-            auto msgIt = std::find_if(
-              req->messages.begin(),
-              req->messages.end(),
-              [&](const Message& m) { return m.id == msgId; });
-            if (msgIt != req->messages.end()) {
-                *msgIt = std::move(req->messages.back());
+            int64_t pos = findInFlightPosLocked(appId, *req, msgId);
+            if (pos >= 0) {
+                auto& index = state.inFlightMsgPos[appId];
+                size_t last = req->messages.size() - 1;
+                if ((size_t)pos != last) {
+                    req->messages[pos] = std::move(req->messages[last]);
+                    index[req->messages[pos].id] = (uint32_t)pos;
+                }
                 req->messages.pop_back();
-                int32_t freedPort = decision->removeMessage(msgId);
+                index.erase(msgId);
+                int32_t freedPort =
+                  decision->removeMessageAt((size_t)pos, msgId);
                 if (hostIt != state.hostMap.end()) {
                     releaseHostMpiPort(hostIt->second, freedPort);
                 }
                 if (req->messages.empty()) {
                     state.inFlightReqs.erase(appId);
+                    state.inFlightMsgPos.erase(appId);
                     state.preloadedSchedulingDecisions.erase(appId);
                     auto bwIt = state.batchDoneWaiters.find(appId);
                     if (bwIt != state.batchDoneWaiters.end()) {
@@ -697,6 +747,20 @@
     std::shared_lock lock(plannerMx);
     return state.inFlightReqs.size();
 }
+size_t Planner::debugMsgIndexCount()
+{
+    std::shared_lock lock(plannerMx);
+    return state.inFlightMsgPos.size();
+}
+int Planner::debugUsedSlots()
+{
+    std::shared_lock lock(plannerMx);
+    int used = 0;
+    for (const auto& [ip, host] : state.hostMap) {
+        used += host->info.usedSlots;
+    }
+    return used;
+}
 
 std::shared_ptr<Message> Planner::getMessageResult(const Message& msg)
 {
@@ -837,6 +901,7 @@
 {
     std::unique_lock lock(plannerMx);
     state.inFlightReqs.clear();
+    state.inFlightMsgPos.clear();
     state.appResults.clear();
     state.appResultWaiters.clear();
     state.preloadedSchedulingDecisions.clear();
@@ -1159,6 +1224,7 @@
 std::shared_ptr<SchedulingDecision> PlannerClient::callFunctions(
   std::shared_ptr<BatchExecuteRequest> req)
 {
+    ProfScope profSubmit("submit_rpc");
     std::string resp =
       rpc.syncSend((uint8_t)PlannerCalls::CallBatch, req->encode());
     auto mappings = PointToPointMappings::decode(resp);
@@ -1277,6 +1343,7 @@
 
 bool PlannerClient::waitBatchDone(int32_t appId, int timeoutMs)
 {
+    ProfScope profWait("wait_batch_done");
     if (!functionCallServerRunning()) {
         auto deadline = std::chrono::steady_clock::now() +
                         std::chrono::milliseconds(timeoutMs);
diff --git a/cpp/src/scheduler.cpp b/cpp/src/scheduler.cpp
--- a/cpp/src/scheduler.cpp
+++ b/cpp/src/scheduler.cpp
@@ -39,78 +39,6 @@
     void doWork() override { Scheduler::get().reapStaleExecutors(); }
 };
 
-namespace {
-
-class DispatchPool
-{
-  public:
-    static constexpr int N = 7;
-
-    int run(const std::function<void()>& fn)
-    {
-        std::lock_guard<std::mutex> lock(mx);
-        ensureStarted();
-        current = fn;
-        generation++;
-        cv.notify_all();
-        return N;
-    }
-
-    void awaitDone(std::atomic<int>& done, int target)
-    {
-        while (done.load(std::memory_order_acquire) < target) {
-            std::this_thread::yield();
-        }
-        std::lock_guard<std::mutex> lock(mx);
-        current = nullptr;
-    }
-
-  private:
-    void ensureStarted()
-    {
-        if (started) {
-            return;
-        }
-        started = true;
-        for (int i = 0; i < N; i++) {
-            workers.emplace_back([this] { loop(); });
-            workers.back().detach();
-        }
-    }
-
-    void loop()
-    {
-        uint64_t seen = 0;
-        while (true) {
-            std::function<void()> fn;
-            {
-                std::unique_lock<std::mutex> lock(mx);
-                cv.wait(lock, [&] {
-                    return generation != seen && current != nullptr;
-                });
-                seen = generation;
-                fn = current;
-            }
-            fn();
-        }
-    }
-
-    std::mutex mx;
-    std::condition_variable cv;
-    std::vector<std::thread> workers;
-    std::function<void()> current;
-    uint64_t generation = 0;
-    bool started = false;
-};
-
-DispatchPool& dispatchPool()
-{
-    static DispatchPool* pool = new DispatchPool();
-    return *pool;
-}
-
-}
-
 Scheduler::Scheduler() = default;
 
 Scheduler& Scheduler::get()
@@ -165,16 +93,24 @@
         exec->executeTasks(idxs, req);
     } else {
         size_t n = req->messages.size();
-        auto dispatchOne = [&](size_t i) {
+        std::vector<std::shared_ptr<Executor>> execs;
+        std::vector<std::string> claimErrors;
+        PROF_START(dispatch_claim)
+        claimExecutors(*req, execs, claimErrors);
+        PROF_END(dispatch_claim)
+
+        PROF_START(dispatch_enqueue)
+        for (size_t i = 0; i < n; i++) {
             try {
-                PROF_START(dispatch_claim)
-                auto exec = claimExecutor(req->messages[i]);
-                PROF_END(dispatch_claim)
-                PROF_START(dispatch_enqueue)
-                exec->executeTasks({ (int)i }, req);
-                PROF_END(dispatch_enqueue)
+                if (!execs[i]) {
+                    throw FaabricException(claimErrors[i]);
+                }
+                execs[i]->executeSingleTask((int)i, req);
             } catch (const std::exception& e) {
                 FAM_ERROR("claiming executor failed: %s", e.what());
+                if (execs[i]) {
+                    execs[i]->releaseClaim();
+                }
                 auto msg = std::make_shared<Message>(req->messages[i]);
                 msg->returnValue = 1;
                 msg->executedHost = getSystemConfig().endpointHost;
@@ -182,67 +118,30 @@
                                   e.what();
                 getPlannerClient().setMessageResult(msg);
             }
-        };
-        if (n < 32) {
-            for (size_t i = 0; i < n; i++) {
-                dispatchOne(i);
-            }
-        } else {
-            static std::mutex fanMx;
-            std::lock_guard<std::mutex> fanLock(fanMx);
-            std::atomic<size_t> next{ 0 };
-            std::atomic<int> done{ 0 };
-            auto work = [&] {
-                size_t i;
-                while ((i = next.fetch_add(1)) < n) {
-                    dispatchOne(i);
-                }
-                done.fetch_add(1, std::memory_order_acq_rel);
-            };
-            int helpers = dispatchPool().run(work);
-            work();
-            dispatchPool().awaitDone(done, helpers + 1);
-        }
+        }
+        PROF_END(dispatch_enqueue)
     }
     PROF_END(sched_execute_batch)
 }
 
-std::shared_ptr<Executor> Scheduler::claimExecutor(Message& msg)
-{
-    std::string key = msg.user + "/" + msg.function;
-
-    {
-        std::shared_lock<std::shared_mutex> rlock(schedMx);
-        auto it = executors.find(key);
-        if (it != executors.end()) {
-            auto& pool = *it->second;
-            size_t n = pool.list.size();
-            if (n > 0) {
-                size_t start =
-                  pool.hint.fetch_add(1, std::memory_order_relaxed);
-                for (size_t k = 0; k < n; k++) {
-                    size_t i = (start + k) % n;
-                    if (pool.list[i]->tryClaim()) {
-                        return pool.list[i];
-                    }
-                }
-            }
-        }
-    }
-
-    std::unique_lock<std::shared_mutex> lock(schedMx);
-    auto& poolPtr = executors[key];
-    if (!poolPtr) {
-        poolPtr = std::make_unique<WarmPool>();
-    }
-    auto& pool = *poolPtr;
-    for (auto& e : pool.list) {
+static std::shared_ptr<Executor> popIdleClaimed(
+  Executor::IdleExecutors& idle)
+{
+    std::shared_ptr<Executor> e;
+    while (idle.pop(e)) {
         if (e->tryClaim()) {
             return e;
         }
     }
+    return nullptr;
+}
+
+std::shared_ptr<Executor> Scheduler::createExecutorLocked(WarmPool& pool,
+                                                          Message& msg)
+{
     auto exec = getExecutorFactory()->createExecutor(msg);
     exec->claim();
+    exec->setIdleList(pool.idle);
     if (getNumGpus() > 0) {
         const auto& conf = getSystemConfig();
         exec->gpuDevice =
@@ -254,6 +153,101 @@
     return exec;
 }
 
+std::shared_ptr<Executor> Scheduler::claimExecutor(Message& msg)
+{
+    std::string key = msg.user + "/" + msg.function;
+
+    {
+        std::shared_lock<std::shared_mutex> rlock(schedMx);
+        auto it = executors.find(key);
+        if (it != executors.end()) {
+            if (auto e = popIdleClaimed(*it->second->idle)) {
+                return e;
+            }
+        }
+    }
+
+    std::unique_lock<std::shared_mutex> lock(schedMx);
+    auto& poolPtr = executors[key];
+    if (!poolPtr) {
+        poolPtr = std::make_unique<WarmPool>();
+    }
+    if (auto e = popIdleClaimed(*poolPtr->idle)) {
+        return e;
+    }
+    return createExecutorLocked(*poolPtr, msg);
+}
+
+void Scheduler::claimExecutors(
+  BatchExecuteRequest& req,
+  std::vector<std::shared_ptr<Executor>>& execs,
+  std::vector<std::string>& errors)
+{
+    size_t n = req.messages.size();
+    execs.assign(n, nullptr);
+    errors.assign(n, std::string());
+
+    const Message& first = req.messages[0];
+    bool oneFunction = true;
+    for (size_t i = 1; i < n && oneFunction; i++) {
+        oneFunction = req.messages[i].function == first.function &&
+                      req.messages[i].user == first.user;
+    }
+    if (!oneFunction) {
+        for (size_t i = 0; i < n; i++) {
+            try {
+                execs[i] = claimExecutor(req.messages[i]);
+            } catch (const std::exception& e) {
+                errors[i] = e.what();
+            }
+        }
+        return;
+    }
+
+    std::string key = first.user + "/" + first.function;
+    std::vector<std::shared_ptr<Executor>> popped;
+    popped.reserve(n);
+    size_t got = 0;
+    auto takeIdle = [&](Executor::IdleExecutors& idle) {
+        while (got < n) {
+            popped.clear();
+            if (idle.popMany(n - got, popped) == 0) {
+                return;
+            }
+            for (auto& e : popped) {
+                if (e->tryClaim()) {
+                    execs[got++] = std::move(e);
+                }
+            }
+        }
+    };
+    {
+        std::shared_lock<std::shared_mutex> rlock(schedMx);
+        auto it = executors.find(key);
+        if (it != executors.end()) {
+            takeIdle(*it->second->idle);
+        }
+    }
+    if (got == n) {
+        return;
+    }
+
+    std::unique_lock<std::shared_mutex> lock(schedMx);
+    auto& poolPtr = executors[key];
+    if (!poolPtr) {
+        poolPtr = std::make_unique<WarmPool>();
+    }
+    takeIdle(*poolPtr->idle);
+    poolPtr->list.reserve(poolPtr->list.size() + (n - got));
+    for (; got < n; got++) {
+        try {
+            execs[got] = createExecutorLocked(*poolPtr, req.messages[got]);
+        } catch (const std::exception& e) {
+            errors[got] = e.what();
+        }
+    }
+}
+
 int Scheduler::reapStaleExecutors()
 {
     std::unique_lock<std::shared_mutex> lock(schedMx);
@@ -263,8 +257,9 @@
         auto& list = pool->list;
         for (auto it = list.begin(); it != list.end();) {
             auto& exec = *it;
-            if (!exec->isClaimed() &&
-                exec->getMillisSinceLastExec() > conf.boundTimeout) {
+            if (exec->getMillisSinceLastExec() > conf.boundTimeout &&
+                exec->tryClaim()) {
+                pool->idle->remove(exec);
                 exec->shutdown();
                 it = list.erase(it);
                 reaped++;
@@ -359,6 +354,7 @@
 {
     std::unique_lock<std::shared_mutex> lock(schedMx);
     for (auto& [key, pool] : executors) {
+        pool->idle->close();
         for (auto& e : pool->list) {
             e->flush();
         }
@@ -372,6 +368,7 @@
     stopReaper();
     std::unique_lock<std::shared_mutex> lock(schedMx);
     for (auto& [key, pool] : executors) {
+        pool->idle->close();
         for (auto& e : pool->list) {
             e->shutdown();
         }
@@ -405,6 +402,16 @@
     size_t n = 0;
     for (auto& [key, pool] : executors) {
         n += pool->list.size();
+    }
+    return n;
+}
+
+size_t Scheduler::debugIdleCount()
+{
+    std::shared_lock<std::shared_mutex> lock(schedMx);
+    size_t n = 0;
+    for (auto& [key, pool] : executors) {
+        n += pool->idle->size();
     }
     return n;
 }
@@ -471,8 +478,10 @@
     (void)seq;
     switch ((FunctionCalls)code) {
         case FunctionCalls::ExecuteFunctions: {
+            PROF_START(exec_decode)
             auto req = std::make_shared<BatchExecuteRequest>(
               BatchExecuteRequest::decode(body));
+            PROF_END(exec_decode)
             Scheduler::get().executeBatch(req);
             break;
         }
diff --git a/cpp/src/utilextras.cpp b/cpp/src/utilextras.cpp
--- a/cpp/src/utilextras.cpp
+++ b/cpp/src/utilextras.cpp
@@ -260,10 +260,28 @@
   profStarts;
 }
 
-static bool profEnabled()
+bool profEnabled()
 {
     static const bool v = getEnvVarInt("FAABRIC_PROF", 0) != 0;
     return v;
+}
+
+int64_t profNowNs()
+{
+    return std::chrono::duration_cast<std::chrono::nanoseconds>(
+             std::chrono::steady_clock::now().time_since_epoch())
+      .count();
+}
+
+void profRecord(const char* name, double ms)
+{
+    if (!profEnabled()) {
+        return;
+    }
+    auto& st = profState();
+    std::lock_guard<std::mutex> lock(st.mx);
+    st.totalsMs[name] += ms;
+    st.counts[name] += 1;
 }
 
 void profStart(const std::string& name)
```
